# GuidoManni/BodySLAM

Measured on AMD Instinct MI355X. Metric: frames/sec depth+pose+back-proj, 640x480 seq, higher is better.
Workload: dtype f16

## Files before the change

bodyslam_amd/_lib.py:

```python
from __future__ import annotations

import ctypes as C
import os
from typing import Optional

import torch

_HERE = os.path.dirname(os.path.abspath(__file__))
LIB_PATH = os.environ.get("BODYSLAM_HIP_LIB") or os.path.join(_HERE, "libbodyslam_hip.so")

F32, F16, BF16 = 0, 1, 2
F64 = 3
ACT_NONE, ACT_RELU, ACT_GELU, ACT_SOFTPLUS, ACT_SOFTPLUS_FAST = 0, 1, 2, 3, 4
OUT_PLAIN, OUT_SHUFFLE, OUT_QKV = 0, 1, 2

_TORCH2BS = {torch.float32: F32, torch.float16: F16, torch.bfloat16: BF16}
BS2TORCH = {F32: torch.float32, F16: torch.float16, BF16: torch.bfloat16}


class BodySlamHipError(RuntimeError):
    pass


class GemmDesc(C.Structure):
    _fields_ = [
        ("A", C.c_void_p), ("W", C.c_void_p), ("dtype", C.c_int32),
        ("M", C.c_int32), ("N", C.c_int32), ("K", C.c_int32), ("lda", C.c_int32), ("conv", C.c_int32),
        ("Hin", C.c_int32), ("Win", C.c_int32), ("Cin", C.c_int32), ("Hout", C.c_int32), ("Wout", C.c_int32),
        ("KH", C.c_int32), ("KW", C.c_int32), ("stride", C.c_int32), ("pad_h", C.c_int32), ("pad_w", C.c_int32),
        ("relu_a", C.c_int32),
        ("bias", C.c_void_p), ("bias_group_rows", C.c_int32), ("act", C.c_int32),
        ("scale", C.c_void_p), ("res", C.c_void_p), ("res_dtype", C.c_int32), ("ldr", C.c_int32), ("res2", C.c_void_p),
        ("out", C.c_void_p), ("out2", C.c_void_p), ("out3", C.c_void_p),
        ("out_dtype", C.c_int32), ("ldo", C.c_int32), ("out_mode", C.c_int32),
        ("out_group_rows", C.c_int32), ("out_group_stride", C.c_int32), ("out_row_offset", C.c_int32),
        ("shuffle_s", C.c_int32), ("shuffle_cout", C.c_int32),
        ("qkv_hidden", C.c_int32), ("qkv_tokens", C.c_int32), ("qkv_sp", C.c_int32), ("q_scale", C.c_float),
        ("tile", C.c_int32), ("seg1", C.c_int32), ("out_split_off", C.c_int32), ("res_split_off", C.c_int32),
        ("f8_seg", C.c_int32), ("f8_scales", C.c_uint32), ("out_f8", C.c_int32), ("res_f8", C.c_int32),
        ("qkv_cls_last", C.c_int32), ("qkv_cls_rows", C.c_int32), ("qkv_patch_row0", C.c_int32), ("f8_wonly_from", C.c_int32), ("out_lo8_rows", C.c_int32),
        ("f8_skip_from", C.c_int32), ("bias2_row0", C.c_int32), ("bias2_group_rows", C.c_int32), ("out_planes_rows", C.c_int32),
        ("bias2", C.c_void_p),
        ("qkv_lo_off", C.c_int32), ("out2_relu", C.c_int32),
    ]


_lib: Optional[C.CDLL] = None

_SIGS = {
    "bs_init": [C.c_int],
    "bs_version": [],
    "bs_gemm": [C.POINTER(GemmDesc), C.c_void_p],
    "bs_gemm_tile": [C.POINTER(GemmDesc)],
    "bs_attention": [C.c_void_p] * 5 + [C.c_int32] * 5 + [C.c_void_p],
    "bs_attention_table": [C.c_void_p] * 5 + [C.c_int32] * 7 + [C.c_void_p],
    "bs_attention_table_corr": [C.c_void_p] * 8 + [C.c_int32] * 7 + [C.c_void_p],
    "bs_layernorm": [C.c_void_p] * 5 + [C.c_int32, C.c_int32, C.c_float, C.c_int32, C.c_void_p],
    "bs_cast": [C.c_void_p, C.c_void_p, C.c_int64, C.c_int32, C.c_void_p],
    "bs_copy_f32": [C.c_void_p, C.c_void_p, C.c_int64, C.c_void_p],
    "bs_cast_split": [C.c_void_p, C.c_void_p, C.c_int64, C.c_int32, C.c_int32, C.c_void_p],
    "bs_relu_split": [C.c_void_p, C.c_void_p, C.c_int64, C.c_int32, C.c_int32, C.c_void_p],
    "bs_preprocess_patches": [C.c_void_p, C.c_void_p] + [C.c_int32] * 7 + [C.c_void_p],
    "bs_preprocess_image": [C.c_void_p, C.c_void_p] + [C.c_int32] * 6 + [C.c_void_p],
    "bs_fill_rows": [C.c_void_p, C.c_void_p, C.c_int32, C.c_int32, C.c_int32, C.c_void_p],
    "bs_resize_bilinear_nhwc": [C.c_void_p, C.c_void_p] + [C.c_int32] * 8 + [C.c_void_p],
    "bs_upconv_tapsum": [C.c_void_p] * 3 + [C.c_int32] * 9 + [C.c_void_p],
    "bs_upconv_fused": [C.c_void_p] * 4 + [C.c_int32] * 15 + [C.c_void_p],
    "bs_resize_bias_relu_nhwc": [C.c_void_p] * 3 + [C.c_int32] * 8 + [C.c_void_p],
    "bs_col_mean": [C.c_void_p, C.c_int64] + [C.c_int32] * 5 + [C.c_void_p, C.c_void_p, C.c_int64, C.c_int32, C.c_void_p],
    "bs_rank1_bias": [C.c_void_p] * 3 + [C.c_int32] * 3 + [C.c_void_p],
    "bs_depth_u16_to_m": [C.c_void_p, C.c_int64, C.c_double, C.c_double, C.c_void_p, C.c_void_p],
    "bs_engine_load": [C.c_char_p, C.c_void_p],
    "bs_engine_destroy": [C.c_void_p],
    "bs_engine_io": [C.c_void_p, C.c_char_p, C.c_void_p, C.c_void_p],
    "bs_engine_device_bytes": [C.c_void_p],
    "bs_engine_run": [C.c_void_p, C.c_void_p],
    "bs_engine_upload": [C.c_void_p, C.c_char_p, C.c_void_p, C.c_int64],
    "bs_engine_download": [C.c_void_p, C.c_char_p, C.c_void_p, C.c_int64],
    "bs_zoedepth_forward": [C.c_void_p, C.c_void_p, C.c_int32, C.c_int32, C.c_int32, C.c_void_p, C.c_void_p, C.c_void_p],
    "bs_cyclepose_forward": [C.c_void_p, C.c_void_p, C.c_int32, C.c_int32, C.c_int32, C.c_void_p, C.c_int32, C.c_void_p, C.c_void_p],
    "bs_tsdf_frames_upload": [C.c_void_p, C.c_void_p, C.c_void_p, C.c_void_p, C.c_void_p, C.c_int32, C.c_void_p, C.c_void_p],
    "bs_tsdf_touch_batch": [C.c_void_p, C.c_int32, C.c_int32, C.c_int32, C.c_int32, C.c_double, C.c_double, C.c_void_p, C.c_void_p, C.c_int32, C.c_void_p,
                            C.c_void_p],
    "bs_tsdf_integrate_batch": [C.c_void_p, C.c_int32, C.c_int32, C.c_int32, C.c_void_p, C.c_void_p, C.c_void_p, C.c_int32, C.c_void_p, C.c_int32, C.c_void_p,
                                C.c_void_p, C.c_void_p, C.c_void_p, C.c_int32, C.c_int32, C.c_double, C.c_double, C.c_void_p],
    "bs_tsdf_update_batch": [C.c_void_p, C.c_int32, C.c_int32, C.c_int32, C.c_void_p, C.c_void_p, C.c_void_p, C.c_int32, C.c_void_p, C.c_int32, C.c_void_p,
                             C.c_void_p, C.c_void_p, C.c_void_p, C.c_int32, C.c_int32, C.c_double, C.c_double, C.c_uint64, C.c_void_p],
    "bs_odo_prepare": [C.c_void_p, C.c_void_p, C.c_int32, C.c_int32, C.c_int32, C.c_double, C.c_void_p, C.c_void_p, C.c_void_p],
    "bs_odo_pyrdown": [C.c_void_p, C.c_int32, C.c_int32, C.c_int32, C.c_void_p, C.c_int32, C.c_double, C.c_void_p],
    "bs_odo_sobel": [C.c_void_p, C.c_int32, C.c_int32, C.c_int32, C.c_void_p, C.c_void_p, C.c_void_p],
    "bs_odo_accumulate": [C.c_void_p] * 8 + [C.c_int32, C.c_int32, C.c_void_p, C.c_void_p, C.c_double, C.c_double, C.c_double, C.c_void_p, C.c_void_p,
                                              C.c_int32, C.c_void_p],
    "bs_odo_step": [C.c_void_p] * 8 + [C.c_int32, C.c_int32, C.c_int32, C.c_void_p, C.c_void_p, C.c_int32, C.c_double, C.c_double, C.c_double, C.c_void_p,
                                        C.c_void_p, C.c_int32, C.c_void_p],
    "bs_odo_p2p_prepare": [C.c_void_p, C.c_int32, C.c_int32, C.c_int32, C.c_double, C.c_void_p, C.c_void_p],
    "bs_odo_p2p_target": [C.c_void_p, C.c_int32, C.c_int32, C.c_int32, C.c_void_p, C.c_void_p, C.c_void_p],
    "bs_odo_p2p_accumulate": [C.c_void_p, C.c_void_p, C.c_int32, C.c_int32, C.c_void_p, C.c_void_p, C.c_double, C.c_double, C.c_void_p, C.c_void_p,
                              C.c_void_p],
    "bs_odo_p2p_step": [C.c_void_p, C.c_void_p, C.c_int32, C.c_int32, C.c_int32, C.c_void_p, C.c_void_p, C.c_int32, C.c_double, C.c_double, C.c_void_p,
                        C.c_void_p, C.c_void_p],
    "bs_tsdf_touch": [C.c_void_p, C.c_int32, C.c_int32, C.c_int32, C.c_void_p, C.c_void_p, C.c_double, C.c_double, C.c_void_p, C.c_void_p, C.c_void_p,
                      C.c_int32, C.c_int32, C.c_void_p, C.c_int32, C.c_void_p, C.c_void_p, C.c_void_p],
    "bs_tsdf_integrate": [C.c_void_p, C.c_void_p, C.c_int32, C.c_int32, C.c_void_p, C.c_void_p, C.c_void_p, C.c_void_p, C.c_int32, C.c_void_p, C.c_int32,
                          C.c_int32, C.c_double, C.c_double, C.c_void_p, C.c_void_p],
    "bs_tsdf_extract": [C.c_void_p, C.c_int32, C.c_void_p, C.c_void_p, C.c_int32, C.c_void_p, C.c_int32, C.c_int32, C.c_double, C.c_void_p, C.c_void_p,
                        C.c_void_p, C.c_void_p, C.c_void_p, C.c_void_p],
    "bs_tsdf_mesh": [C.c_void_p, C.c_int32, C.c_void_p, C.c_void_p, C.c_int32, C.c_void_p, C.c_int32, C.c_int32, C.c_double, C.c_void_p, C.c_int32] + [C.c_void_p] * 7,
    "bs_tsdf_raycast": [C.c_void_p, C.c_void_p, C.c_int32, C.c_int32, C.c_int32, C.c_double, C.c_double, C.c_void_p, C.c_void_p, C.c_int32, C.c_void_p,
                        C.c_int32, C.c_int32, C.c_double, C.c_double, C.c_void_p, C.c_void_p, C.c_void_p, C.c_void_p, C.c_void_p],
    "bs_attractor_step": [C.c_void_p] * 4 + [C.c_int32] * 8 + [C.c_void_p],
    "bs_add_resized": [C.c_void_p] * 3 + [C.c_int32] * 7 + [C.c_void_p],
    "bs_mlp2": [C.c_void_p, C.c_int32] + [C.c_void_p] * 5 + [C.c_int32] * 6 + [C.c_void_p],
    "bs_mlp2_add": [C.c_void_p] * 7 + [C.c_int32] * 10 + [C.c_void_p],
    "bs_projector_level": [C.c_void_p] * 10 + [C.c_int32] * 9 + [C.c_void_p],
    "bs_logbinom_depth": [C.c_void_p] * 8 + [C.c_int32] * 5 + [C.c_float, C.c_float, C.c_int32, C.c_void_p],
    "bs_logbinom_depth_ex": [C.c_void_p] * 7 + [C.c_int32] + [C.c_void_p] * 2 + [C.c_int32] * 5 + [C.c_float, C.c_float, C.c_int32, C.c_void_p],
    "bs_small_attention": [C.c_void_p, C.c_void_p, C.c_int32, C.c_int32, C.c_int32, C.c_int32, C.c_void_p],
    "bs_route_argmax": [C.c_void_p, C.c_int32, C.c_void_p, C.c_int32, C.c_void_p],
    "bs_postprocess_depth": [C.c_void_p] * 3 + [C.c_int32] * 6 + [C.c_void_p],
    "bs_cyclepose_im2col": [C.c_void_p] * 3 + [C.c_int32] * 4 + [C.c_void_p],
    "bs_cyclepose_im2col_window": [C.c_void_p] * 3 + [C.c_int32] * 8 + [C.c_void_p],
    "bs_instnorm_relu_nhwc": [C.c_void_p] * 4 + [C.c_int32] * 3 + [C.c_float, C.c_int32, C.c_void_p],
    "bs_avgpool_nhwc": [C.c_void_p, C.c_void_p, C.c_int32, C.c_int32, C.c_int32, C.c_void_p],
    "bs_cyclepose_head": [C.c_void_p] * 12 + [C.c_int32] * 3 + [C.c_void_p],
    "bs_backproject": [C.c_void_p, C.c_int32, C.c_int32, C.c_int32, C.c_void_p, C.c_double, C.c_double] + [C.c_void_p] * 6,
    "bs_pose_chain": [C.c_void_p, C.c_int32, C.c_void_p, C.c_void_p, C.c_void_p],
# ... 18 lines not shown
    "bs_loop_register": [C.c_void_p, C.c_int32, C.c_void_p, C.c_int32, C.c_void_p, C.c_void_p, C.c_int32, C.c_double, C.c_int32, C.c_int32,
                         C.c_int32, C.c_uint64, C.c_void_p, C.c_void_p, C.c_void_p],
    "bs_pg_linearise": [C.c_void_p, C.c_int32] + [C.c_void_p] * 5 + [C.c_int32, C.c_double, C.c_int32] + [C.c_void_p] * 8,
    "bs_pg_assemble": [C.c_void_p, C.c_void_p, C.c_int32, C.c_int32, C.c_void_p, C.c_void_p, C.c_int32, C.c_int32] + [C.c_void_p] * 5,
    "bs_pg_solve": [C.c_void_p] * 4 + [C.c_int32, C.c_int32, C.c_double, C.c_void_p, C.c_int32, C.c_void_p, C.c_int32, C.c_void_p, C.c_void_p, C.c_int32,
                                       C.c_void_p, C.c_int32, C.c_int32] + [C.c_void_p] * 7,
    "bs_pg_update": [C.c_void_p, C.c_void_p, C.c_int32] + [C.c_void_p] * 4,
    "bs_pc_bounds": [C.c_void_p, C.c_int64, C.c_void_p, C.c_void_p],
    "bs_pc_grid_count": [C.c_void_p, C.c_int64, C.c_void_p, C.c_void_p, C.c_float, C.c_void_p, C.c_void_p, C.c_void_p],
    "bs_pc_grid_scatter": [C.c_void_p, C.c_int64, C.c_void_p, C.c_void_p, C.c_float, C.c_void_p, C.c_void_p, C.c_int64, C.c_void_p, C.c_void_p],
    "bs_pc_query_grid": [C.c_void_p, C.c_void_p, C.c_int64, C.c_void_p, C.c_void_p, C.c_float, C.c_void_p, C.c_void_p, C.c_int64, C.c_float, C.c_int32,
                         C.c_void_p, C.c_void_p, C.c_void_p, C.c_void_p, C.c_void_p],
    "bs_pc_query_brute": [C.c_void_p, C.c_int64, C.c_void_p, C.c_void_p, C.c_int64, C.c_float, C.c_void_p, C.c_void_p, C.c_void_p, C.c_void_p],
    "bs_pc_transform": [C.c_void_p, C.c_int32, C.c_int64, C.c_void_p, C.c_void_p, C.c_void_p],
    "bs_pc_stats": [C.c_void_p, C.c_int64, C.c_void_p, C.c_int32, C.c_void_p, C.c_int64, C.c_void_p, C.c_void_p],
    "bs_icp_step": [C.c_void_p, C.c_void_p, C.c_int64, C.c_void_p, C.c_void_p, C.c_float, C.c_void_p, C.c_void_p, C.c_void_p, C.c_int64, C.c_void_p,
                    C.c_int32, C.c_int64, C.c_float, C.c_int32, C.c_int32, C.c_void_p, C.c_void_p, C.c_void_p],
    "bs_icp_finish": [C.c_void_p, C.c_int64, C.c_void_p, C.c_void_p, C.c_int32, C.c_int32, C.c_int32, C.c_double, C.c_double, C.c_void_p, C.c_void_p],
}
EXPORTS = sorted(list(_SIGS) + ["bs_last_error"])


def load_library() -> C.CDLL:
    global _lib
    if _lib is not None:
        return _lib
    if not os.path.exists(LIB_PATH):
        raise BodySlamHipError(
            f"{LIB_PATH} is missing: build it with `python -c 'import __graft_entry__ as g; g.build()'` "
            f"(or `make -C bodyslam_amd/csrc`).  There is no CPU fallback.")
    lib = C.CDLL(LIB_PATH)
    for name, args in _SIGS.items():
        fn = getattr(lib, name)
        fn.argtypes = args
        fn.restype = C.c_int
    lib.bs_last_error.restype = C.c_char_p
    lib.bs_last_error.argtypes = []
    lib.bs_engine_device_bytes.restype = C.c_int64
    lib.bs_depth_metrics_workspace.restype = C.c_int64
    _lib = lib
    return lib


_inited_device: Optional[int] = None


def init(device: int = 0) -> None:
    global _inited_device
    lib = load_library()
    if _inited_device == device:
        return
    if not torch.cuda.is_available():
        raise BodySlamHipError("bodyslam_amd needs an MI355X (gfx950) GPU: torch.cuda.is_available() is False "
                               "and there is no CPU fallback")
    check(lib.bs_init(device), "bs_init")
    _inited_device = device


def check(status: int, what: str) -> None:
    if status != 0:
        msg = load_library().bs_last_error().decode(errors="replace")
        raise BodySlamHipError(f"{what} failed with status {status}: {msg}")


def stream_ptr() -> int:
    return torch.cuda.current_stream().cuda_stream


def dt(t: torch.Tensor) -> int:
    return _TORCH2BS[t.dtype]


def p(t: Optional[torch.Tensor]) -> Optional[int]:
    return None if t is None else t.data_ptr()


def make_gemm_desc(A: torch.Tensor, W: torch.Tensor, out: torch.Tensor, *, M: int, N: int, K: int, lda: int,
                   conv=None, relu_a: bool = False, bias: Optional[torch.Tensor] = None, bias_group_rows: int = 0,
                   act: int = ACT_NONE, scale: Optional[torch.Tensor] = None, res: Optional[torch.Tensor] = None,
                   res2: Optional[torch.Tensor] = None, ldr: int = 0, ldo: Optional[int] = None, out_group=None,
                   shuffle=None, qkv=None, a_offset: int = 0, tile: int = 0, seg1: int = 0, out_split_off: int = 0,
                   res_split_off: int = 0, f8_seg: int = 0, f8_scales=(127, 127, 127, 127), out_f8=None, res_f8: bool = False,
                   f8_wonly_from: int = 0, out_lo8_rows: int = 0, f8_skip_from: int = 0, bias2=None, out_planes_rows: int = 0,
                   out_relu: Optional[torch.Tensor] = None) -> GemmDesc:
    d = GemmDesc()
    d.A = A.data_ptr() + a_offset * A.element_size()
    d.W = W.data_ptr()
    assert A.dtype == W.dtype and A.dtype in (torch.float16, torch.bfloat16), (A.dtype, W.dtype)
    d.dtype = dt(A)
    d.M, d.N, d.K, d.lda = M, N, K, lda
    if conv is not None:
        d.conv = 1
        (d.Hin, d.Win, d.Cin, d.Hout, d.Wout, d.KH, d.KW, d.stride, d.pad_h, d.pad_w) = conv
    d.relu_a = int(relu_a)
    if bias is not None:
        assert bias.dtype == torch.float32
        d.bias = bias.data_ptr()
    d.bias_group_rows = bias_group_rows
    d.act = act
    if scale is not None:
        assert scale.dtype == torch.float32
        d.scale = scale.data_ptr()
    if res is not None:
        d.res = res.data_ptr()
        d.res_dtype = dt(res)
        d.ldr = ldr if ldr else N
    if res2 is not None:
        assert res is not None and res2.dtype == A.dtype
        d.res2 = res2.data_ptr()
    d.out = out.data_ptr()
    d.out_dtype = dt(out)
    d.ldo = N if ldo is None else ldo
    if out_group is not None:
        d.out_group_rows, d.out_group_stride, d.out_row_offset = out_group
    if shuffle is not None:
        d.out_mode = OUT_SHUFFLE
        d.shuffle_s, d.shuffle_cout, d.Hout, d.Wout = shuffle
    if qkv is not None:
        d.out_mode = OUT_QKV
        hidden, tokens, sp, q_scale, out_k, out_vt = qkv[:6]
        d.qkv_cls_last = int(bool(qkv[6])) if len(qkv) > 6 else 0
        d.qkv_cls_rows = int(qkv[7]) if len(qkv) > 7 else 0
        d.qkv_patch_row0 = int(qkv[8]) if len(qkv) > 8 else d.qkv_cls_rows
        d.qkv_lo_off = int(qkv[9]) if len(qkv) > 9 else 0
        d.qkv_hidden, d.qkv_tokens, d.qkv_sp, d.q_scale = hidden, tokens, sp, q_scale
        d.out2 = out_k.data_ptr()
        d.out3 = out_vt.data_ptr()
    d.tile = tile
    d.seg1, d.out_split_off, d.res_split_off = seg1, out_split_off, res_split_off
    d.f8_seg = f8_seg
    d.f8_scales = f8_scales[0] | (f8_scales[1] << 8) | (f8_scales[2] << 16) | (f8_scales[3] << 24)
    d.out_f8 = 0 if out_f8 is None else ((out_f8[0] & 0xff) | ((out_f8[1] & 0xff) << 8))
    d.res_f8 = int(res_f8)
    d.f8_wonly_from = f8_wonly_from
    d.out_lo8_rows = out_lo8_rows
    d.f8_skip_from = f8_skip_from
    d.out_planes_rows = out_planes_rows
    if bias2 is not None:
        b2, row0, grows = bias2
        assert b2.dtype == torch.float32 and b2.shape[-1] == N
        d.bias2, d.bias2_row0, d.bias2_group_rows = b2.data_ptr(), row0, grows
    if out_relu is not None:
        assert qkv is None and out_f8 is not None and out_relu.dtype == out.dtype and out_relu.numel() == out.numel()
        d.out2 = out_relu.data_ptr()
        d.out2_relu = 1
    return d


def gemm(A: torch.Tensor, W: torch.Tensor, out: torch.Tensor, **kw) -> None:
    d = make_gemm_desc(A, W, out, **kw)
    check(load_library().bs_gemm(C.byref(d), stream_ptr()), "bs_gemm")


def _gemm_bytes(d) -> float:
    rows_in = float(d.M if not d.conv else d.M / max(d.stride * d.stride, 1))
    rows_f8 = 0.0 if d.f8_skip_from < 0 else (rows_in if (d.conv or not d.f8_skip_from) else float(min(d.f8_skip_from, d.M)))
    taps = d.KH * d.KW if d.conv else 1
    a = rows_in * (d.Cin if d.conv else d.K) * 2 + rows_f8 * d.f8_seg
    w = float(d.N) * (d.K * 2 + taps * d.f8_seg)
    if d.out_dtype == F32:
        per_row = [4.0, 4.0, 4.0]
    elif d.out_f8:
        per_row = [4.0, 3.0, 2.0]
    else:
        per_row = [2.0 * (2 if d.out_split_off else 1)] * 3
    full = float(d.M)
    r_planes = float(min(d.out_planes_rows, d.M)) if d.out_planes_rows else full
    r_lo = float(min(d.out_lo8_rows, d.M)) if d.out_lo8_rows else r_planes
    r_lo = min(r_lo, r_planes)
    out = d.N * (r_lo * per_row[0] + (r_planes - r_lo) * per_row[1] + (full - r_planes) * per_row[2])
    res = float(d.M) * d.N * (4 if (d.res and d.res_dtype == F32) else 0)
    return a + w + out + res


class Plan:

    def __init__(self, device=None):
        self.device = None if device is None else torch.device(device)
        self.calls = []
        self.names = []
        self.keep = []
        self.keep_descs = []
        self.marks = {}
        self.gemm_info = {}
        self.stack_info = {}
        self.events = None
        self._graph = None

    def gemm(self, name, A, W, out, **kw):
        passes = kw.pop("precision_passes", 1)
        d = make_gemm_desc(A, W, out, **kw)
        kw["precision_passes"] = passes
        self.keep.append((d, A, W, out, kw))
        self.keep_descs.append(d)
        self.calls.append((load_library().bs_gemm, (C.byref(d),)))
        self.names.append(name)
        self.gemm_info[len(self.calls) - 1] = dict(
            name=name, tile=load_library().bs_gemm_tile(C.byref(d)), conv=bool(d.conv),
            flops=2.0 * d.N * (d.M * d.K + (0 if d.f8_skip_from < 0 else (min(d.f8_skip_from, d.M) if d.f8_skip_from else d.M)) * (d.KH * d.KW if d.conv else 1) * d.f8_seg
                               / (4 if d.f8_wonly_from else 2)),
            alg_flops=2.0 * d.M * d.N * (d.K / kw.get("precision_passes", 1)),
            bytes=_gemm_bytes(d))

    def add(self, name, fn_name, *args):
        cargs = []
        for a in args:
            if isinstance(a, torch.Tensor):
                self.keep.append(a)
                cargs.append(a.data_ptr())
            else:
                cargs.append(a)
        self.calls.append((getattr(load_library(), fn_name), tuple(cargs)))
        self.names.append(name)

    def tag_stack(self, alg_flops: float, flops: float):
        self.stack_info[len(self.calls) - 1] = dict(name=self.names[-1], alg_flops=float(alg_flops), flops=float(flops))

    def mark(self, name, tensor, meta=None):
        self.marks.setdefault(len(self.calls), []).append((name, tensor, meta))

    def run_timed(self, events: list):
        stream = torch.cuda.current_stream(self.device)
        st = stream.cuda_stream
        for i, (fn, args) in enumerate(self.calls):
            if i in self.gemm_info or i in self.stack_info:
                e0, e1 = torch.cuda.Event(enable_timing=True), torch.cuda.Event(enable_timing=True)
                e0.record(stream)
                rc = fn(*args, st)
                e1.record(stream)
                events.append((i, e0, e1))
            else:
                rc = fn(*args, st)
            if rc:
                check(rc, self.names[i])

    def capture(self):
        if self._graph is not None:
            return
        self.run()
        torch.cuda.synchronize(self.device)
        g = torch.cuda.CUDAGraph()
        cap = torch.cuda.Stream(device=self.device)
        cap.wait_stream(torch.cuda.current_stream(self.device))
        with torch.cuda.stream(cap):
            with torch.cuda.graph(g, stream=cap, capture_error_mode="thread_local"):
                self.run()
        torch.cuda.current_stream(self.device).wait_stream(cap)
        self._graph = g

    def run(self, taps: Optional[dict] = None):
        if taps is None and self.events is not None:
            return self.run_timed(self.events)
        if taps is None and self._graph is not None and not torch.cuda.is_current_stream_capturing():
            self._graph.replay()
            return
        st = torch.cuda.current_stream(self.device).cuda_stream
        if taps is None:
            for i, (fn, args) in enumerate(self.calls):
                rc = fn(*args, st)
                if rc:
                    check(rc, self.names[i])
            return
        means = taps.get("__site_means__")
        for i in range(len(self.calls) + 1):
            for (name, t, meta) in self.marks.get(i, []):
                if meta and meta[0] == "chanmean":
                    if means is not None:
                        _, off, M, lda, K = meta
                        means[name] = t.view(-1)[off: off + M * lda].view(M, lda)[:, :K].float().mean(0)
                    continue
                if means is None:
                    taps[name] = (t.clone(), meta)
            if i < len(self.calls):
                fn, args = self.calls[i]
                check(fn(*args, st), self.names[i])


_F8_ON_DEVICE = {}


def _f8_pack_device(device):
    if device is None or os.environ.get("BS_PACK_ON_HOST") == "1":
        return torch.device("cpu")
    device = torch.device(device)
    if device.type != "cuda":
        return torch.device("cpu")
    ok = _F8_ON_DEVICE.get(device.index)
    if ok is None:
        g = torch.Generator().manual_seed(7)
        t = torch.cat([torch.randn(4096, generator=g) * 100.0, torch.randn(4096, generator=g) * 1e-2, torch.linspace(-460.0, 460.0, 4097),
                       torch.arange(0, 4096, dtype=torch.float32) * 2.0 ** -11, torch.tensor([0.0, -0.0, 448.0, -448.0, 2.0 ** -9, 2.0 ** -10, 3 * 2.0 ** -11])])
        t = t.clamp(-448.0, 448.0)
        try:
            ok = bool(torch.equal(t.to(torch.float8_e4m3fn).view(torch.uint8), t.to(device).to(torch.float8_e4m3fn).view(torch.uint8).cpu()))
        except Exception:
            ok = False
        _F8_ON_DEVICE[device.index] = ok
    return device if ok else torch.device("cpu")


def f8_weight(w: torch.Tensor, dtype, planes: str = "both", device=None) -> tuple:
    import math
    w = w.detach().to(_f8_pack_device(device)).float()
    hi = w.to(dtype)
    lo = w - hi.float()

    def plane(t):
        mx = float(t.abs().max())
        e = 0 if mx == 0.0 else min(int(math.floor(math.log2(448.0 / mx))), 100)
        return (t * (2.0 ** e)).clamp(-448.0, 448.0).to(torch.float8_e4m3fn).view(torch.uint8), e

    hi8, e_hi = plane(hi.float())
    lo8, e_lo = plane(lo)
    hi16 = hi.contiguous().view(torch.uint8).view(w.shape[0], -1)
    if planes == "lo":
        row = torch.cat([hi16, lo8], 1).contiguous()
    elif planes == "hi_only":
        row = torch.cat([hi16, torch.zeros_like(lo8), hi8], 1).contiguous()
    else:
        row = torch.cat([hi16, lo8, hi8], 1).contiguous()
    return row.view(dtype), (127 - e_lo, 127 - e_hi)


def f8_conv_weight(w_ohwi: torch.Tensor, dtype, device=None) -> tuple:
    import math
    w = w_ohwi.detach().to(_f8_pack_device(device)).float()
    O, kh, kw, I = w.shape
    assert I % 128 == 0, I
    hi = w.to(dtype)
    lo = w - hi.float()

    def plane(t):
        mx = float(t.abs().max())
        e = 0 if mx == 0.0 else min(int(math.floor(math.log2(448.0 / mx))), 100)
        q = (t * (2.0 ** e)).clamp(-448.0, 448.0).to(torch.float8_e4m3fn).view(torch.uint8)
        return q.reshape(O, kh, kw, I // 128, 128).permute(0, 3, 1, 2, 4).reshape(O, -1), e

    hi8, e_hi = plane(hi.float())
    lo8, e_lo = plane(lo)
    hi16 = conv_weight(hi).view(torch.uint8).view(O, -1)
    row = torch.cat([hi16, lo8, hi8], 1).contiguous()
    return row.view(dtype), (127 - e_lo, 127 - e_hi)


F8_ACT_HI_EXP, F8_ACT_LO_EXP = 0, 11


def conv_weight(w_ohwi: torch.Tensor) -> torch.Tensor:
    O, kh, kw, I = w_ohwi.shape
    assert I % 64 == 0, I
    return w_ohwi.reshape(O, kh, kw, I // 64, 64).permute(0, 3, 1, 2, 4).reshape(O, -1).contiguous()


def conv_geom(Hin, Win, Cin, KH, KW, stride, pad):
    Hout = (Hin + 2 * pad - KH) // stride + 1
# ... 386 lines not shown
```

bodyslam_amd/csrc/common.h:

```cpp
#pragma once
#include <hip/hip_runtime.h>
#include <stdint.h>
#include <stdio.h>
#include <stdlib.h>

#include <atomic>

#include "../../include/bodyslam_hip.h"

namespace bs {

typedef _Float16 f16;
typedef __bf16 bf16;
typedef _Float16 f16x4 __attribute__((ext_vector_type(4)));
typedef _Float16 f16x8 __attribute__((ext_vector_type(8)));
typedef __bf16 bf16x4 __attribute__((ext_vector_type(4)));
typedef __bf16 bf16x8 __attribute__((ext_vector_type(8)));
typedef float f32x4 __attribute__((ext_vector_type(4)));
typedef float f32x16 __attribute__((ext_vector_type(16)));
typedef unsigned int u32x4 __attribute__((ext_vector_type(4)));
typedef unsigned int u32x2 __attribute__((ext_vector_type(2)));

void set_error(const char* fmt, ...);
const void* zero_page();
// ... 70 lines not shown
    float p = 2.5060822736122645e-05f;
    p = fmaf(p, t, -0.0006993855931796134f);
    p = fmaf(p, t, 0.00785447470843792f);
    p = fmaf(p, t, -0.053071241825819016f);
    p = fmaf(p, t, -0.4590134918689728f);
    p = fmaf(p, t, -1.1511290073394775f);
    p = fmaf(p, t, -0.9999995231628418f);
    const float e = __builtin_amdgcn_exp2f(p);
    return x * (x < 0.0f ? e : 1.0f - e);
}
typedef float f32x2_ __attribute__((ext_vector_type(2)));
__device__ __forceinline__ f32x2_ gelu_erf2(f32x2_ x) {
    const f32x2_ t = __builtin_elementwise_min(__builtin_elementwise_abs(x), f32x2_{6.0f, 6.0f});
    f32x2_ p = f32x2_{2.5060822736122645e-05f, 2.5060822736122645e-05f};
    p = __builtin_elementwise_fma(p, t, f32x2_{-0.0006993855931796134f, -0.0006993855931796134f});
    p = __builtin_elementwise_fma(p, t, f32x2_{0.00785447470843792f, 0.00785447470843792f});
    p = __builtin_elementwise_fma(p, t, f32x2_{-0.053071241825819016f, -0.053071241825819016f});
    p = __builtin_elementwise_fma(p, t, f32x2_{-0.4590134918689728f, -0.4590134918689728f});
    p = __builtin_elementwise_fma(p, t, f32x2_{-1.1511290073394775f, -1.1511290073394775f});
    p = __builtin_elementwise_fma(p, t, f32x2_{-0.9999995231628418f, -0.9999995231628418f});
    const f32x2_ e = {__builtin_amdgcn_exp2f(p[0]), __builtin_amdgcn_exp2f(p[1])};
    const f32x2_ om = f32x2_{1.0f, 1.0f} - e;
    const f32x2_ s = {x[0] < 0.0f ? e[0] : om[0], x[1] < 0.0f ? e[1] : om[1]};
    return x * s;
}
__device__ __forceinline__ f32x2_ bilerp2(f32x2_ p00, f32x2_ p01, f32x2_ p10, f32x2_ p11, f32x2_ hx, f32x2_ lx, f32x2_ hy, f32x2_ ly) {
    const f32x2_ top = __builtin_elementwise_fma(lx, p01, hx * p00), bot = __builtin_elementwise_fma(lx, p11, hx * p10);
    return __builtin_elementwise_fma(ly, bot, hy * top);
}
__device__ __forceinline__ float erf_as(float x) {
    const float ax = fabsf(x);
    const float t = __frcp_rn(1.0f + 0.3275911f * ax);
    const float poly = ((((1.061405429f * t - 1.453152027f) * t + 1.421413741f) * t - 0.284496736f) * t + 0.254829592f) * t;
    const float r = 1.0f - poly * __expf(-ax * ax);
    return copysignf(r, x);
}
__device__ __forceinline__ float gelu_erf_as(float x) { return 0.5f * x * (1.0f + erf_as(x * 0.70710678118654752440f)); }
__device__ __forceinline__ f32x2_ gelu_erf_as2(f32x2_ x) {
    const f32x2_ ax = __builtin_elementwise_abs(x) * f32x2_{0.70710678118654752440f, 0.70710678118654752440f};
    const f32x2_ den = __builtin_elementwise_fma(f32x2_{0.3275911f, 0.3275911f}, ax, f32x2_{1.0f, 1.0f});
    const f32x2_ t = {__builtin_amdgcn_rcpf(den[0]), __builtin_amdgcn_rcpf(den[1])};
    f32x2_ q = __builtin_elementwise_fma(f32x2_{1.061405429f, 1.061405429f}, t, f32x2_{-1.453152027f, -1.453152027f});
    q = __builtin_elementwise_fma(q, t, f32x2_{1.421413741f, 1.421413741f});
    q = __builtin_elementwise_fma(q, t, f32x2_{-0.284496736f, -0.284496736f});
    q = __builtin_elementwise_fma(q, t, f32x2_{0.254829592f, 0.254829592f});
    q = q * t;
    const f32x2_ arg = (ax * ax) * f32x2_{-1.4426950408889634f, -1.4426950408889634f};
    const f32x2_ ex = {__builtin_amdgcn_exp2f(arg[0]), __builtin_amdgcn_exp2f(arg[1])};
    const f32x2_ r = __builtin_elementwise_fma(-q, ex, f32x2_{1.0f, 1.0f});
    const f32x2_ erf = {copysignf(r[0], x[0]), copysignf(r[1], x[1])};
    return (x * f32x2_{0.5f, 0.5f}) * (erf + f32x2_{1.0f, 1.0f});
}
__device__ __forceinline__ float softplus20(float x) { return x > 20.0f ? x : log1pf(expf(x)); }
__device__ __forceinline__ float softplus_fast(float x) {
    const float e = __builtin_amdgcn_exp2f(x * 1.4426950408889634f);
    const float series = e * fmaf(e, fmaf(e, fmaf(e, -0.25f, 0.3333333432674408f), -0.5f), 1.0f);
    const float lg = __builtin_amdgcn_logf(1.0f + e) * 0.6931471805599453f;
    const float y = e < 0.015625f ? series : lg;
    return x > 20.0f ? x : y;
}

__device__ __forceinline__ float apply_act(float y, int act) {
    if (act == BS_ACT_RELU) return fmaxf(y, 0.0f);
    if (act == BS_ACT_GELU) return gelu_erf(y);
    if (act == BS_ACT_SOFTPLUS) return softplus20(y);
    if (act == BS_ACT_SOFTPLUS_FAST) return softplus_fast(y);
    return y;
}

__device__ __forceinline__ int f8_pack4(float a, float b, float c, float d) {
    auto cl = [](float v) { return __builtin_amdgcn_fmed3f(v, -448.0f, 448.0f); };
    int r = 0;
    r = __builtin_amdgcn_cvt_pk_fp8_f32(cl(a), cl(b), r, false);
    r = __builtin_amdgcn_cvt_pk_fp8_f32(cl(c), cl(d), r, true);
    return r;
}
__device__ __forceinline__ void f8_unpack4(int packed, float (&o)[4]) {
    typedef float f32x2 __attribute__((ext_vector_type(2)));
    const f32x2 a = __builtin_amdgcn_cvt_pk_f32_fp8(packed, false), b = __builtin_amdgcn_cvt_pk_f32_fp8(packed, true);
    o[0] = a[0]; o[1] = a[1]; o[2] = b[0]; o[3] = b[1];
}
constexpr int F8_ACT_HI_EXP = BS_F8_ACT_HI_EXP, F8_ACT_LO_EXP = BS_F8_ACT_LO_EXP;

__device__ __forceinline__ void glds16(const void* gptr, void* lds_wave_base) {
    __builtin_amdgcn_global_load_lds((const __attribute__((address_space(1))) void*)gptr,
                                     (__attribute__((address_space(3))) void*)lds_wave_base, 16, 0, 0);
}

static inline int cdiv(int a, int b) { return (a + b - 1) / b; }
static inline int64_t cdiv64(int64_t a, int64_t b) { return (a + b - 1) / b; }

}
```

bodyslam_amd/csrc/elementwise.hip:

```cpp
#include "common.h"

namespace bs {

template <typename T>
__global__ __launch_bounds__(256) void layernorm_kernel(const float* x, const float* gamma, const float* beta, T* out16, float* out32,
                                                         int rows, int cols, float eps, int split, int plane_rows) {
    const int row = blockIdx.x * 4 + (threadIdx.x >> 6), lane = threadIdx.x & 63;
    if (row >= rows) return;
    const float* xr = x + (int64_t)row * cols;
    constexpr int VPT = 4;
    f32x4 v[VPT];
    const int nvec = cols >> 2;
    const bool cached = nvec <= 64 * VPT;
    float s = 0.f;
    if (cached) {
#pragma unroll
        for (int i = 0; i < VPT; ++i) {
            const int vi = lane + i * 64;
            v[i] = vi < nvec ? *reinterpret_cast<const f32x4*>(xr + vi * 4) : f32x4{0, 0, 0, 0};
            s += v[i][0] + v[i][1] + v[i][2] + v[i][3];
        }
    } else {
        for (int vi = lane; vi < nvec; vi += 64) {
            const f32x4 t = *reinterpret_cast<const f32x4*>(xr + vi * 4);
// ... 144 lines not shown
    const int b = blockIdx.x;
    for (int i = threadIdx.x; i < cols; i += blockDim.x) x[(int64_t)b * rows_per_image * cols + i] = v[i];
}

struct PreGeom {
    int H, W, ph, pw, nh, nw;
    float sy, sx;
};

__device__ __forceinline__ float pre_sample(const uint8_t* frame, const PreGeom& g, int c, int y, int x) {
    const float fy = g.sy * (float)y, fx = g.sx * (float)x;
    const int Hp = g.H + 2 * g.ph, Wp = g.W + 2 * g.pw;
    int y0 = (int)fy, x0 = (int)fx;
    y0 = y0 > Hp - 1 ? Hp - 1 : y0;
    x0 = x0 > Wp - 1 ? Wp - 1 : x0;
    const int y1 = y0 + (y0 < Hp - 1 ? 1 : 0), x1 = x0 + (x0 < Wp - 1 ? 1 : 0);
    const float ly = fy - (float)y0, lx = fx - (float)x0;
    const float hy = 1.0f - ly, hx = 1.0f - lx;
    auto refl = [](int i, int pad, int n) {
        int s = i - pad;
        s = s < 0 ? -s : s;
        return s >= n ? 2 * (n - 1) - s : s;
    };
    const int sy0 = refl(y0, g.ph, g.H), sy1 = refl(y1, g.ph, g.H);
    const int sx0 = refl(x0, g.pw, g.W), sx1 = refl(x1, g.pw, g.W);
    const float k = 1.0f / 255.0f;
    const float p00 = (float)frame[((int64_t)sy0 * g.W + sx0) * 3 + c] * k;
    const float p01 = (float)frame[((int64_t)sy0 * g.W + sx1) * 3 + c] * k;
    const float p10 = (float)frame[((int64_t)sy1 * g.W + sx0) * 3 + c] * k;
    const float p11 = (float)frame[((int64_t)sy1 * g.W + sx1) * 3 + c] * k;
    const float v = hy * (hx * p00 + lx * p01) + ly * (hx * p10 + lx * p11);
    return (v - 0.5f) / 0.5f;
}

template <typename T>
__global__ __launch_bounds__(256) void pre_patches_kernel(const uint8_t* frames, T* out, int B, int nimg, PreGeom g, int split) {
    const int hp = g.nh / 16, wp = g.nw / 16;
    const int64_t total = (int64_t)nimg * hp * wp * 768;
    const int64_t gid = (int64_t)blockIdx.x * blockDim.x + threadIdx.x;
    if (gid >= total) return;
    const int k = (int)(gid % 768);
    const int64_t r = gid / 768;
    const int px = (int)(r % wp), py = (int)((r / wp) % hp), img = (int)(r / ((int64_t)wp * hp));
    const int c = k >> 8, ky = (k >> 4) & 15, kx = k & 15;
    const int y = py * 16 + ky;
    int x = px * 16 + kx;
    const int b = img >= B ? img - B : img;
    if (img >= B) x = g.nw - 1 - x;
    const float v = pre_sample(frames + (int64_t)b * g.H * g.W * 3, g, c, y, x);
    const T hi = T16<T>::from_f32(v);
    if (split == 2) {
        out[r * 1536 + k] = hi;
        char* planes = reinterpret_cast<char*>(out + r * 1536 + 768);
        planes[k] = (char)(f8_pack4(v * __builtin_ldexpf(1.0f, F8_ACT_HI_EXP), 0.f, 0.f, 0.f) & 0xff);
        planes[768 + k] = (char)(f8_pack4((v - T16<T>::to_f32(hi)) * __builtin_ldexpf(1.0f, F8_ACT_LO_EXP), 0.f, 0.f, 0.f) & 0xff);
    } else if (split) {
        out[r * 1536 + k] = hi;
        out[r * 1536 + 768 + k] = T16<T>::from_f32(v - T16<T>::to_f32(hi));
    } else {
        out[gid] = hi;
    }
}

__global__ __launch_bounds__(256) void pre_image_kernel(const uint8_t* frames, float* out, int B, int nimg, PreGeom g) {
    const int64_t total = (int64_t)nimg * 3 * g.nh * g.nw;
    const int64_t gid = (int64_t)blockIdx.x * blockDim.x + threadIdx.x;
    if (gid >= total) return;
    int x = (int)(gid % g.nw);
    const int y = (int)((gid / g.nw) % g.nh), c = (int)((gid / ((int64_t)g.nw * g.nh)) % 3), img = (int)(gid / ((int64_t)3 * g.nw * g.nh));
    const int b = img >= B ? img - B : img;
    if (img >= B) x = g.nw - 1 - x;
    out[gid] = pre_sample(frames + (int64_t)b * g.H * g.W * 3, g, c, y, x);
}

template <typename T, bool LO = true, bool HI8 = true>
__global__ __launch_bounds__(256) void resize_nhwc_f8_kernel(const T* x, T* out, int B, int Hin, int Win, int C, int Hout, int Wout, float sy,
                                                              float sx, int align) {
    const int c16n = C >> 4;
    const unsigned idx = blockIdx.x * blockDim.x + threadIdx.x;
    if (idx >= (unsigned)Wout * c16n) return;
    const int c16 = idx % c16n, ox = idx / c16n;
    const int b = blockIdx.y / Hout, oy = blockIdx.y - b * Hout;
    const int64_t pix = ((int64_t)b * Hout + oy) * Wout + ox;
    float fy, fx;
    if (align) {
        fy = sy * (float)oy;
        fx = sx * (float)ox;
    } else {
        fy = fmaxf(__fmaf_rn(sy, (float)oy + 0.5f, -0.5f), 0.0f);
        fx = fmaxf(__fmaf_rn(sx, (float)ox + 0.5f, -0.5f), 0.0f);
    }
    int y0 = (int)fy, x0 = (int)fx;
    y0 = y0 > Hin - 1 ? Hin - 1 : y0;
    x0 = x0 > Win - 1 ? Win - 1 : x0;
    const int y1 = y0 + (y0 < Hin - 1 ? 1 : 0), x1 = x0 + (x0 < Win - 1 ? 1 : 0);
    const float ly = fy - (float)y0, lx = fx - (float)x0, hy = 1.0f - ly, hx = 1.0f - lx;
    typedef typename T16<T>::v8 v8;
    typedef int i32x4 __attribute__((ext_vector_type(4)));
    const T* xb = x + (int64_t)b * Hin * Win * C * 2;
    const float sc = __builtin_ldexpf(1.0f, -F8_ACT_LO_EXP);
    float q00[16], q01[16], q10[16], q11[16];
    auto ld = [&](int yy, int xx, float (&q)[16]) {
        const T* pp = xb + ((int64_t)yy * Win + xx) * C * 2;
        const v8 h0 = *reinterpret_cast<const v8*>(pp + c16 * 16), h1 = *reinterpret_cast<const v8*>(pp + c16 * 16 + 8);
        const i32x4 l = *reinterpret_cast<const i32x4*>(reinterpret_cast<const char*>(pp + C + (C >> 1)) + c16 * 16);
#pragma unroll
        for (int e = 0; e < 8; ++e) {
            q[e] = (float)h0[e];
            q[8 + e] = (float)h1[e];
        }
#pragma unroll
        for (int g = 0; g < 4; ++g) {
            float lo[4];
            f8_unpack4(l[g], lo);
#pragma unroll
            for (int e = 0; e < 4; ++e) q[4 * g + e] = fmaf(lo[e], sc, q[4 * g + e]);
        }
    };
    ld(y0, x0, q00);
    ld(y0, x1, q01);
    ld(y1, x0, q10);
    ld(y1, x1, q11);
    v8 o0, o1;
    float vv[16], rl[16];
    const f32x2_ hx2 = {hx, hx}, lx2 = {lx, lx}, hy2 = {hy, hy}, ly2 = {ly, ly};
#pragma unroll
    for (int e = 0; e < 16; e += 2) {
        const f32x2_ v2 = bilerp2(f32x2_{q00[e], q00[e + 1]}, f32x2_{q01[e], q01[e + 1]}, f32x2_{q10[e], q10[e + 1]}, f32x2_{q11[e], q11[e + 1]}, hx2, lx2, hy2, ly2);
#pragma unroll
        for (int u = 0; u < 2; ++u) {
            const float v = v2[u];
            vv[e + u] = v;
            const T h = T16<T>::from_f32(v);
            if (e + u < 8) o0[e + u] = h; else o1[e + u - 8] = h;
            if (LO) rl[e + u] = v - (float)h;
        }
    }
    T* op = out + pix * C * 2;
    *reinterpret_cast<v8*>(op + c16 * 16) = o0;
    *reinterpret_cast<v8*>(op + c16 * 16 + 8) = o1;
    if (!HI8) return;
    const float sh = __builtin_ldexpf(1.0f, F8_ACT_HI_EXP), sl = __builtin_ldexpf(1.0f, F8_ACT_LO_EXP);
    char* planes = reinterpret_cast<char*>(op + C);
    i32x4 ph, pl;
#pragma unroll
    for (int g = 0; g < 4; ++g) {
        ph[g] = f8_pack4(vv[4 * g] * sh, vv[4 * g + 1] * sh, vv[4 * g + 2] * sh, vv[4 * g + 3] * sh);
        if (LO) pl[g] = f8_pack4(rl[4 * g] * sl, rl[4 * g + 1] * sl, rl[4 * g + 2] * sl, rl[4 * g + 3] * sl);
    }
    *reinterpret_cast<i32x4*>(planes + c16 * 16) = ph;
    if (LO) *reinterpret_cast<i32x4*>(planes + C + c16 * 16) = pl;
}

template <typename T, int SPLIT>
__global__ __launch_bounds__(256) void upconv_tapsum_kernel(const float* y, const float* bias, T* out, int B, int Hin, int Win, int Co, int Hout,
                                                             int Wout, float sy, float sx, int align, int relu) {
    const int groups = Co >> 2;
    const int per = 256 / groups, TW = per >= 8 ? 8 : per, TH = per / TW;
    const int g = threadIdx.x % groups, px = threadIdx.x / groups;
    const int ox = blockIdx.x * TW + px % TW;
    const int nty = (Hout + TH - 1) / TH;
    const int b = blockIdx.y / nty, oy = (blockIdx.y - b * nty) * TH + px / TW;
    if (px >= per || ox >= Wout || oy >= Hout) return;
    const int ld = 9 * Co;
    const float* yb = y + (int64_t)b * Hin * Win * ld + 4 * g;
    typedef float f32x4_ __attribute__((ext_vector_type(4)));
    f32x4_ acc = *reinterpret_cast<const f32x4_*>(bias + 4 * g);
#pragma unroll
    for (int ky = 0; ky < 3; ++ky) {
        const int r = oy + ky - 1;
        if (r < 0 || r >= Hout) continue;
        const float fy = align ? sy * (float)r : fmaxf(__fmaf_rn(sy, (float)r + 0.5f, -0.5f), 0.0f);
        int y0 = (int)fy;
        y0 = y0 > Hin - 1 ? Hin - 1 : y0;
        const int y1 = y0 + (y0 < Hin - 1 ? 1 : 0);
        const float ly = fy - (float)y0, hy = 1.0f - ly;
#pragma unroll
        for (int kx = 0; kx < 3; ++kx) {
            const int c = ox + kx - 1;
            if (c < 0 || c >= Wout) continue;
            const float fx = align ? sx * (float)c : fmaxf(__fmaf_rn(sx, (float)c + 0.5f, -0.5f), 0.0f);
            int x0 = (int)fx;
            x0 = x0 > Win - 1 ? Win - 1 : x0;
            const int x1 = x0 + (x0 < Win - 1 ? 1 : 0);
            const float lx = fx - (float)x0, hx = 1.0f - lx;
            const float* yt = yb + (ky * 3 + kx) * Co;
            const f32x4_ q00 = *reinterpret_cast<const f32x4_*>(yt + ((int64_t)y0 * Win + x0) * ld);
            const f32x4_ q01 = *reinterpret_cast<const f32x4_*>(yt + ((int64_t)y0 * Win + x1) * ld);
            const f32x4_ q10 = *reinterpret_cast<const f32x4_*>(yt + ((int64_t)y1 * Win + x0) * ld);
            const f32x4_ q11 = *reinterpret_cast<const f32x4_*>(yt + ((int64_t)y1 * Win + x1) * ld);
            typedef float f32x2 __attribute__((ext_vector_type(2)));
            const f32x2 hx2 = {hx, hx}, lx2 = {lx, lx}, hy2 = {hy, hy}, ly2 = {ly, ly};
#pragma unroll
            for (int e = 0; e < 4; e += 2) {
                const f32x2 top = __builtin_elementwise_fma(lx2, f32x2{q01[e], q01[e + 1]}, hx2 * f32x2{q00[e], q00[e + 1]});
                const f32x2 bot = __builtin_elementwise_fma(lx2, f32x2{q11[e], q11[e + 1]}, hx2 * f32x2{q10[e], q10[e + 1]});
                const f32x2 v = __builtin_elementwise_fma(ly2, bot, hy2 * top);
                acc[e] += v[0];
                acc[e + 1] += v[1];
            }
        }
    }
    if (relu) {
#pragma unroll
        for (int e = 0; e < 4; ++e) acc[e] = fmaxf(acc[e], 0.0f);
    }
    const int64_t pix = ((int64_t)b * Hout + oy) * Wout + ox;
    typedef T t4 __attribute__((ext_vector_type(4)));
    t4 hi;
    float rl[4];
#pragma unroll
    for (int e = 0; e < 4; ++e) {
        hi[e] = T16<T>::from_f32(acc[e]);
        rl[e] = acc[e] - T16<T>::to_f32(hi[e]);
    }
    if (SPLIT == 0) {
        *reinterpret_cast<t4*>(out + pix * Co + 4 * g) = hi;
    } else if (SPLIT == 1) {
        t4 lo;
#pragma unroll
        for (int e = 0; e < 4; ++e) lo[e] = T16<T>::from_f32(rl[e]);
        *reinterpret_cast<t4*>(out + pix * 2 * Co + 4 * g) = hi;
        *reinterpret_cast<t4*>(out + pix * 2 * Co + Co + 4 * g) = lo;
    } else {
        T* op = out + pix * 2 * Co;
        *reinterpret_cast<t4*>(op + 4 * g) = hi;
        const float sh = __builtin_ldexpf(1.0f, F8_ACT_HI_EXP), sl = __builtin_ldexpf(1.0f, F8_ACT_LO_EXP);
        char* planes = reinterpret_cast<char*>(op + Co);
        *reinterpret_cast<int*>(planes + 4 * g) = f8_pack4(acc[0] * sh, acc[1] * sh, acc[2] * sh, acc[3] * sh);
        *reinterpret_cast<int*>(planes + Co + 4 * g) = f8_pack4(rl[0] * sl, rl[1] * sl, rl[2] * sl, rl[3] * sl);
    }
}
// ... 51 lines not shown
            const float l = f - (float)i0, h = 1.0f - l;
            e = i32x4_{(i0 - w0) * unit, (i1 - w0) * unit, __float_as_int(h), __float_as_int(l)};
        }
        tabs[tid] = e;
    }
    asm volatile("s_waitcnt vmcnt(0)" ::: "memory");
    __syncthreads();
    const int g = tid & 7;
    const f32x4_ bias4 = *reinterpret_cast<const f32x4_*>(bias + 4 * g);
    const char* yg = smem + TS_TAB + 16 * g;
    for (int it = 0; it < TS_TW * TS_TH / 64; ++it) {
        const int px = it * 64 + (tid >> 3);
        const int lx_ = px % TS_TW, ly_ = px / TS_TW;
        const int ox = tx0 + lx_, oy = ty0 + ly_;
        if (ox >= Wout || oy >= Hout) continue;
        f32x2 a01 = {bias4[0], bias4[1]}, a23 = {bias4[2], bias4[3]};
#pragma unroll
        for (int ky = 0; ky < 3; ++ky) {
            const i32x4_ ry = tabs[ly_ + ky];
            const float hy = __int_as_float(ry[2]), wy = __int_as_float(ry[3]);
#pragma unroll
            for (int kx = 0; kx < 3; ++kx) {
                const i32x4_ cx = tabs[TS_TH + 2 + lx_ + kx];
                const float hx = __int_as_float(cx[2]), wx = __int_as_float(cx[3]);
                const char* yt = yg + (ky * 3 + kx) * Co * 4;
                const f32x4_ q00 = *reinterpret_cast<const f32x4_*>(yt + ry[0] + cx[0]);
                const f32x4_ q01 = *reinterpret_cast<const f32x4_*>(yt + ry[0] + cx[1]);
                const f32x4_ q10 = *reinterpret_cast<const f32x4_*>(yt + ry[1] + cx[0]);
                const f32x4_ q11 = *reinterpret_cast<const f32x4_*>(yt + ry[1] + cx[1]);
                const float w00 = hy * hx, w01 = hy * wx, w10 = wy * hx, w11 = wy * wx;
                const f32x2 v00 = {w00, w00}, v01 = {w01, w01}, v10 = {w10, w10}, v11 = {w11, w11};
                a01 = __builtin_elementwise_fma(v00, f32x2{q00[0], q00[1]}, a01);
                a23 = __builtin_elementwise_fma(v00, f32x2{q00[2], q00[3]}, a23);
                a01 = __builtin_elementwise_fma(v01, f32x2{q01[0], q01[1]}, a01);
                a23 = __builtin_elementwise_fma(v01, f32x2{q01[2], q01[3]}, a23);
                a01 = __builtin_elementwise_fma(v10, f32x2{q10[0], q10[1]}, a01);
                a23 = __builtin_elementwise_fma(v10, f32x2{q10[2], q10[3]}, a23);
                a01 = __builtin_elementwise_fma(v11, f32x2{q11[0], q11[1]}, a01);
                a23 = __builtin_elementwise_fma(v11, f32x2{q11[2], q11[3]}, a23);
            }
        }
        f32x4_ acc = {a01[0], a01[1], a23[0], a23[1]};
        if (relu) {
#pragma unroll
            for (int e = 0; e < 4; ++e) acc[e] = fmaxf(acc[e], 0.0f);
        }
        const int64_t pix = ((int64_t)b * Hout + oy) * Wout + ox;
        typedef T t4 __attribute__((ext_vector_type(4)));
        t4 hi;
        float rl[4];
#pragma unroll
        for (int e = 0; e < 4; ++e) {
            hi[e] = T16<T>::from_f32(acc[e]);
            rl[e] = acc[e] - T16<T>::to_f32(hi[e]);
        }
        if (SPLIT == 0) {
            *reinterpret_cast<t4*>(out + pix * Co + 4 * g) = hi;
        } else if (SPLIT == 1) {
            t4 lo;
#pragma unroll
            for (int e = 0; e < 4; ++e) lo[e] = T16<T>::from_f32(rl[e]);
            *reinterpret_cast<t4*>(out + pix * 2 * Co + 4 * g) = hi;
            *reinterpret_cast<t4*>(out + pix * 2 * Co + Co + 4 * g) = lo;
        } else {
            T* op = out + pix * 2 * Co;
            *reinterpret_cast<t4*>(op + 4 * g) = hi;
            const float sh = __builtin_ldexpf(1.0f, F8_ACT_HI_EXP), sl = __builtin_ldexpf(1.0f, F8_ACT_LO_EXP);
            char* planes = reinterpret_cast<char*>(op + Co);
            *reinterpret_cast<int*>(planes + 4 * g) = f8_pack4(acc[0] * sh, acc[1] * sh, acc[2] * sh, acc[3] * sh);
            *reinterpret_cast<int*>(planes + Co + 4 * g) = f8_pack4(rl[0] * sl, rl[1] * sl, rl[2] * sl, rl[3] * sl);
        }
    }
}

template <typename T, bool ADD, int SPLIT, bool BIAS_RELU = false>
__global__ __launch_bounds__(256) void resize_nhwc_kernel(const T* x, const T* addend, T* out, int B, int Hin, int Win, int C, int Hout,
                                                           int Wout, float sy, float sx, int align, const float* bias = nullptr) {
    const int c8n = C >> 3;
    const unsigned idx = blockIdx.x * blockDim.x + threadIdx.x;
    if (idx >= (unsigned)Wout * c8n) return;
    const int c8 = idx % c8n, ox = idx / c8n;
    const int b = blockIdx.y / Hout, oy = blockIdx.y - b * Hout;
    const int64_t pix = ((int64_t)b * Hout + oy) * Wout + ox;
    float fy, fx;
    if (align) {
        fy = sy * (float)oy;
        fx = sx * (float)ox;
    } else {
        fy = fmaxf(__fmaf_rn(sy, (float)oy + 0.5f, -0.5f), 0.0f);
        fx = fmaxf(__fmaf_rn(sx, (float)ox + 0.5f, -0.5f), 0.0f);
    }
    int y0 = (int)fy, x0 = (int)fx;
    y0 = y0 > Hin - 1 ? Hin - 1 : y0;
    x0 = x0 > Win - 1 ? Win - 1 : x0;
    const int y1 = y0 + (y0 < Hin - 1 ? 1 : 0), x1 = x0 + (x0 < Win - 1 ? 1 : 0);
    const float ly = fy - (float)y0, lx = fx - (float)x0, hy = 1.0f - ly, hx = 1.0f - lx;
    typedef typename T16<T>::v8 v8;
    constexpr int PS = SPLIT ? 2 : 1;
    const T* xb = x + (int64_t)b * Hin * Win * C * PS + c8 * 8;
    float q00[8], q01[8], q10[8], q11[8], av[8];
    auto ld = [&](const T* ptr, float (&dst)[8]) {
        const v8 h = *reinterpret_cast<const v8*>(ptr);
#pragma unroll
        for (int e = 0; e < 8; ++e) dst[e] = (float)h[e];
        if (SPLIT == 1) {
            const v8 l = *reinterpret_cast<const v8*>(ptr + C);
#pragma unroll
            for (int e = 0; e < 8; ++e) dst[e] += (float)l[e];
        } else if (SPLIT == 2) {
            const char* lo8 = reinterpret_cast<const char*>(ptr - c8 * 8 + C + (C >> 1)) + c8 * 8;
            const int p0 = *reinterpret_cast<const int*>(lo8), p1 = *reinterpret_cast<const int*>(lo8 + 4);
            float l0[4], l1[4];
            f8_unpack4(p0, l0);
            f8_unpack4(p1, l1);
            const float sc = __builtin_ldexpf(1.0f, -F8_ACT_LO_EXP);
#pragma unroll
            for (int e = 0; e < 4; ++e) {
                dst[e] = fmaf(l0[e], sc, dst[e]);
                dst[4 + e] = fmaf(l1[e], sc, dst[4 + e]);
            }
        }
    };
    ld(xb + ((int64_t)y0 * Win + x0) * C * PS, q00);
    ld(xb + ((int64_t)y0 * Win + x1) * C * PS, q01);
    ld(xb + ((int64_t)y1 * Win + x0) * C * PS, q10);
    ld(xb + ((int64_t)y1 * Win + x1) * C * PS, q11);
    if (ADD) ld(addend + pix * C * PS + c8 * 8, av);
    v8 o, ol;
    float vv[8];
    const f32x2_ hx2 = {hx, hx}, lx2 = {lx, lx}, hy2 = {hy, hy}, ly2 = {ly, ly};
#pragma unroll
    for (int e = 0; e < 8; e += 2) {
        f32x2_ v = bilerp2(f32x2_{q00[e], q00[e + 1]}, f32x2_{q01[e], q01[e + 1]}, f32x2_{q10[e], q10[e + 1]}, f32x2_{q11[e], q11[e + 1]}, hx2, lx2, hy2, ly2);
        if (ADD) v += f32x2_{av[e], av[e + 1]};
        if (BIAS_RELU) {
            v += *reinterpret_cast<const f32x2_*>(bias + c8 * 8 + e);
            v = f32x2_{fmaxf(v[0], 0.0f), fmaxf(v[1], 0.0f)};
        }
#pragma unroll
        for (int u = 0; u < 2; ++u) {
            vv[e + u] = v[u];
            o[e + u] = T16<T>::from_f32(v[u]);
            if (SPLIT == 1) ol[e + u] = T16<T>::from_f32(v[u] - (float)o[e + u]);
        }
    }
    *reinterpret_cast<v8*>(out + pix * C * PS + c8 * 8) = o;
    if (SPLIT == 1) *reinterpret_cast<v8*>(out + pix * C * PS + C + c8 * 8) = ol;
    if (SPLIT == 2) {
        const float sh = __builtin_ldexpf(1.0f, F8_ACT_HI_EXP), sl = __builtin_ldexpf(1.0f, F8_ACT_LO_EXP);
        char* planes = reinterpret_cast<char*>(out + pix * C * 2 + C);
        typedef int i32x2 __attribute__((ext_vector_type(2)));
        *reinterpret_cast<i32x2*>(planes + c8 * 8) = i32x2{f8_pack4(vv[0] * sh, vv[1] * sh, vv[2] * sh, vv[3] * sh),
                                                           f8_pack4(vv[4] * sh, vv[5] * sh, vv[6] * sh, vv[7] * sh)};
        *reinterpret_cast<i32x2*>(planes + C + c8 * 8) =
            i32x2{f8_pack4((vv[0] - (float)o[0]) * sl, (vv[1] - (float)o[1]) * sl, (vv[2] - (float)o[2]) * sl, (vv[3] - (float)o[3]) * sl),
                  f8_pack4((vv[4] - (float)o[4]) * sl, (vv[5] - (float)o[5]) * sl, (vv[6] - (float)o[6]) * sl, (vv[7] - (float)o[7]) * sl)};
    }
}

__device__ __forceinline__ void cubic_coeffs(float t, float (&c)[4]) {
    const float A = -0.75f;
    auto c1 = [&](float x) { return ((A + 2.0f) * x - (A + 3.0f)) * x * x + 1.0f; };
    auto c2 = [&](float x) { return ((A * x - 5.0f * A) * x + 8.0f * A) * x - 4.0f * A; };
    c[0] = c2(t + 1.0f);
    c[1] = c1(t);
    c[2] = c1(1.0f - t);
    c[3] = c2(2.0f - t);
}

__global__ __launch_bounds__(256) void postprocess_kernel(const float* dnet, float* depth_m, uint16_t* depth_u16, int B, int H, int W,
                                                           int nh, int nw, int ph, int pw, float sy, float sx, int flip) {
    const int64_t total = (int64_t)B * H * W;
    const int64_t gid = (int64_t)blockIdx.x * blockDim.x + threadIdx.x;
    if (gid >= total) return;
    const int x = (int)(gid % W), y = (int)((gid / W) % H), b = (int)(gid / ((int64_t)W * H));
    const int yp = y + ph, xp = x + pw;
    const float fy = __fmaf_rn(sy, (float)yp + 0.5f, -0.5f), fx = __fmaf_rn(sx, (float)xp + 0.5f, -0.5f);
    const float fly = floorf(fy), flx = floorf(fx);
    const int iy = (int)fly, ix = (int)flx;
    float cy[4], cx[4];
    cubic_coeffs(fy - fly, cy);
    cubic_coeffs(fx - flx, cx);
    const float* d0 = dnet + (int64_t)b * nh * nw;
    const float* d1 = dnet + (int64_t)(B + b) * nh * nw;
    float acc = 0.f;
#pragma unroll
    for (int i = 0; i < 4; ++i) {
        int yy = iy - 1 + i;
        yy = yy < 0 ? 0 : (yy > nh - 1 ? nh - 1 : yy);
        float row = 0.f;
#pragma unroll
        for (int j = 0; j < 4; ++j) {
            int xx = ix - 1 + j;
            xx = xx < 0 ? 0 : (xx > nw - 1 ? nw - 1 : xx);
            float v = d0[(int64_t)yy * nw + xx];
            if (flip) v = (v + d1[(int64_t)yy * nw + (nw - 1 - xx)]) / 2.0f;
            row += v * cx[j];
        }
        acc += row * cy[i];
    }
    depth_m[gid] = acc;
    if (depth_u16) {
        float s = acc * 256.0f;
        s = s < 0.f ? 0.f : (s > 65535.f ? 65535.f : s);
        depth_u16[gid] = (uint16_t)s;
    }
}

static PreGeom make_geom(int H, int W, int nh, int nw) {
    PreGeom g;
    g.H = H; g.W = W; g.nh = nh; g.nw = nw;
    g.ph = (int)(sqrt((double)H / 2.0) * 3.0);
    g.pw = (int)(sqrt((double)W / 2.0) * 3.0);
    g.sy = nh > 1 ? (float)(H + 2 * g.ph - 1) / (float)(nh - 1) : 0.f;
    g.sx = nw > 1 ? (float)(W + 2 * g.pw - 1) / (float)(nw - 1) : 0.f;
    return g;
}

}

using namespace bs;
#define BS_ENTRY(name) \
    if (!initialized()) { set_error(name ": call bs_init first"); return BS_ERR_NOT_INIT; }

extern "C" int bs_layernorm(const float* x, const float* gamma, const float* beta, void* out16, float* out32, int32_t rows,
                            int32_t cols, float eps, int32_t dtype, void* stream) {
    BS_ENTRY("bs_layernorm");
    BS_REQUIRE(x && gamma && beta && (out16 || out32) && rows >= 0 && cols > 0 && cols % 4 == 0, "bs_layernorm: bad argument");
    const int split = (dtype & 32) ? 2 : ((dtype & 16) ? 1 : 0);
    const int plane_rows = dtype >> 8;
    dtype &= 15;
    BS_REQUIRE(!out16 || dtype == BS_F16 || dtype == BS_BF16, "bs_layernorm: dtype");
    if (rows == 0) return BS_OK;
    hipStream_t st = reinterpret_cast<hipStream_t>(stream);
    dim3 grid(cdiv(rows, 4));
    if (dtype == BS_BF16)
        hipLaunchKernelGGL(layernorm_kernel<bf16>, grid, dim3(256), 0, st, x, gamma, beta, (bf16*)out16, out32, rows, cols, eps, split, plane_rows);
    else
        hipLaunchKernelGGL(layernorm_kernel<f16>, grid, dim3(256), 0, st, x, gamma, beta, (f16*)out16, out32, rows, cols, eps, split, plane_rows);
    BS_CHECK_LAUNCH();
    return BS_OK;
}

extern "C" int bs_cast(const float* x, void* out, int64_t n, int32_t out_dtype, void* stream) {
    BS_ENTRY("bs_cast");
    BS_REQUIRE(x && out && n >= 0 && n % 4 == 0, "bs_cast: n must be a multiple of 4");
    BS_REQUIRE(out_dtype == BS_F16 || out_dtype == BS_BF16, "bs_cast: dtype");
    if (n == 0) return BS_OK;
    hipStream_t st = reinterpret_cast<hipStream_t>(stream);
    const int64_t n4 = n / 4;
    const unsigned blocks = (unsigned)(cdiv64(n4, 256) < 8192 ? cdiv64(n4, 256) : 8192);
    if (out_dtype == BS_F16)
        hipLaunchKernelGGL(cast_kernel<f16>, dim3(blocks), dim3(256), 0, st, x, (f16*)out, n4);
    else
        hipLaunchKernelGGL(cast_kernel<bf16>, dim3(blocks), dim3(256), 0, st, x, (bf16*)out, n4);
    BS_CHECK_LAUNCH();
    return BS_OK;
}

extern "C" int bs_fill_rows(float* x, const float* v, int32_t B, int32_t rows_per_image, int32_t cols, void* stream) {
    BS_ENTRY("bs_fill_rows");
    BS_REQUIRE(x && v && B >= 0 && rows_per_image > 0 && cols > 0, "bs_fill_rows: bad argument");
    if (B == 0) return BS_OK;
    hipLaunchKernelGGL(fill_rows_kernel, dim3(B), dim3(256), 0, reinterpret_cast<hipStream_t>(stream), x, v, rows_per_image, cols);
    BS_CHECK_LAUNCH();
    return BS_OK;
}

extern "C" int bs_preprocess_patches(const uint8_t* frames, void* out, int32_t B, int32_t H, int32_t W, int32_t nh, int32_t nw,
                                     int32_t flip, int32_t out_dtype, void* stream) {
    BS_ENTRY("bs_preprocess_patches");
    BS_REQUIRE(frames && out && B >= 0 && H > 1 && W > 1 && nh % 16 == 0 && nw % 16 == 0 && nh > 0 && nw > 0,
               "bs_preprocess_patches: bad geometry");
    const int split = (out_dtype & 32) ? 2 : ((out_dtype & 16) ? 1 : 0);
    out_dtype &= 15;
    BS_REQUIRE(out_dtype == BS_F16 || out_dtype == BS_BF16, "bs_preprocess_patches: dtype");
    if (B == 0) return BS_OK;
    const PreGeom g = make_geom(H, W, nh, nw);
    BS_REQUIRE(g.ph < H && g.pw < W, "bs_preprocess_patches: reflect pad exceeds the frame");
    const int nimg = flip ? 2 * B : B;
    const int64_t total = (int64_t)nimg * (nh / 16) * (nw / 16) * 768;
    hipStream_t st = reinterpret_cast<hipStream_t>(stream);
    if (out_dtype == BS_F16)
        hipLaunchKernelGGL(pre_patches_kernel<f16>, dim3((unsigned)cdiv64(total, 256)), dim3(256), 0, st, frames, (f16*)out, B, nimg, g, split);
    else
        hipLaunchKernelGGL(pre_patches_kernel<bf16>, dim3((unsigned)cdiv64(total, 256)), dim3(256), 0, st, frames, (bf16*)out, B, nimg, g, split);
    BS_CHECK_LAUNCH();
    return BS_OK;
}

extern "C" int bs_preprocess_image(const uint8_t* frames, float* out, int32_t B, int32_t H, int32_t W, int32_t nh, int32_t nw,
                                   int32_t flip, void* stream) {
    BS_ENTRY("bs_preprocess_image");
    BS_REQUIRE(frames && out && B >= 0 && H > 1 && W > 1 && nh > 0 && nw > 0, "bs_preprocess_image: bad geometry");
    if (B == 0) return BS_OK;
    const PreGeom g = make_geom(H, W, nh, nw);
    BS_REQUIRE(g.ph < H && g.pw < W, "bs_preprocess_image: reflect pad exceeds the frame");
    const int nimg = flip ? 2 * B : B;
    const int64_t total = (int64_t)nimg * 3 * nh * nw;
    hipLaunchKernelGGL(pre_image_kernel, dim3((unsigned)cdiv64(total, 256)), dim3(256), 0, reinterpret_cast<hipStream_t>(stream), frames,
                       out, B, nimg, g);
    BS_CHECK_LAUNCH();
    return BS_OK;
}

template <typename T>
static int launch_resize(const void* x, const void* addend, void* out, int B, int Hin, int Win, int C, int Hout, int Wout, int align,
                         hipStream_t st, int split = 0) {
    float sy, sx;
    if (align) {
        sy = Hout > 1 ? (float)(Hin - 1) / (float)(Hout - 1) : 0.f;
        sx = Wout > 1 ? (float)(Win - 1) / (float)(Wout - 1) : 0.f;
    } else {
        sy = (float)Hin / (float)Hout;
        sx = (float)Win / (float)Wout;
    }
    const dim3 blocks(cdiv(Wout * (C / 8), 256), B * Hout);
    if (split >= 2 && split <= 4) {
        const dim3 blocks16(cdiv(Wout * (C / 16), 256), B * Hout);
        if (split == 4)
            hipLaunchKernelGGL((resize_nhwc_f8_kernel<T, false, false>), blocks16, dim3(256), 0, st, (const T*)x, (T*)out, B, Hin, Win, C, Hout, Wout, sy, sx, align);
        else if (split == 3)
            hipLaunchKernelGGL((resize_nhwc_f8_kernel<T, false>), blocks16, dim3(256), 0, st, (const T*)x, (T*)out, B, Hin, Win, C, Hout, Wout, sy, sx, align);
        else
            hipLaunchKernelGGL((resize_nhwc_f8_kernel<T, true>), blocks16, dim3(256), 0, st, (const T*)x, (T*)out, B, Hin, Win, C, Hout, Wout, sy, sx, align);
        BS_CHECK_LAUNCH();
        return BS_OK;
    }
    if (split) {
        if (addend)
            hipLaunchKernelGGL((resize_nhwc_kernel<T, true, 1>), blocks, dim3(256), 0, st, (const T*)x, (const T*)addend, (T*)out, B, Hin, Win,
                               C, Hout, Wout, sy, sx, align);
        else
            hipLaunchKernelGGL((resize_nhwc_kernel<T, false, 1>), blocks, dim3(256), 0, st, (const T*)x, (const T*)nullptr, (T*)out, B, Hin,
                               Win, C, Hout, Wout, sy, sx, align);
        BS_CHECK_LAUNCH();
        return BS_OK;
    }
    if (addend)
        hipLaunchKernelGGL((resize_nhwc_kernel<T, true, 0>), blocks, dim3(256), 0, st, (const T*)x, (const T*)addend, (T*)out, B, Hin,
                           Win, C, Hout, Wout, sy, sx, align);
    else
        hipLaunchKernelGGL((resize_nhwc_kernel<T, false, 0>), blocks, dim3(256), 0, st, (const T*)x, (const T*)nullptr, (T*)out, B,
                           Hin, Win, C, Hout, Wout, sy, sx, align);
    BS_CHECK_LAUNCH();
    return BS_OK;
}

template <typename T>
__global__ __launch_bounds__(256) void col_mean_kernel(const T* A, int64_t lda, int row0, int rows_per_group, int row_step, int K,
                                                        bf16* out, float* zero_out, int64_t zero_n) {
    for (int64_t i = ((int64_t)blockIdx.y * gridDim.x + blockIdx.x) * 256 + threadIdx.x; i < zero_n; i += (int64_t)gridDim.x * gridDim.y * 256)
        zero_out[i] = 0.0f;
    typedef typename T16<T>::v8 v8;
    __shared__ float red[8][32][8];
    const int tx = threadIdx.x & 31, ty = threadIdx.x >> 5;
    const int g = blockIdx.y, c0 = (blockIdx.x * 32 + tx) * 8;
    const T* base = A + ((int64_t)row0 + (int64_t)g * rows_per_group) * lda;
    float acc[8] = {0.f, 0.f, 0.f, 0.f, 0.f, 0.f, 0.f, 0.f};
    if (c0 < K) {
        for (int j = ty * row_step; j < rows_per_group; j += 8 * row_step) {
            const v8 v = *reinterpret_cast<const v8*>(base + (int64_t)j * lda + c0);
#pragma unroll
            for (int e = 0; e < 8; ++e) acc[e] += T16<T>::to_f32(v[e]);
        }
    }
#pragma unroll
    for (int e = 0; e < 8; ++e) red[ty][tx][e] = acc[e];
    __syncthreads();
    if (ty == 0 && c0 < K) {
        const int count = (rows_per_group + row_step - 1) / row_step;
        const float inv = 1.0f / (float)count;
#pragma unroll
        for (int e = 0; e < 8; ++e) {
            float s_ = 0.f;
#pragma unroll
            for (int r = 0; r < 8; ++r) s_ += red[r][tx][e];
            out[(int64_t)g * K + c0 + e] = T16<bf16>::from_f32(s_ * inv);
        }
    }
}

extern "C" int bs_col_mean(const void* A, int64_t lda, int32_t row0, int32_t rows_per_group, int32_t groups, int32_t row_step, int32_t K,
                           void* out_bf16, float* zero_out, int64_t zero_n, int32_t dtype, void* stream) {
    BS_ENTRY("bs_col_mean");
    BS_REQUIRE(A && out_bf16, "bs_col_mean: null operand");
    BS_REQUIRE(row0 >= 0 && rows_per_group > 0 && groups > 0 && row_step > 0 && K > 0 && K % 8 == 0 && lda >= K && lda % 8 == 0,
               "bs_col_mean: bad geometry (K and lda must be multiples of 8)");
    BS_REQUIRE(dtype == BS_F16 || dtype == BS_BF16, "bs_col_mean: dtype must be f16 or bf16");
    hipStream_t st = reinterpret_cast<hipStream_t>(stream);
    const dim3 grid(cdiv(K, 256), groups);
    if (dtype == BS_F16)
        hipLaunchKernelGGL((col_mean_kernel<f16>), grid, dim3(256), 0, st, (const f16*)A, lda, row0, rows_per_group, row_step, K,
                           (bf16*)out_bf16, zero_out, zero_out ? zero_n : 0);
    else
        hipLaunchKernelGGL((col_mean_kernel<bf16>), grid, dim3(256), 0, st, (const bf16*)A, lda, row0, rows_per_group, row_step, K,
                           (bf16*)out_bf16, zero_out, zero_out ? zero_n : 0);
    BS_CHECK_LAUNCH();
    return BS_OK;
// ... 243 lines not shown
```

bodyslam_amd/csrc/engine.hip:

```cpp
#include <stdio.h>
#include <string.h>

#include <exception>
#include <map>
#include <string>
#include <tuple>
#include <type_traits>
#include <utility>
#include <memory>
#include <vector>

#include "common.h"

namespace {

constexpr char kMagic[8] = {'B', 'S', 'E', 'N', 'G', '0', '2', '\0'};
enum { KIND_WORKSPACE = 0, KIND_ZERO = 1, KIND_DATA = 2 };
enum { ARG_I64 = 0, ARG_F64 = 1, ARG_PTR = 2, ARG_NULL = 3, ARG_DESC = 4 };
enum { OP_CALL = 0, OP_SIGNAL = 1, OP_WAIT = 2 };

struct Arg {
    int64_t i = 0;
    double d = 0.0;
    void* p = nullptr;
};

template <typename T>
T arg_as(const Arg& a) {
    if constexpr (std::is_pointer<T>::value) return reinterpret_cast<T>(a.p);
    else if constexpr (std::is_floating_point<T>::value) return static_cast<T>(a.d);
    else return static_cast<T>(a.i);
}
template <typename... Args, size_t... I>
int call_unpacked(int (*fn)(Args...), const Arg* args, void* st, std::index_sequence<I...>) {
    using Tup = std::tuple<Args...>;
    return fn(arg_as<std::tuple_element_t<I, Tup>>(args[I])..., st);
}
struct Entry {
    int nargs;
    int (*thunk)(const void* fn, const Arg* args, void* st);
    const void* fn;
};
template <typename... Args>
Entry make_entry(int (*fn)(Args...)) {
    static_assert(sizeof...(Args) >= 1, "an entry point takes the stream last");
    Entry e;
    e.nargs = (int)sizeof...(Args) - 1;
    e.fn = reinterpret_cast<const void*>(fn);
    e.thunk = [](const void* f, const Arg* args, void* st) {
        return call_unpacked<Args...>(reinterpret_cast<int (*)(Args...)>(const_cast<void*>(f)), args, st, std::make_index_sequence<sizeof...(Args) - 1>{});
    };
    return e;
}
#define BS_ENGINE_ENTRY(name) {#name, make_entry(name)}
const std::map<std::string, Entry>& entries() {
    static const std::map<std::string, Entry> m = {
        BS_ENGINE_ENTRY(bs_gemm),           BS_ENGINE_ENTRY(bs_attention),          BS_ENGINE_ENTRY(bs_attention_table),
        BS_ENGINE_ENTRY(bs_attention_table_corr),
        BS_ENGINE_ENTRY(bs_layernorm),      BS_ENGINE_ENTRY(bs_cast),               BS_ENGINE_ENTRY(bs_copy_f32),
        BS_ENGINE_ENTRY(bs_cast_split),     BS_ENGINE_ENTRY(bs_relu_split),         BS_ENGINE_ENTRY(bs_preprocess_patches),
        BS_ENGINE_ENTRY(bs_fill_rows),      BS_ENGINE_ENTRY(bs_upconv_tapsum),      BS_ENGINE_ENTRY(bs_small_attention),
        BS_ENGINE_ENTRY(bs_route_argmax),   BS_ENGINE_ENTRY(bs_resize_bilinear_nhwc), BS_ENGINE_ENTRY(bs_rank1_bias),
        BS_ENGINE_ENTRY(bs_postprocess_depth), BS_ENGINE_ENTRY(bs_logbinom_depth_ex), BS_ENGINE_ENTRY(bs_col_mean),
        BS_ENGINE_ENTRY(bs_attractor_step), BS_ENGINE_ENTRY(bs_add_resized),        BS_ENGINE_ENTRY(bs_instnorm_relu_nhwc),
        BS_ENGINE_ENTRY(bs_cyclepose_im2col), BS_ENGINE_ENTRY(bs_cyclepose_im2col_window), BS_ENGINE_ENTRY(bs_cyclepose_head),
        BS_ENGINE_ENTRY(bs_avgpool_nhwc),   BS_ENGINE_ENTRY(bs_mlp2),            BS_ENGINE_ENTRY(bs_mlp2_add),
        BS_ENGINE_ENTRY(bs_upconv_fused),   BS_ENGINE_ENTRY(bs_resize_bias_relu_nhwc), BS_ENGINE_ENTRY(bs_projector_level),
    };
    return m;
}

struct Op {
    int kind = OP_CALL, lane = 0;
    const Entry* entry = nullptr;
    std::vector<Arg> args;
    std::vector<char> desc;
    std::string name;
};
struct Io {
    void* ptr;
    int64_t nbytes;
};

}

struct bs_engine {
    int device = 0;
    std::vector<void*> bufs;
    std::vector<Op> ops;
    std::map<std::string, Io> io;
    hipStream_t side = nullptr;
    std::map<int, hipEvent_t> events;
    int64_t device_bytes = 0;
};

namespace {

struct Reader {
    FILE* f;
// ... 296 lines not shown
```

bodyslam_amd/csrc/igemm.hip:

```cpp
#include <stdlib.h>

#include <map>
#include <mutex>
#include <utility>

#include "igemm_kernel.h"

namespace bs {

#define BS_DECL_TILE(t, cm)                                                  \
    int igemm_launch_tile##t##_f16_cm##cm(const IgemmParams&, bool, hipStream_t); \
    int igemm_launch_tile##t##_bf16_cm##cm(const IgemmParams&, bool, hipStream_t);
BS_DECL_TILE(1, 0) BS_DECL_TILE(1, 1)
BS_DECL_TILE(2, 0) BS_DECL_TILE(2, 1)
BS_DECL_TILE(3, 0) BS_DECL_TILE(3, 1)
BS_DECL_TILE(9, 0) BS_DECL_TILE(9, 1)
BS_DECL_TILE(10, 0) BS_DECL_TILE(11, 0)
BS_DECL_TILE(9s8, 0) BS_DECL_TILE(9s8, 1)
#undef BS_DECL_TILE

static int auto_tile(int M, int N, int K, int tile, bool conv) {
    if (tile != 0) return tile;
    if (N <= 32) return 3;
    if (N <= 64) return 2;
// ... 50 lines not shown
    int dev = 0;
    BS_CHECK_HIP(hipGetDevice(&dev));
    std::lock_guard<std::mutex> lock(mu);
    auto it = lanes.find({dev, caller});
    if (it == lanes.end()) {
        TailLane l{};
        BS_CHECK_HIP(hipStreamCreateWithFlags(&l.side, hipStreamNonBlocking));
        BS_CHECK_HIP(hipEventCreateWithFlags(&l.fork, hipEventDisableTiming));
        BS_CHECK_HIP(hipEventCreateWithFlags(&l.join, hipEventDisableTiming));
        it = lanes.emplace(std::make_pair(dev, caller), l).first;
    }
    side = it->second.side; ev_fork = it->second.fork; ev_join = it->second.join;
    return BS_OK;
}

static int dispatch(IgemmParams& p, int dtype, bool conv, int tile, hipStream_t st) {
    tile = auto_tile(p.M, p.N, p.K, tile, conv);
    if ((p.f8_seg > 0 || p.out_f8 || p.res_f8) && (tile == 10 || tile == 11)) tile = 9;
    int BM, BN;
    tile_dims(tile, BM, BN);
    const int rem = p.M % BM, full = p.M / BM, ntn = cdiv(p.N, BN), cus = cu_count();
    static const bool no_split = diag_env("BS_NO_TAIL_SPLIT") != nullptr;
    if (!no_split && !(p.ablate & 8) && !conv && BM == 256 && p.K >= 2048 && full > 0 && rem > 0 && rem <= 128 && p.N % 128 == 0 &&
        cdiv(full * ntn, cus) < cdiv((full + 1) * ntn, cus)) {
        IgemmParams main = p;
        main.M = full * BM;
        main.m_begin = 0;
        p.m_begin = full * BM;
        static const bool side_ok = diag_env("BS_NO_TAIL_STREAM") == nullptr;
        hipStream_t side = nullptr;
        hipEvent_t ev_fork = nullptr, ev_join = nullptr;
        if (side_ok) {
            const int rc = tail_lane(st, side, ev_fork, ev_join);
            if (rc != BS_OK) return rc;
        }
        if (!side_ok) {
            const int rc = launch_tile(main, dtype, conv, tile, st);
            if (rc != BS_OK) return rc;
            return launch_tile(p, dtype, conv, 1, st);
        }
        BS_CHECK_HIP(hipEventRecord(ev_fork, st));
        BS_CHECK_HIP(hipStreamWaitEvent(side, ev_fork, 0));
        int rc = launch_tile(main, dtype, conv, tile, st);
        if (rc != BS_OK) return rc;
        rc = launch_tile(p, dtype, conv, 1, side);
        if (rc != BS_OK) return rc;
        BS_CHECK_HIP(hipEventRecord(ev_join, side));
        BS_CHECK_HIP(hipStreamWaitEvent(st, ev_join, 0));
        return BS_OK;
    }
    p.m_begin = 0;
    return launch_tile(p, dtype, conv, tile, st);
}

}

extern "C" int bs_gemm_tile(const bs_gemm_desc* d) {
    if (!d) return BS_ERR_INVALID;
    const int tile = bs::auto_tile(d->M, d->N, d->K + d->f8_seg / 2, d->tile % 100, d->conv != 0);
    return ((d->f8_seg > 0 || d->out_f8 || d->res_f8) && (tile == 10 || tile == 11)) ? 9 : tile;
}

extern "C" int bs_gemm(const bs_gemm_desc* d, void* stream) {
    using namespace bs;
    if (!initialized()) { set_error("bs_gemm: call bs_init first"); return BS_ERR_NOT_INIT; }
    BS_REQUIRE(d && d->A && d->W && d->out, "bs_gemm: null operand");
    BS_REQUIRE(d->dtype == BS_F16 || d->dtype == BS_BF16, "bs_gemm: dtype must be f16 or bf16");
    BS_REQUIRE(d->M > 0 && d->N > 0 && d->K > 0, "bs_gemm: empty problem M=%d N=%d K=%d", d->M, d->N, d->K);
    BS_REQUIRE(d->N % 4 == 0, "bs_gemm: N=%d must be a multiple of 4", d->N);
    BS_REQUIRE(d->K % 64 == 0, "bs_gemm: K=%d must be a multiple of 64", d->K);
    BS_REQUIRE(d->lda % 8 == 0, "bs_gemm: lda=%d must be a multiple of 8 (16-byte rows)", d->lda);
    BS_REQUIRE(d->out_dtype == BS_F32 || d->out_dtype == d->dtype, "bs_gemm: out_dtype must be f32 or the operand dtype");
    BS_REQUIRE(!d->res || d->res_dtype == BS_F32 || d->res_dtype == d->dtype, "bs_gemm: res_dtype must be f32 or the operand dtype");
    IgemmParams p{};
    p.A = d->A; p.W = d->W; p.zero = zero_page();
    p.a_bytes = d->conv ? (long long)(d->M / (d->Hout > 0 && d->Wout > 0 ? d->Hout * d->Wout : 1)) * d->Hin * d->Win * d->lda * 2
                        : ((long long)(d->M - 1) * d->lda + (d->K + d->f8_seg / 2 - d->seg1)) * 2;
    BS_REQUIRE((long long)d->N * (d->K + d->f8_seg / 2) * 2 < 0x7FFFFFF0ll, "bs_gemm: weight matrix too large for one descriptor");
    p.M = d->M; p.N = d->N; p.K = d->K + d->f8_seg / 2; p.lda = d->lda;
    p.f8_seg = d->f8_seg;
    p.f8_sa0 = d->f8_scales & 0xff; p.f8_sb0 = (d->f8_scales >> 8) & 0xff; p.f8_sa1 = (d->f8_scales >> 16) & 0xff; p.f8_sb1 = d->f8_scales >> 24;
    p.out_f8 = d->out_f8;
    p.res_f8 = d->res_f8;
    BS_REQUIRE(!d->res_f8 || (d->res && d->res_dtype == d->dtype && d->res_split_off == 0 && d->ldr >= 2 * d->N && d->N % 8 == 0), "bs_gemm: res_f8 needs a 16-bit residual in (hi16 | hi8 | lo8) rows, ldr >= 2N");
    BS_REQUIRE(d->f8_seg >= 0 && d->f8_seg % 256 == 0, "bs_gemm: f8_seg=%d must be a multiple of 256 (two halves of whole 128-byte stages)", d->f8_seg);
    BS_REQUIRE(d->f8_seg == 0 || (d->seg1 == 0 && !d->relu_a), "bs_gemm: the FP8 segment excludes seg1 and relu_a");
    p.f8_stages = d->f8_seg / 128;
    BS_REQUIRE(d->out_f8 == 0 || (d->out_dtype == d->dtype && d->ldo % 8 == 0 &&
                                  ((d->out_mode == BS_OUT_PLAIN && d->out_split_off == d->N && d->N % 8 == 0) ||
                                   (d->out_mode == BS_OUT_SHUFFLE && d->out_split_off == d->shuffle_cout && d->shuffle_cout % 8 == 0))),
               "bs_gemm: out_f8 needs a plain / shuffle 16-bit output with out_split_off = channels, channels %% 8 == 0");
    p.Hin = d->Hin; p.Win = d->Win; p.Cin = d->Cin; p.Hout = d->Hout; p.Wout = d->Wout;
    p.KH = d->KH; p.KW = d->KW; p.stride = d->stride; p.pad_h = d->pad_h; p.pad_w = d->pad_w;
    if (d->conv) {
        BS_REQUIRE(d->Cin > 0 && d->Cin % 64 == 0, "bs_gemm: conv Cin=%d must be a multiple of 64", d->Cin);
        BS_REQUIRE(d->K == d->KH * d->KW * (d->Cin + d->seg1), "bs_gemm: conv K=%d != KH*KW*(Cin+seg1)", d->K);
        BS_REQUIRE(d->Hout > 0 && d->Wout > 0 && d->M % (d->Hout * d->Wout) == 0, "bs_gemm: conv M=%d not a multiple of Hout*Wout", d->M);
        BS_REQUIRE(d->stride > 0 && d->lda >= d->Cin, "bs_gemm: bad conv stride/lda");
        BS_REQUIRE(d->KH > 0 && d->KW > 0 && d->KH * d->KW <= 32, "bs_gemm: conv window %dx%d: at most 32 taps", d->KH, d->KW);
        BS_REQUIRE((long long)d->Hin * d->Win * d->lda * 2 * 4 < 0x7FFFFFF0ll, "bs_gemm: image too large for the 2 GiB tile window");
        p.tiles_per_tap = d->Cin / 64;
        if (d->f8_seg > 0) {
            BS_REQUIRE(d->f8_seg == 2 * d->Cin && d->Cin % 128 == 0 && d->lda >= 2 * d->Cin, "bs_gemm: conv FP8 segment needs f8_seg = 2*Cin, Cin %% 128 == 0, lda >= 2*Cin");
            p.Cin = 2 * d->Cin;
            p.K = d->KH * d->KW * p.Cin;
            p.f8_stages = d->KH * d->KW * (d->f8_seg / 128);
            BS_REQUIRE((long long)d->N * p.K * 2 < 0x7FFFFFF0ll, "bs_gemm: weight matrix too large for one descriptor");
        }
    }
    p.relu_a = d->relu_a;
    p.cin1 = d->seg1;
    p.split_off = d->out_split_off;
    p.res_split_off = d->res_split_off;
    BS_REQUIRE(d->seg1 >= 0 && d->seg1 % 64 == 0, "bs_gemm: seg1=%d must be a multiple of 64", d->seg1);
    BS_REQUIRE(d->conv || d->seg1 < d->K, "bs_gemm: seg1 must be smaller than K");
    BS_REQUIRE(d->out_split_off == 0 || (d->out_mode != BS_OUT_QKV && d->out_dtype == d->dtype), "bs_gemm: split output needs a plain / shuffle 16-bit output");
    BS_REQUIRE(d->res_split_off == 0 || (d->res && d->res_dtype == d->dtype), "bs_gemm: split residual must be 16-bit");
    p.ablate = d->tile >= 100 ? d->tile / 100 : 0;

    BS_REQUIRE(!d->relu_a || d->conv, "bs_gemm: relu_a is only built for conv mode");
    BS_REQUIRE(d->act >= BS_ACT_NONE && d->act <= BS_ACT_SOFTPLUS_FAST, "bs_gemm: unknown activation %d", d->act);
    p.bias = d->bias; p.bias_group_rows = d->bias_group_rows; p.act = d->act; p.scale = d->scale;
    p.res = d->res; p.res2 = d->res2; p.res_dtype = d->res_dtype; p.ldr = d->ldr;
    BS_REQUIRE(!d->res2 || d->res, "bs_gemm: res2 needs res (they share ldr)");
    p.out = d->out; p.out2 = d->out2; p.out3 = d->out3; p.out_dtype = d->out_dtype; p.ldo = d->ldo; p.out_mode = d->out_mode;
    p.out_group_rows = d->out_group_rows; p.out_group_stride = d->out_group_stride; p.out_row_offset = d->out_row_offset;
    p.shuffle_s = d->shuffle_s; p.shuffle_cout = d->shuffle_cout;
    p.qkv_hidden = d->qkv_hidden; p.qkv_tokens = d->qkv_tokens; p.qkv_sp = d->qkv_sp; p.q_scale = d->q_scale;
    p.qkv_cls_last = d->qkv_cls_last;
    p.qkv_cls_rows = d->qkv_cls_rows;
    p.qkv_patch_row0 = d->qkv_patch_row0;
    p.qkv_lo_off = d->qkv_lo_off;
    p.out2_relu = d->out2_relu;
    BS_REQUIRE(!d->out2_relu || (d->out2 && d->out_mode == BS_OUT_PLAIN && d->out_f8 && !d->scale && !d->out_group_rows && !d->bias_group_rows &&
                                 !d->bias2 && (d->act == BS_ACT_NONE || d->act == BS_ACT_RELU) && d->out_split_off == d->N && d->N % 256 == 0 &&
                                 d->ldo % 8 == 0 && d->out_dtype == d->dtype && (!d->res || d->res_f8)),
               "bs_gemm: out2_relu needs the plain (hi16 | hi8 | lo8) output form (out_f8, N %% 256 == 0, no scale / row groups / bias2)");
    BS_REQUIRE(d->qkv_lo_off == 0 || (d->out_mode == BS_OUT_QKV && d->qkv_lo_off > 0 && d->qkv_lo_off % 8 == 0),
               "bs_gemm: qkv_lo_off needs BS_OUT_QKV and a multiple of 8 elements");
    p.f8_wonly_from = d->f8_wonly_from;
    p.out_lo8_rows = d->out_lo8_rows;
    p.f8_skip_from = d->f8_skip_from;
    p.out_planes_rows = d->out_planes_rows;
    BS_REQUIRE(d->out_planes_rows == 0 || (d->out_f8 && d->out_planes_rows > 0 && d->out_planes_rows % 256 == 0),
               "bs_gemm: out_planes_rows needs out_f8 and a multiple of 256 rows");
    p.bias2 = d->bias2;
    p.bias2_row0 = d->bias2_row0;
    p.bias2_group_rows = d->bias2_group_rows;
    BS_REQUIRE(d->f8_skip_from == 0 || (d->f8_seg > 0 && (d->f8_skip_from == -1 || (d->f8_skip_from > 0 && d->f8_skip_from % 256 == 0 && !d->conv))),
               "bs_gemm: f8_skip_from needs the FP8 correction segment and is -1 (every tile) or, for a plain GEMM, a multiple of 256 rows");
    BS_REQUIRE(!d->bias2 || (d->bias2_group_rows > 0 && d->bias2_row0 >= 0 && d->bias_group_rows == 0 && !d->conv && d->out_mode != BS_OUT_SHUFFLE &&
                             d->N % 4 == 0),
               "bs_gemm: bias2 needs bias2_group_rows > 0, a plain GEMM (PLAIN or QKV output) and no bias_group_rows");
    BS_REQUIRE(d->out_lo8_rows == 0 || (d->out_f8 && d->out_lo8_rows % 256 == 0), "bs_gemm: out_lo8_rows needs out_f8 and a multiple of 256 rows");
    BS_REQUIRE(d->f8_wonly_from == 0 || d->f8_seg > 0, "bs_gemm: f8_wonly_from needs the FP8 correction segment");
    BS_REQUIRE(d->qkv_cls_rows == 0 || (d->out_mode == BS_OUT_QKV && d->qkv_cls_last && d->qkv_tokens > 1 && d->qkv_patch_row0 >= d->qkv_cls_rows &&
                                        d->M == d->qkv_patch_row0 + d->qkv_cls_rows * (d->qkv_tokens - 1)),
               "bs_gemm: qkv_cls_rows needs BS_OUT_QKV, qkv_cls_last and M = qkv_patch_row0 + qkv_cls_rows * (tokens - 1)");
    if (d->out_mode == BS_OUT_SHUFFLE) {
        BS_REQUIRE(!d->conv && d->shuffle_s > 0 && d->shuffle_cout % 4 == 0 && d->N == d->shuffle_s * d->shuffle_s * d->shuffle_cout,
                   "bs_gemm: bad shuffle geometry");
        BS_REQUIRE(d->Hout > 0 && d->Wout > 0 && d->M % (d->Hout * d->Wout) == 0, "bs_gemm: shuffle needs the input grid in Hout/Wout");
    } else if (d->out_mode == BS_OUT_QKV) {
        BS_REQUIRE(d->out2 && d->out3 && d->qkv_hidden % 64 == 0 && d->N == 3 * d->qkv_hidden && d->qkv_tokens > 0 &&
                       (d->qkv_cls_rows > 0 || d->M % d->qkv_tokens == 0) && d->qkv_sp >= d->qkv_tokens && d->out_dtype == d->dtype,
                   "bs_gemm: bad qkv geometry");
    } else {
        BS_REQUIRE(d->out_mode == BS_OUT_PLAIN && d->ldo >= d->N, "bs_gemm: bad out_mode/ldo");
        BS_REQUIRE(d->ldo % 4 == 0, "bs_gemm: ldo must be a multiple of 4");
    }
    hipStream_t st = reinterpret_cast<hipStream_t>(stream);
    const int tile = d->tile % 100;
    return dispatch(p, d->dtype, d->conv != 0, tile, st);
}
```

bodyslam_amd/csrc/igemm_kernel.h:

```cpp
#pragma once
#include <type_traits>

#include "common.h"

namespace bs {

struct IgemmParams {
    const void* A;
    const void* W;
    const void* zero;
    long long a_bytes;
    int M, N, K, lda;
    int Hin, Win, Cin, Hout, Wout, KH, KW, stride, pad_h, pad_w;
    int tiles_per_tap;
    int cin1;
    int split_off;
    int res_split_off;
    int relu_a;
    const float* bias;
    int bias_group_rows;
    int act;
    const float* scale;
    const void* res;
    const void* res2;
    int res_dtype, ldr;
    void* out;
    void* out2;
    void* out3;
    int out_dtype, ldo, out_mode;
    int out_group_rows, out_group_stride, out_row_offset;
    int shuffle_s, shuffle_cout;
    int qkv_hidden, qkv_tokens, qkv_sp;
    int qkv_cls_last;
    int qkv_cls_rows;
    int qkv_patch_row0;
    int qkv_lo_off;
    int f8_wonly_from;
    float q_scale;
    int ntm, ntn;
    int m_begin;
    int f8_seg;
    int f8_sa0, f8_sb0, f8_sa1, f8_sb1;
    int f8_stages;
    int res_f8;
    int out_f8;
    int out2_relu;
    int out_lo8_rows;
    int f8_skip_from;
    int out_planes_rows;
    const float* bias2;
    int bias2_row0, bias2_group_rows;
    int strip;
    int ablate;
};

template <typename T>
__device__ __forceinline__ typename T16<T>::v8 relu8(typename T16<T>::v8 x) {
    typedef short s16x8 __attribute__((ext_vector_type(8)));
    s16x8 b = __builtin_bit_cast(s16x8, x);
    s16x8 neg = b >> 15;
    b = b & ~neg;
    return __builtin_bit_cast(typename T16<T>::v8, b);
}

template <typename T>
__device__ __forceinline__ void store4(void* base, int64_t off, int out_dtype, const float (&y)[4], int split_off = 0) {
    if (split_off > 0) {
        typename T16<T>::v4 h, l;
#pragma unroll
        for (int e = 0; e < 4; ++e) {
            h[e] = T16<T>::from_f32(y[e]);
            l[e] = T16<T>::from_f32(y[e] - T16<T>::to_f32(h[e]));
        }
        *reinterpret_cast<typename T16<T>::v4*>(reinterpret_cast<T*>(base) + off) = h;
        *reinterpret_cast<typename T16<T>::v4*>(reinterpret_cast<T*>(base) + off + split_off) = l;
        return;
    }
    if (out_dtype == BS_F32) {
        f32x4 v = {y[0], y[1], y[2], y[3]};
        *reinterpret_cast<f32x4*>(reinterpret_cast<float*>(base) + off) = v;
    } else {
        typename T16<T>::v4 v;
        v[0] = T16<T>::from_f32(y[0]);
        v[1] = T16<T>::from_f32(y[1]);
        v[2] = T16<T>::from_f32(y[2]);
        v[3] = T16<T>::from_f32(y[3]);
        *reinterpret_cast<typename T16<T>::v4*>(reinterpret_cast<T*>(base) + off) = v;
    }
}

template <typename T>
__device__ __forceinline__ void store8(void* base, int64_t off, int out_dtype, const float (&y)[8], int split_off = 0) {
    typedef typename T16<T>::v8 v8;
    if (split_off > 0) {
        v8 h, l;
#pragma unroll
        for (int e = 0; e < 8; ++e) {
            h[e] = T16<T>::from_f32(y[e]);
            l[e] = T16<T>::from_f32(y[e] - T16<T>::to_f32(h[e]));
        }
        *reinterpret_cast<v8*>(reinterpret_cast<T*>(base) + off) = h;
        *reinterpret_cast<v8*>(reinterpret_cast<T*>(base) + off + split_off) = l;
        return;
    }
    if (out_dtype == BS_F32) {
        *reinterpret_cast<f32x4*>(reinterpret_cast<float*>(base) + off) = f32x4{y[0], y[1], y[2], y[3]};
        *reinterpret_cast<f32x4*>(reinterpret_cast<float*>(base) + off + 4) = f32x4{y[4], y[5], y[6], y[7]};
    } else {
        v8 v;
#pragma unroll
        for (int e = 0; e < 8; ++e) v[e] = T16<T>::from_f32(y[e]);
        *reinterpret_cast<v8*>(reinterpret_cast<T*>(base) + off) = v;
    }
}

template <typename T>
__device__ __forceinline__ void store8_f8(void* base, int64_t row_off, int n, int plane_off, const float (&y)[8], int ea, int el, bool lo = true,
                                          bool hi8 = true) {
    typedef typename T16<T>::v8 v8;
    typedef int i32x2 __attribute__((ext_vector_type(2)));
    v8 h;
    f32x2_ yh[4];
    const float sa = __builtin_ldexpf(1.0f, ea), sl = __builtin_ldexpf(1.0f, el);
    const f32x2_ sa2 = {sa, sa}, sl2 = {sl, sl};
#pragma unroll
    for (int e = 0; e < 8; e += 2) {
        h[e] = T16<T>::from_f32(y[e]);
        h[e + 1] = T16<T>::from_f32(y[e + 1]);
        const f32x2_ v = f32x2_{y[e], y[e + 1]} * sa2;
        yh[e >> 1] = f32x2_{__builtin_amdgcn_fmed3f(v[0], -448.0f, 448.0f), __builtin_amdgcn_fmed3f(v[1], -448.0f, 448.0f)};
    }
    T* rowp = reinterpret_cast<T*>(base) + row_off;
    *reinterpret_cast<v8*>(rowp + n) = h;
    if (!hi8) return;
    int ph0 = 0, ph1 = 0;
    ph0 = __builtin_amdgcn_cvt_pk_fp8_f32(yh[0][0], yh[0][1], ph0, false);
    ph0 = __builtin_amdgcn_cvt_pk_fp8_f32(yh[1][0], yh[1][1], ph0, true);
    ph1 = __builtin_amdgcn_cvt_pk_fp8_f32(yh[2][0], yh[2][1], ph1, false);
    ph1 = __builtin_amdgcn_cvt_pk_fp8_f32(yh[3][0], yh[3][1], ph1, true);
    char* bytes = reinterpret_cast<char*>(rowp + plane_off);
    *reinterpret_cast<i32x2*>(bytes + n) = i32x2{ph0, ph1};
    if (lo) {
        f32x2_ yl[4];
#pragma unroll
        for (int e = 0; e < 8; e += 2) {
            const f32x2_ r = (f32x2_{y[e], y[e + 1]} + f32x2_{-T16<T>::to_f32(h[e]), -T16<T>::to_f32(h[e + 1])}) * sl2;
            yl[e >> 1] = f32x2_{__builtin_amdgcn_fmed3f(r[0], -448.0f, 448.0f), __builtin_amdgcn_fmed3f(r[1], -448.0f, 448.0f)};
        }
        int pl0 = 0, pl1 = 0;
        pl0 = __builtin_amdgcn_cvt_pk_fp8_f32(yl[0][0], yl[0][1], pl0, false);
        pl0 = __builtin_amdgcn_cvt_pk_fp8_f32(yl[1][0], yl[1][1], pl0, true);
        pl1 = __builtin_amdgcn_cvt_pk_fp8_f32(yl[2][0], yl[2][1], pl1, false);
        pl1 = __builtin_amdgcn_cvt_pk_fp8_f32(yl[3][0], yl[3][1], pl1, true);
        *reinterpret_cast<i32x2*>(bytes + plane_off + n) = i32x2{pl0, pl1};
    }
}

template <typename T>
__device__ __forceinline__ void add_lo8(float* y, const void* base, int64_t row_off, int C, int n) {
    const char* lp = reinterpret_cast<const char*>(reinterpret_cast<const T*>(base) + row_off + C + (C >> 1)) + n;
    const int packed = *reinterpret_cast<const int*>(lp);
    typedef float f32x2 __attribute__((ext_vector_type(2)));
    const f32x2 a = __builtin_amdgcn_cvt_pk_f32_fp8(packed, false), b = __builtin_amdgcn_cvt_pk_f32_fp8(packed, true);
    const float sc = __builtin_ldexpf(1.0f, -BS_F8_ACT_LO_EXP);
    y[0] += a[0] * sc; y[1] += a[1] * sc; y[2] += b[0] * sc; y[3] += b[1] * sc;
}

constexpr int NW_CHECK(int a, int b) { return a * b; }

template <int N>
__device__ __forceinline__ void wait_vmcnt() {
    asm volatile("s_waitcnt vmcnt(%0)" ::"n"(N) : "memory");
}

template <typename T, int BM, int BN, int WM, int WN, int BK, int STAGES, int MODE, bool PP = false, int CM = 0, int SCHED = 0>
__global__ __launch_bounds__(WM* WN * 64, 2) void igemm_kernel(const IgemmParams p) {
#if defined(__HIP_DEVICE_COMPILE__)
    constexpr bool CONV = MODE != 0;
    constexpr bool RELU_A = MODE == 2;
    constexpr bool F8 = CM != 0;
    constexpr int NT = WM * WN * 64;
    constexpr int ROWB = BK * 2;
    constexpr int LPR = ROWB / 16;
    constexpr int RPR = NT / LPR;
    constexpr int RPW = 64 / LPR;
    constexpr int RA = BM / RPR, RB = BN / RPR;
    static_assert(BK == 64 || BK == 32, "BK");
    static_assert(BM % RPR == 0 && BN % RPR == 0, "tile rows must be a multiple of the DMA round");
    constexpr int GL = RA + RB;
    static_assert(GL * (STAGES - 1) <= 63, "vmcnt range");
    constexpr int TM = BM / WM, TN = BN / WN;
    constexpr int FM = TM / 16, FN = TN / 16;
    static_assert(TM % 16 == 0 && TN % 16 == 0, "wave tile must be a multiple of 16");
    constexpr int A_BYTES = BM * ROWB, B_BYTES = BN * ROWB, STAGE = A_BYTES + B_BYTES;
    constexpr int LDS_BYTES = STAGES * STAGE;
    constexpr unsigned OOB = 0x80000000u;
    typedef typename T16<T>::v8 v8;

    extern __shared__ __attribute__((aligned(16))) char smem[];

    const int nwg = gridDim.x, bid = blockIdx.x;
    const int xq = nwg >> 3, xr = nwg & 7, xcd = bid & 7, loc = bid >> 3;
    const int wg = (xcd < xr ? xcd * (xq + 1) : xr * (xq + 1) + (xcd - xr) * xq) + loc;
    int tm, tn;
    if (p.strip > 0) {
        const int per = p.ntm * p.strip, s = wg / per, r = wg - s * per;
        const int wl = p.ntn - s * p.strip < p.strip ? p.ntn - s * p.strip : p.strip;
        tm = r / wl;
        tn = s * p.strip + (r - tm * wl);
    } else {
        tm = wg / p.ntn;
        tn = wg - tm * p.ntn;
    }

    const int tid = threadIdx.x, lane = tid & 63;
    const int wave = __builtin_amdgcn_readfirstlane(tid >> 6);
    const int wm = wave / WN, wn = wave - wm * WN;
    const int srow = tid / LPR;
    const int sswz = (BK == 64) ? (srow & 7) : ((0 - (srow >> 2)) & 3);
    const int cs16 = ((tid & (LPR - 1)) ^ sswz) * 16;

    const int m0 = p.m_begin + tm * BM;
    long long a_base_el;
    int img0 = 0;
    if (CONV) {
        img0 = m0 / (p.Hout * p.Wout);
        a_base_el = (long long)img0 * p.Hin * p.Win * p.lda;
    } else {
        a_base_el = (long long)m0 * p.lda;
    }
    long long a_left = p.a_bytes - a_base_el * 2;
    a_left = a_left > 0x7FFFFFF0ll ? 0x7FFFFFF0ll : a_left;
    const __amdgpu_buffer_rsrc_t a_rsrc = __builtin_amdgcn_make_buffer_rsrc(
        const_cast<T*>(reinterpret_cast<const T*>(p.A)) + a_base_el, 0, (int)a_left, 0x00020000);
    const int w_pitch = p.K * 2;
    const __amdgpu_buffer_rsrc_t w_rsrc = __builtin_amdgcn_make_buffer_rsrc(
        const_cast<void*>(p.W), 0, (int)((long long)p.N * w_pitch), 0x00020000);

    unsigned a_off[RA];
    unsigned a_mask[RA];
#pragma unroll
    for (int j = 0; j < RA; ++j) {
        int m = m0 + j * RPR + srow;
        m = m < p.M ? m : p.M - 1;
        if (CONV) {
            const int hw = p.Hout * p.Wout;
            const int b = m / hw, rem = m - b * hw;
            const int oy = rem / p.Wout, ox = rem - oy * p.Wout;
            const int iy0 = oy * p.stride - p.pad_h, ix0 = ox * p.stride - p.pad_w;
            a_off[j] = (unsigned)((((b - img0) * p.Hin + iy0) * p.Win + ix0) * p.lda * 2 + cs16);
// ... 332 lines not shown
        const int grp = wm;
        v8 af[FM], bf[FN];
        auto load_frags = [&](int buf) {
            const char* sa = smem + buf * STAGE;
            const char* sb = sa + A_BYTES;
#pragma unroll
            for (int i = 0; i < FM; ++i) {
                af[i] = *reinterpret_cast<const v8*>(sa + a_base + i * 16 * ROWB + koff0);
                if (RELU_A) af[i] = relu8<T>(af[i]);
            }
#pragma unroll
            for (int j = 0; j < FN; ++j) bf[j] = *reinterpret_cast<const v8*>(sb + b_base + j * 16 * ROWB + koff0);
        };
        auto compute = [&]() {
            __builtin_amdgcn_s_setprio(1);
#pragma unroll
            for (int i = 0; i < FM; ++i)
#pragma unroll
                for (int j = 0; j < FN; ++j) acc[i][j] = T16<T>::mfma16(bf[j], af[i], acc[i][j]);
            __builtin_amdgcn_s_setprio(0);
        };
        auto wait_tiles = [&](int younger) {
            if (younger >= 2) wait_vmcnt<2 * GL>();
            else if (younger == 1) wait_vmcnt<GL>();
            else wait_vmcnt<0>();
        };
        auto phase_barrier = [&]() {
            __builtin_amdgcn_sched_barrier(0);
            __builtin_amdgcn_s_barrier();
            __builtin_amdgcn_sched_barrier(0);
        };
#pragma unroll
        for (int s = 0; s < 3; ++s)
            if (s < nt) stage(s);
        wait_tiles((nt - 1 < 2 ? nt - 1 : 2));
        phase_barrier();
        int issued = nt - 1 < 2 ? nt - 1 : 2;
        if (grp == 1) {
            phase_barrier();
            if (3 < nt) { stage(3); issued = 3; }
        }
        __builtin_amdgcn_s_waitcnt(0xc07f);
        load_frags(0);
        int buf = 0;
        const int last = nt - 1;
        for (int t = 0; t < nt; ++t) {
            const int nbuf = buf == 3 ? 0 : buf + 1;
            if (grp == 1 && t + 1 < nt) wait_tiles(issued - (t + 1));
            phase_barrier();
            compute();
            if (grp == 0 && t + 1 < nt) wait_tiles(issued - (t + 1));
            phase_barrier();
            if (t + 1 < nt) {
                if (issued < last) { ++issued; stage(issued & 3); }
                load_frags(nbuf);
            }
            buf = nbuf;
        }
        if (grp == 0) phase_barrier();
    }

#define BS_FRESH_LANE                                                                                                       \
    int lane;                                                                                                               \
    asm volatile("v_mbcnt_lo_u32_b32 %0, -1, 0\n\tv_mbcnt_hi_u32_b32 %0, -1, %0" : "=v"(lane));                             \
    const int frow = lane & 15, fq = lane >> 4;                                                                             \
    (void)frow; (void)fq;
    {
    const int n_wave = tn * BN + wn * TN;
    const bool v_tile = (p.out_mode == BS_OUT_QKV) && (tn * BN >= 2 * p.qkv_hidden);
    if (p.ablate & 4) {
        if (acc[0][0][0] == 12345.678f) reinterpret_cast<float*>(p.out)[0] = 1.f;
        return;
    }
    int g2 = -1;
    bool b2_rows = false;
    if (p.bias2) {
        const int lo = m0 - p.bias2_row0, hi = (m0 + BM < p.M ? m0 + BM : p.M) - 1 - p.bias2_row0;
        if (hi >= 0) {
            if (lo >= 0 && lo / p.bias2_group_rows == hi / p.bias2_group_rows) g2 = lo / p.bias2_group_rows;
            else b2_rows = true;
        }
    }
    if (!v_tile) {
        auto epi = [&](auto act_tag) {
            constexpr int ACT = decltype(act_tag)::value;
            BS_FRESH_LANE
            f32x4 bj[FN], sj[FN];
            int n0j[FN];
            int64_t coff[FN];
            int which[FN];
#pragma unroll
            for (int j = 0; j < FN; ++j) {
                const int n0 = n_wave + (j >> 1) * 32 + fq * 8 + (j & 1) * 4;
                n0j[j] = n0;
                const bool ok = n0 < p.N;
                bj[j] = (p.bias && !p.bias_group_rows && ok) ? *reinterpret_cast<const f32x4*>(p.bias + n0) : f32x4{0.f, 0.f, 0.f, 0.f};
                if (g2 >= 0 && ok) bj[j] += *reinterpret_cast<const f32x4*>(p.bias2 + (int64_t)g2 * p.N + n0);
                sj[j] = (p.scale && ok) ? *reinterpret_cast<const f32x4*>(p.scale + n0) : f32x4{1.f, 1.f, 1.f, 1.f};
                which[j] = 0;
                if (p.out_mode == BS_OUT_PLAIN) {
                    coff[j] = n0;
                } else if (p.out_mode == BS_OUT_SHUFFLE) {
                    const int s = p.shuffle_s;
                    const int tap = n0 / p.shuffle_cout, co = n0 - tap * p.shuffle_cout;
                    const int ky = tap / s, kx = tap - ky * s;
                    coff[j] = ((int64_t)ky * (p.Wout * s) + kx) * p.ldo + co;
                } else {
                    const int w_ = n0 / p.qkv_hidden, rem = n0 - w_ * p.qkv_hidden;
                    which[j] = w_;
                    coff[j] = (int64_t)(rem >> 6) * p.qkv_sp * 64 + (rem & 63);
                    if (w_ == 0) {
#pragma unroll
                        for (int e = 0; e < 4; ++e) { sj[j][e] *= p.q_scale; bj[j][e] *= 1.0f; }
                    }
                }
            }
            const bool wide_ok = (p.out_mode == BS_OUT_QKV) || (p.ldo % 8 == 0 && p.split_off % 8 == 0);
#pragma unroll
            for (int i = 0; i < FM; ++i) {
                const int m = m0 + wm * TM + i * 16 + frow;
                if (m >= p.M) continue;
                int64_t orow = m;
                int64_t roff;
                const float* brow = nullptr;
                if (p.bias && p.bias_group_rows) brow = p.bias + (int64_t)(m / p.bias_group_rows) * p.N;
                const float* brow2 = (b2_rows && m >= p.bias2_row0) ? p.bias2 + (int64_t)((m - p.bias2_row0) / p.bias2_group_rows) * p.N : nullptr;
                if (p.out_mode == BS_OUT_PLAIN) {
                    if (p.out_group_rows) {
                        const int g = m / p.out_group_rows;
                        orow = (int64_t)g * p.out_group_stride + (m - g * p.out_group_rows) + p.out_row_offset;
                    }
                    roff = orow * p.ldo;
                } else if (p.out_mode == BS_OUT_SHUFFLE) {
                    const int hw = p.Hout * p.Wout;
                    const int ob = m / hw, rem = m - ob * hw;
                    const int oy = rem / p.Wout, ox = rem - oy * p.Wout;
                    const int s = p.shuffle_s;
                    roff = (((int64_t)(ob * p.Hout + oy) * s) * (p.Wout * s) + ox * s) * p.ldo;
                } else {
                    int ob, otok;
                    if (p.qkv_cls_rows > 0) {
                        if (m >= p.qkv_cls_rows && m < p.qkv_patch_row0) continue;
                        const int mp = m - p.qkv_patch_row0;
                        ob = mp < 0 ? m : mp / (p.qkv_tokens - 1);
                        otok = mp < 0 ? p.qkv_tokens - 1 : mp - ob * (p.qkv_tokens - 1);
                    } else {
                        ob = m / p.qkv_tokens;
                        otok = m - ob * p.qkv_tokens;
                        if (p.qkv_cls_last) otok = otok == 0 ? p.qkv_tokens - 1 : otok - 1;
                    }
                    roff = ((int64_t)ob * (p.qkv_hidden >> 6) * p.qkv_sp + otok) * 64;
                }
                float yall[FN / 2][8];
#pragma unroll
                for (int jp = 0; jp < FN / 2; ++jp) {
                    float (&y8)[8] = yall[jp];
#pragma unroll
                    for (int h = 0; h < 2; ++h) {
                        const int j = jp * 2 + h;
                        float* y = y8 + h * 4;
                        if (n0j[j] >= p.N) continue;
                        f32x4 bsum = brow ? *reinterpret_cast<const f32x4*>(brow + n0j[j]) : bj[j];
                        if (brow2) bsum += *reinterpret_cast<const f32x4*>(brow2 + n0j[j]);
#pragma unroll
                        for (int e = 0; e < 4; ++e) y[e] = acc[i][j][e] + bsum[e];
                        const bool res32 = p.res && p.res_dtype == BS_F32;
                        if (ACT == BS_ACT_GELU) {
                            const f32x2_ g0 = gelu_erf2(f32x2_{y[0], y[1]}), g1 = gelu_erf2(f32x2_{y[2], y[3]});
                            y[0] = g0[0]; y[1] = g0[1]; y[2] = g1[0]; y[3] = g1[1];
                        }
#pragma unroll
                        for (int e = 0; e < 4; ++e) {
                            if (ACT == BS_ACT_RELU) y[e] = fmaxf(y[e], 0.0f);
                            else if (ACT == BS_ACT_SOFTPLUS) y[e] = softplus20(y[e]);
                            else if (ACT == BS_ACT_SOFTPLUS_FAST) y[e] = softplus_fast(y[e]);
                            if (!res32) y[e] *= sj[j][e];
                        }
                        if (p.res) {
                            const int64_t ro = orow * p.ldr + n0j[j];
                            if (p.res_dtype == BS_F32) {
                                const f32x4 rr = *reinterpret_cast<const f32x4*>(reinterpret_cast<const float*>(p.res) + ro);
#pragma unroll
                                for (int e = 0; e < 4; ++e) y[e] = __builtin_fmaf(y[e], sj[j][e], rr[e]);
                            } else {
                                const typename T16<T>::v4 rr = *reinterpret_cast<const typename T16<T>::v4*>(reinterpret_cast<const T*>(p.res) + ro);
#pragma unroll
                                for (int e = 0; e < 4; ++e) y[e] += T16<T>::to_f32(rr[e]);
                                if (p.res_split_off > 0) {
                                    const typename T16<T>::v4 rl = *reinterpret_cast<const typename T16<T>::v4*>(reinterpret_cast<const T*>(p.res) + ro + p.res_split_off);
#pragma unroll
                                    for (int e = 0; e < 4; ++e) y[e] += T16<T>::to_f32(rl[e]);
                                } else if (F8 && p.res_f8) {
                                    add_lo8<T>(y, p.res, orow * p.ldr, p.N, n0j[j]);
                                }
                            }
                            if (p.res2) {
                                const typename T16<T>::v4 rr = *reinterpret_cast<const typename T16<T>::v4*>(reinterpret_cast<const T*>(p.res2) + ro);
#pragma unroll
                                for (int e = 0; e < 4; ++e) y[e] += T16<T>::to_f32(rr[e]);
                                if (p.res_split_off > 0) {
                                    const typename T16<T>::v4 rl = *reinterpret_cast<const typename T16<T>::v4*>(reinterpret_cast<const T*>(p.res2) + ro + p.res_split_off);
#pragma unroll
                                    for (int e = 0; e < 4; ++e) y[e] += T16<T>::to_f32(rl[e]);
                                } else if (F8 && p.res_f8) {
                                    add_lo8<T>(y, p.res2, orow * p.ldr, p.N, n0j[j]);
                                }
                            }
                        }
                    }
                }
#pragma unroll
                for (int jp = 0; jp < FN / 2; ++jp) {
                    float (&y8)[8] = yall[jp];
                    const int j0 = jp * 2, j1 = j0 + 1;
                    if (n0j[j0] >= p.N) continue;
                    void* dst = (p.out_mode == BS_OUT_QKV && which[j0] == 1) ? p.out2 : p.out;
                    const int so = p.out_mode != BS_OUT_QKV ? p.split_off : p.qkv_lo_off;
                    if (F8 && p.out_f8) {
                        const int nloc = p.out_mode == BS_OUT_SHUFFLE ? n0j[j0] % p.shuffle_cout : n0j[j0];
                        store8_f8<T>(dst, roff + coff[j0] - nloc, nloc, so, y8, p.out_f8 & 0xff, (p.out_f8 >> 8) & 0xff);
                    } else if (wide_ok && n0j[j1] < p.N && coff[j1] == coff[j0] + 4 && which[j1] == which[j0]) {
                        store8<T>(dst, roff + coff[j0], p.out_dtype, y8, so);
                    } else {
                        const float(&ya)[4] = *reinterpret_cast<const float(*)[4]>(y8);
                        store4<T>(dst, roff + coff[j0], p.out_dtype, ya, so);
                        if (n0j[j1] < p.N) {
                            const float(&yb)[4] = *reinterpret_cast<const float(*)[4]>(y8 + 4);
                            void* dst1 = (p.out_mode == BS_OUT_QKV && which[j1] == 1) ? p.out2 : p.out;
                            store4<T>(dst1, roff + coff[j1], p.out_dtype, yb, so);
                        }
                    }
                }
            }
        };
        const bool plain_full = p.out_mode == BS_OUT_PLAIN && !p.out_group_rows && p.bias && !p.bias_group_rows && p.N % BN == 0 &&
                                p.ldo % 8 == 0 && !b2_rows && !(p.ablate & 16);
        if (plain_full && p.act == BS_ACT_NONE && p.res && p.res_dtype == BS_F32 && !p.res2 && p.out_dtype == BS_F32 && p.split_off == 0 &&
            !(F8 && p.out_f8) && p.scale && p.ldr % 4 == 0) {
            BS_FRESH_LANE
            constexpr int NP = FM * (FN / 2), DEPTH = 8;
            const float* resp = reinterpret_cast<const float*>(p.res);
            float* outp = reinterpret_cast<float*>(p.out);
            f32x4 bj[FN], sj[FN];
#pragma unroll
            for (int j = 0; j < FN; ++j) {
                const int n0 = n_wave + (j >> 1) * 32 + fq * 8 + (j & 1) * 4;
                bj[j] = *reinterpret_cast<const f32x4*>(p.bias + n0);
                if (g2 >= 0) bj[j] += *reinterpret_cast<const f32x4*>(p.bias2 + (int64_t)g2 * p.N + n0);
                sj[j] = *reinterpret_cast<const f32x4*>(p.scale + n0);
            }
            const int mrow = m0 + wm * TM + frow;
            f32x4 rq[DEPTH][2];
            auto issue = [&](int it, int slot) {
                const int i = it / (FN / 2), jp = it - i * (FN / 2);
                int m = mrow + i * 16;
                m = m < p.M ? m : p.M - 1;
                const float* rp = resp + (int64_t)m * p.ldr + n_wave + jp * 32 + fq * 8;
                rq[slot][0] = *reinterpret_cast<const f32x4*>(rp);
                rq[slot][1] = *reinterpret_cast<const f32x4*>(rp + 4);
            };
#pragma unroll
            for (int it = 0; it < DEPTH; ++it) issue(it, it);
#pragma unroll
            for (int it = 0; it < NP; ++it) {
                const int i = it / (FN / 2), jp = it - i * (FN / 2);
                const int m = mrow + i * 16;
                f32x4 y0, y1;
#pragma unroll
                for (int e = 0; e < 4; ++e) {
                    y0[e] = __builtin_fmaf(acc[i][2 * jp][e] + bj[2 * jp][e], sj[2 * jp][e], rq[it % DEPTH][0][e]);
                    y1[e] = __builtin_fmaf(acc[i][2 * jp + 1][e] + bj[2 * jp + 1][e], sj[2 * jp + 1][e], rq[it % DEPTH][1][e]);
                }
                if (it + DEPTH < NP) issue(it + DEPTH, it % DEPTH);
                if (m < p.M) {
                    float* op = outp + (int64_t)m * p.ldo + n_wave + jp * 32 + fq * 8;
                    *reinterpret_cast<f32x4*>(op) = y0;
                    *reinterpret_cast<f32x4*>(op + 4) = y1;
                }
            }
            return;
        }
        if constexpr (F8) {
            if (p.out_mode == BS_OUT_PLAIN && !p.out_group_rows && !p.bias_group_rows && p.N % BN == 0 && p.ldo % 8 == 0 && !b2_rows &&
                !(p.ablate & (16 | 2048)) && p.out_f8 && !p.scale && (p.act == BS_ACT_NONE || p.act == BS_ACT_RELU) && p.split_off == p.N &&
                p.N % 8 == 0 && p.out_dtype != BS_F32 &&
                (!p.res || (p.res_f8 && p.res_dtype != BS_F32 && p.res_split_off == 0 && p.ldr % 8 == 0)) && (!p.res2 || p.res)) {
                BS_FRESH_LANE
                typedef typename T16<T>::v8 v8;
                typedef int i32x2 __attribute__((ext_vector_type(2)));
                typedef float f32x2 __attribute__((ext_vector_type(2)));
                constexpr int NP = FM * (FN / 2), RDEPTH = 4;
                f32x4 bj[FN];
#pragma unroll
                for (int j = 0; j < FN; ++j) {
                    const int n0 = n_wave + (j >> 1) * 32 + fq * 8 + (j & 1) * 4;
                    bj[j] = p.bias ? *reinterpret_cast<const f32x4*>(p.bias + n0) : f32x4{0.f, 0.f, 0.f, 0.f};
                    if (g2 >= 0) bj[j] += *reinterpret_cast<const f32x4*>(p.bias2 + (int64_t)g2 * p.N + n0);
                }
                const bool relu = p.act == BS_ACT_RELU;
                const int mrow = m0 + wm * TM + frow;
                const int ea = p.out_f8 & 0xff, el = (p.out_f8 >> 8) & 0xff;
                const bool lo_plane = !(p.out_lo8_rows > 0 && m0 >= p.out_lo8_rows);
                const bool hi_plane = !(p.out_planes_rows > 0 && m0 >= p.out_planes_rows);
                const float lsc = __builtin_ldexpf(1.0f, -BS_F8_ACT_LO_EXP);
                auto body = [&](auto nres_tag) {
                    constexpr int NRES = decltype(nres_tag)::value;
                    v8 rh[NRES ? RDEPTH : 1][NRES ? NRES : 1];
                    i32x2 rl[NRES ? RDEPTH : 1][NRES ? NRES : 1];
                    auto issue = [&](int it, int slot) {
                        const int i = it / (FN / 2), jp = it - i * (FN / 2);
                        int m = mrow + i * 16;
                        m = m < p.M ? m : p.M - 1;
                        const int n = n_wave + jp * 32 + fq * 8;
#pragma unroll
                        for (int q = 0; q < NRES; ++q) {
                            const T* rp = reinterpret_cast<const T*>(q ? p.res2 : p.res) + (int64_t)m * p.ldr;
                            rh[slot][q] = *reinterpret_cast<const v8*>(rp + n);
                            rl[slot][q] = *reinterpret_cast<const i32x2*>(reinterpret_cast<const char*>(rp + p.N + (p.N >> 1)) + n);
                        }
                    };
                    if constexpr (NRES > 0) {
#pragma unroll
                        for (int it = 0; it < RDEPTH; ++it) issue(it, it);
                    }
#pragma unroll
                    for (int it = 0; it < NP; ++it) {
                        const int i = it / (FN / 2), jp = it - i * (FN / 2);
                        const int m = mrow + i * 16;
                        float y8[8];
#pragma unroll
                        for (int h = 0; h < 2; ++h)
#pragma unroll
                            for (int e = 0; e < 4; ++e) {
                                float y = acc[i][2 * jp + h][e] + bj[2 * jp + h][e];
                                if (relu) y = fmaxf(y, 0.0f);
                                y8[4 * h + e] = y;
                            }
                        if constexpr (NRES > 0) {
#pragma unroll
                            for (int q = 0; q < NRES; ++q) {
                                const v8 hv = rh[it % RDEPTH][q];
                                const i32x2 lv = rl[it % RDEPTH][q];
#pragma unroll
                                for (int h = 0; h < 2; ++h) {
#pragma unroll
                                    for (int e = 0; e < 4; ++e) y8[4 * h + e] += T16<T>::to_f32(hv[4 * h + e]);
                                    const f32x2 a = __builtin_amdgcn_cvt_pk_f32_fp8(lv[h], false), b = __builtin_amdgcn_cvt_pk_f32_fp8(lv[h], true);
                                    y8[4 * h] += a[0] * lsc; y8[4 * h + 1] += a[1] * lsc; y8[4 * h + 2] += b[0] * lsc; y8[4 * h + 3] += b[1] * lsc;
                                }
                            }
                            if (it + RDEPTH < NP) issue(it + RDEPTH, it % RDEPTH);
                        }
                        if (m < p.M) store8_f8<T>(p.out, (int64_t)m * p.ldo, n_wave + jp * 32 + fq * 8, p.split_off, y8, ea, el, lo_plane && hi_plane, hi_plane);
                        if (p.out2_relu) {
#pragma unroll
                            for (int e = 0; e < 8; ++e) y8[e] = fmaxf(y8[e], 0.0f);
                            if (m < p.M) store8_f8<T>(p.out2, (int64_t)m * p.ldo, n_wave + jp * 32 + fq * 8, p.split_off, y8, ea, el);
                        }
                    }
                };
                if (p.res2) body(std::integral_constant<int, 2>{});
                else if (p.res) body(std::integral_constant<int, 1>{});
                else body(std::integral_constant<int, 0>{});
                return;
            }
            if (plain_full && p.act == BS_ACT_GELU && !p.res && p.out_f8 && !p.scale && p.split_off == p.N && p.N % 8 == 0) {
                BS_FRESH_LANE
                const bool lo = !(p.out_lo8_rows > 0 && m0 >= p.out_lo8_rows);
                const bool planes = !(p.out_planes_rows > 0 && m0 >= p.out_planes_rows);
                f32x4 bj[FN];
#pragma unroll
                for (int j = 0; j < FN; ++j) {
                    const int n0 = n_wave + (j >> 1) * 32 + fq * 8 + (j & 1) * 4;
                    bj[j] = *reinterpret_cast<const f32x4*>(p.bias + n0);
                    if (g2 >= 0) bj[j] += *reinterpret_cast<const f32x4*>(p.bias2 + (int64_t)g2 * p.N + n0);
                }
                if constexpr (TM == 128 && TN == 64 && LDS_BYTES >= WM * WN * 16384) {
                    if (!planes && m0 + BM <= p.M && !(p.ablate & 1024)) {
                        typedef unsigned u32x4_ __attribute__((ext_vector_type(4)));
                        __syncthreads();
                        char* sw = smem + wave * 16384;
                        const int s7 = frow & 7;
                        const int wb0 = frow * 128 + ((fq ^ s7) << 4), wb1 = frow * 128 + (((4 + fq) ^ s7) << 4);
                        const int rr = lane >> 3, pc = lane & 7;
                        const int rb = rr * 128 + ((pc ^ rr) << 4);
                        T* op = reinterpret_cast<T*>(p.out) + (int64_t)(m0 + wm * TM + rr) * p.ldo + n_wave + pc * 8;
                        const int64_t step = (int64_t)8 * p.ldo;
#pragma unroll
                        for (int ip = 0; ip < FM; ip += 2) {
                            char* sr = sw + ((ip >> 1) & 1) * 4096;
#pragma unroll
                            for (int ii = 0; ii < 2; ++ii) {
                                const int i = ip + ii;
#pragma unroll
                                for (int jp = 0; jp < FN / 2; ++jp) {
                                    typename T16<T>::v8 h8v;
#pragma unroll
                                    for (int h = 0; h < 2; ++h) {
                                        const f32x4 v = acc[i][2 * jp + h] + bj[2 * jp + h];
                                        const f32x2_ g0 = gelu_erf2(f32x2_{v[0], v[1]}), g1 = gelu_erf2(f32x2_{v[2], v[3]});
                                        h8v[4 * h] = T16<T>::from_f32(g0[0]); h8v[4 * h + 1] = T16<T>::from_f32(g0[1]);
                                        h8v[4 * h + 2] = T16<T>::from_f32(g1[0]); h8v[4 * h + 3] = T16<T>::from_f32(g1[1]);
                                    }
                                    *reinterpret_cast<typename T16<T>::v8*>(sr + (jp ? wb1 : wb0) + ii * 2048) = h8v;
                                }
                            }
                            __builtin_amdgcn_fence(__ATOMIC_RELEASE, "wavefront");
                            __builtin_amdgcn_wave_barrier();
#pragma unroll
                            for (int it = 0; it < 4; ++it) {
                                *reinterpret_cast<u32x4_*>(op) = *reinterpret_cast<const u32x4_*>(sr + rb + it * 1024);
                                op += step;
                            }
                        }
                        return;
                    }
                }
#pragma unroll
                for (int i = 0; i < FM; ++i) {
                    const int m = m0 + wm * TM + i * 16 + frow;
                    if (m >= p.M) continue;
#pragma unroll
                    for (int jp = 0; jp < FN / 2; ++jp) {
                        float y8[8];
#pragma unroll
                        for (int h = 0; h < 2; ++h) {
                            const f32x4 v = acc[i][2 * jp + h] + bj[2 * jp + h];
                            const f32x2_ g0 = gelu_erf2(f32x2_{v[0], v[1]}), g1 = gelu_erf2(f32x2_{v[2], v[3]});
                            y8[4 * h] = g0[0]; y8[4 * h + 1] = g0[1]; y8[4 * h + 2] = g1[0]; y8[4 * h + 3] = g1[1];
                        }
                        if (planes) {
                            store8_f8<T>(p.out, (int64_t)m * p.ldo, n_wave + jp * 32 + fq * 8, p.split_off, y8, p.out_f8 & 0xff, (p.out_f8 >> 8) & 0xff, lo);
                        } else {
                            typename T16<T>::v8 h;
#pragma unroll
                            for (int e = 0; e < 8; ++e) h[e] = T16<T>::from_f32(y8[e]);
                            *reinterpret_cast<typename T16<T>::v8*>(reinterpret_cast<T*>(p.out) + (int64_t)m * p.ldo + n_wave + jp * 32 + fq * 8) = h;
                        }
                    }
                }
                return;
            }
        }
        if (F8 && p.out_mode == BS_OUT_QKV && p.qkv_hidden % BN == 0 && p.act == BS_ACT_NONE && !p.res && p.bias && !p.bias_group_rows && !b2_rows &&
            p.out_dtype != BS_F32 && !(p.ablate & 16)) {
            BS_FRESH_LANE
// ... 302 lines not shown
```

bodyslam_amd/engine_export.py:

```python
from __future__ import annotations

import bisect
import ctypes as C
import struct
from typing import Dict, Iterable, List, Tuple

import torch

from . import _lib as L

MAGIC = b"BSENG02\0"
KIND_WORKSPACE, KIND_ZERO, KIND_DATA = 0, 1, 2
ARG_I64, ARG_F64, ARG_PTR, ARG_NULL, ARG_DESC = 0, 1, 2, 3, 4
OP_CALL = 0


def _tensors(obj, out: list):
    if isinstance(obj, torch.Tensor):
        if obj.is_cuda:
            out.append(obj)
    elif isinstance(obj, (tuple, list)):
        for o in obj:
            _tensors(o, out)
    elif isinstance(obj, dict):
        for o in obj.values():
            _tensors(o, out)


class _Buffers:

    def __init__(self, tensors: Iterable[torch.Tensor], workspace_ptrs: set):
        seen: Dict[int, torch.Tensor] = {}
        for t in tensors:
            st = t.untyped_storage()
            if st.data_ptr() not in seen:
                seen[st.data_ptr()] = t
        self.base = sorted(seen)
        self.size = [seen[b].untyped_storage().nbytes() for b in self.base]
        self.rep = [seen[b] for b in self.base]
        self.workspace = [b in workspace_ptrs for b in self.base]

    def locate(self, ptr: int, what: str) -> Tuple[int, int]:
        i = bisect.bisect_right(self.base, ptr) - 1
        if i < 0 or ptr >= self.base[i] + max(self.size[i], 1):
            raise ValueError(f"engine export: {what} points at device memory the plan does not keep alive ({ptr:#x})")
        return i, ptr - self.base[i]

    def bytes_of(self, i: int) -> torch.Tensor:
        st = self.rep[i].untyped_storage()
        return torch.empty(0, dtype=torch.uint8, device=self.rep[i].device).set_(st, 0, (st.nbytes(),)).cpu()


def _pack_name(s: str, n: int) -> bytes:
    b = s.encode()
    assert len(b) < n, s
    return b + b"\0" * (n - len(b))


def export_plan(plan: L.Plan, path: str, io: Dict[str, torch.Tensor], workspace: Iterable[torch.Tensor] = ()) -> dict:
    ts: List[torch.Tensor] = []
    _tensors(plan.keep, ts)
    _tensors(list(io.values()), ts)
    ws = list(workspace)
    _tensors(ws, ts)
    bufs = _Buffers(ts, {t.untyped_storage().data_ptr() for t in ws})
    io_ptrs = {t.untyped_storage().data_ptr() for t in io.values()}
    desc_of = {}
    gi = 0
    for i, (fn, args) in enumerate(plan.calls):
        if fn.__name__ == "bs_gemm":
            desc_of[i] = plan.keep_descs[gi]
            gi += 1
    ptr_fields = [(name, getattr(L.GemmDesc, name).offset) for name, ty in L.GemmDesc._fields_ if ty is C.c_void_p]

    calls = bytearray()
    n_ops = 0
    for i, (fn, args) in enumerate(plan.calls):
        name = fn.__name__
        sig = L._SIGS[name][:-1]
        assert len(sig) == len(args), (name, len(sig), len(args))
        calls += struct.pack("<II", OP_CALL, 0) + _pack_name(name, 48) + struct.pack("<I", len(args))
        for j, (ty, a) in enumerate(zip(sig, args)):
            if name == "bs_gemm":
                d = desc_of[i]
                raw = bytes(C.string_at(C.addressof(d), C.sizeof(d)))
                rel = []
                for fname, off in ptr_fields:
                    v = getattr(d, fname)
                    if v:
                        b, o = bufs.locate(int(v), f"{plan.names[i]}: bs_gemm_desc.{fname}")
                        rel.append((off, b, o))
                calls += struct.pack("<II", ARG_DESC, len(raw)) + raw + struct.pack("<I", len(rel))
                for off, b, o in rel:
                    calls += struct.pack("<IIq", off, b, o)
# ... 84 lines not shown
```

bodyslam_amd/zoedepth.py:

```python
from __future__ import annotations

import math
import os
import warnings
import dataclasses
from dataclasses import dataclass
from typing import Dict, Optional, Sequence, Tuple

import numpy as np
import torch
import torch.nn.functional as F

from . import _lib as L
from .calibration import DEFAULT_POLICY, NECK_RELHEAD_WONLY, CalibrationPolicy, Scope, choose, finish_report, saving_gflop, worst

LOG2E = 1.4426950408889634


@dataclass
class ZoeConfig:
    hidden: int = 1024
    layers: int = 24
    heads: int = 16
    intermediate: int = 4096
    taps: Tuple[int, ...] = (6, 12, 18, 24)
    image_size: int = 384
    patch: int = 16
    ln_eps: float = 1e-12
    neck_hidden: Tuple[int, ...] = (256, 512, 1024, 1024)
    fusion: int = 256
    rel_features: int = 32
    bottleneck: int = 256
    bin_dim: int = 128
    n_attractors: int = 16
    n_bins: int = 64
    min_temp: float = 0.0212
    max_temp: float = 50.0
    pt_layers: int = 4
    pt_hidden: int = 128
    pt_inter: int = 1024
    pt_heads: int = 4
    head_names: Tuple[str, ...] = ("nyu", "kitti")
    add_projection: bool = True
    level_attractors: Tuple[int, ...] = (16, 8, 4, 1)

    @property
    def single_head(self) -> bool:
        return len(self.head_names) == 1

    @property
    def seed_mlp(self) -> int:
        return 256 if self.single_head else self.bin_dim // 2

    @property
    def proj_mlp(self) -> int:
        return 128 if self.single_head else self.bin_dim // 2

    @property
    def clb_hidden(self) -> int:
        return (self.rel_features + 1 + self.bin_dim) // 2 if self.single_head else (self.rel_features + self.bin_dim) // 4

    def attractors_at(self, level: int) -> int:
        return self.level_attractors[level] if self.single_head else self.n_attractors


BACKBONE_CLASSES = ("qkv", "o", "fc1", "fc2")
ACCURATE_CLASS_MODES = "auto"
AUTO_CANDIDATES = DEFAULT_POLICY.candidates
AUTO_TOL_CLASS_M = DEFAULT_POLICY.tol_class
AUTO_TOL_TOTAL_M = DEFAULT_POLICY.tol_total
AUTO_TOL_ABS_M = DEFAULT_POLICY.tol_abs
TOLERANCE_M = DEFAULT_POLICY.tolerance_m
ACCURATE_ATTN_MODE = "auto"
AUTO_ATTN_RATE_FACTOR = DEFAULT_POLICY.attn_rate_factor
AUTO_NECK_CANDIDATES = DEFAULT_POLICY.neck_candidates
AUTO_TOL_NECK_ABS_M = DEFAULT_POLICY.tol_neck_abs
AUTO_NECK_SITE_MIN_SHARE = DEFAULT_POLICY.neck_site_min_share
AUTO_NECK_SMALL_GROUPS = dict(DEFAULT_POLICY.neck_small_groups)
AUTO_NECK_PLAIN_MIN_SHARE = DEFAULT_POLICY.neck_plain_min_share
AUTO_TOL_NECK_PLAIN_ABS_M = DEFAULT_POLICY.tol_neck_plain_abs
AUTO_NECK_WONLY_INCREMENT_M = DEFAULT_POLICY.neck_wonly_increment
AUTO_NECK_PLAIN_INCREMENT_M = DEFAULT_POLICY.neck_plain_increment
AUTO_TOL_NECK_CAP_M = DEFAULT_POLICY.tol_neck_cap
AUTO_CAL_FRAMES = DEFAULT_POLICY.cal_frames
AUTO_HOLDOUT_FRAMES = DEFAULT_POLICY.holdout_frames
AUTO_TOL_HOLDOUT_M = DEFAULT_POLICY.tol_holdout
AUTO_CAL_SEEDS = DEFAULT_POLICY.cal_seeds
AUTO_HOLDOUT_SEEDS = DEFAULT_POLICY.holdout_seeds
ACCURATE_NECK_MODE = "full"

_CALIBRATION_CACHE: Dict[Tuple, dict] = {}
_ARITHMETIC_SWITCHES = ("BS_UPCONV_FUSED", "BS_NECK_PLAIN", "BS_MLP2", "BS_NECK_BIAS_CORR", "BS_PROJECTOR_LEVEL", "BS_AUTO_WSTAT")

ZOED_NK = ZoeConfig()
ZOED_N = ZoeConfig(head_names=("nyu",))
ZOED_K = ZoeConfig(head_names=("kitti",))


def pad_sizes(h: int, w: int) -> Tuple[int, int]:
    return int(np.sqrt(h / 2) * 3), int(np.sqrt(w / 2) * 3)


def net_size(h: int, w: int, out_hw=(384, 512), multiple: int = 32) -> Tuple[int, int]:
    ph, pw = pad_sizes(h, w)
    hp, wp = h + 2 * ph, w + 2 * pw
    sh, sw = out_hw[0] / hp, out_hw[1] / wp
    if abs(1 - sw) < abs(1 - sh):
        sh = sw
    else:
        sw = sh
    return int(np.round(sh * hp / multiple) * multiple), int(np.round(sw * wp / multiple) * multiple)


def _relative_position_index(wh: int, ww: int) -> torch.Tensor:
    nrd = (2 * wh - 1) * (2 * ww - 1) + 3
    coords = torch.stack(torch.meshgrid(torch.arange(wh), torch.arange(ww), indexing="ij")).flatten(1)
    rel = (coords[:, :, None] - coords[:, None, :]).permute(1, 2, 0).contiguous()
    rel[:, :, 0] += wh - 1
    rel[:, :, 1] += ww - 1
    rel[:, :, 0] *= 2 * ww - 1
    idx = torch.zeros((wh * ww + 1,) * 2, dtype=rel.dtype)
    idx[1:, 1:] = rel.sum(-1)
    idx[0, 0:] = nrd - 3
    idx[0:, 0] = nrd - 2
    idx[0, 0] = nrd - 1
    return idx


class _Measurement:

    def __init__(self, eng: "ZoeDepthEngine", frames_u8: torch.Tensor):
        self.eng, self.frames, self.hold = eng, frames_u8, None
        self.ncal, self.H, self.W = int(frames_u8.shape[0]), int(frames_u8.shape[1]), int(frames_u8.shape[2])
        self.site_flops: Dict[str, float] = {}
        self.ref = self.truth = self.truth_hold = None

    def depth(self, modes, neck, attn, holdout=False, means=None):
        frames = self.hold if holdout else self.frames
        self.eng.set_class_modes(modes, neck, attn)
        plan = _ZoePlan(self.eng, int(frames.shape[0]), self.H, self.W, True)
        plan.frames.copy_(frames)
        plan.run(None if means is None else {"__site_means__": means})
        d = plan.depth_m.clone()
        torch.cuda.synchronize(self.eng.dev)
        self.site_flops.update(plan.site_flops)
        del plan
        return d

    def set_site_bias_corr(self, means):
        e = self.eng
        e.site_bias_corr = {k_[3:]: (e.dw_sum[k_[3:]].double() * m_.double()).sum(1).float().contiguous() for k_, m_ in means.items() if k_[3:] in e.dw_sum}
        e._bias_corr_cache.clear()
        return sorted(e.site_bias_corr)

class ZoeDepthEngine:

    def __init__(self, weights: Dict[str, torch.Tensor], cfg: Optional[ZoeConfig] = None, dtype=torch.float16,
                 device: int = 0, target_hw: Tuple[int, int] = (384, 512), precision: str = "fast",
                 class_modes: Optional[Dict[str, str]] = None, neck_mode: Optional[str] = None, attn_mode: Optional[str] = None):
        L.init(device)
        assert precision in ("fast", "accurate", "reference")
        if precision == "reference":
            class_modes, neck_mode, attn_mode = "pairs", "pairs", "corr"
        self.precision = precision
        self.acc = precision != "fast"
        self._sd = weights if self.acc else None
        self.target_hw = target_hw
        self.cfg = cfg or ZoeConfig()
        assert dtype in (torch.float16, torch.bfloat16)
        self.dtype = dtype
        self.dev = torch.device("cuda", device)
        self.w: Dict[str, torch.Tensor] = {}
        self._bias_cache: Dict[Tuple[int, int], list] = {}
        self._plans: Dict[Tuple, "_ZoePlan"] = {}
        self._raw_tables = []
# ... 724 lines not shown
                P.gemm(f"ro{i}.tok", t16, w[f"ro{i}.w_tok"], r16, M=NB * T0, N=Hd, K=Hd * np3, lda=Hd * m2, conv=(1, S, Hd * m2, 1, T0, 1, 1, 1, 0, -1),
                       seg1=Hd if acc else 0, bias=cb, bias_group_rows=T0, act=L.ACT_GELU, ldo=Hd * m2, out_split_off=Hd if acc else 0,
                       precision_passes=np3)
            pr = e16(NB * T0, ch * m2)
            nplain(f"ra{i}.proj", r16, f"ra{i}.proj.w", pr, NB * T0, ch, Hd, bias=w[f"ra{i}.proj.b"])
            if i == 0 or i == 1:
                s_ = 4 if i == 0 else 2
                up = e16(NB, hp * s_, wp * s_, ch * m2)
                nplain(f"ra{i}.up", pr, f"ra{i}.up.w", up, NB * T0, s_ * s_ * ch, ch, shuffle=(s_, ch, hp, wp), bias=w[f"ra{i}.up.b"])
                free(pr)
                fh, fw, src = hp * s_, wp * s_, up
            elif i == 2:
                fh, fw, src = hp, wp, pr
            else:
                fh, fw = (hp + 2 - 3) // 2 + 1, (wp + 2 - 3) // 2 + 1
                src = e16(NB, fh, fw, ch * m2)
                nconv(f"ra{i}.down", pr, f"ra{i}.down.w", src, hp, wp, ch, ch, stride=2, bias=w[f"ra{i}.down.b"])
                free(pr)
            P.mark(f"reassemble{i}", src, ("nhwc", NB, fh, fw, ch, self.mfmt()))
            f16_ = e16(NB, fh, fw, c.fusion * m2)
            nconv(f"nc{i}", src, f"nc{i}.w", f16_, fh, fw, ch, c.fusion)
            free(src)
            P.mark(f"neckconv{i}", f16_, ("nhwc", NB, fh, fw, c.fusion, self.mfmt()))
            feats.append(f16_)
            fshape.append((fh, fw))
        free(r16, cb)
        return feats, fshape

    def _bins_seed(self, bott, bh_, bw_):
        c, w, P, NB, acc, m2, np3, dev = self.c, self.w, self.plan, self.NB, self.acc, self.m2, self.np3, self.eng.dev
        e16, e32 = self.e16, self.e32
        Mb = NB * bh_ * bw_
        xb = e16(Mb, c.bottleneck * m2)
        self.nplain("mh.conv2", bott, "mh.conv2.w", xb, Mb, c.bottleneck, c.bottleneck, bias=w["mh.conv2.b"], out8=False)
        self.logits = torch.empty(NB, 4, device=dev, dtype=torch.float32)
        self.route = torch.zeros(NB, dtype=torch.int32, device=dev)
        if not c.single_head:
            self._router(xb, bh_, bw_)
        E, nb, SM, PM, KB = c.bin_dim, c.n_bins, c.seed_mlp, c.proj_mlp, c.bottleneck
        sh = e16(Mb, 2 * SM * m2)
        P.gemm("seed.c1", xb, w["seed.c1.w"], sh, M=Mb, N=2 * SM, K=KB * np3, lda=KB * m2, seg1=KB if acc else 0, bias=w["seed.c1.b"], act=L.ACT_RELU,
               ldo=2 * SM * m2, out_split_off=2 * SM if acc else 0, precision_passes=np3)
        bins = e32(NB, bh_, bw_, 2 * nb)
        P.gemm("seed.c2", sh, w["seed.c2.w"], bins, M=Mb, N=2 * nb, K=2 * SM * np3, lda=2 * SM * m2, seg1=2 * SM if acc else 0, bias=w["seed.c2.b"],
               act=L.ACT_SOFTPLUS, precision_passes=np3)
        shp = e16(Mb, PM)
        P.gemm("seedproj.c1", xb, w["seedproj.c1.w"], shp, M=Mb, N=PM, K=KB, lda=KB * m2, bias=w["seedproj.c1.b"], act=L.ACT_RELU)
        emb = e16(Mb, E * m2)
        P.gemm("seedproj.c2", shp, w["seedproj.c2.w"], emb, M=Mb, N=E, K=PM, lda=PM, bias=w["seedproj.c2.b"],
               ldo=E * m2, out_split_off=E if acc else 0)
        return bins, emb

    def _router(self, xb, bh_, bw_):
        c, w, P, NB, e16, e32 = self.c, self.w, self.plan, self.NB, self.e16, self.e32
        D, St, Mb = c.pt_hidden, bh_ * bw_ + 1, NB * bh_ * bw_
        pos = torch.arange(0, St, dtype=torch.float32).unsqueeze(1)
        div = torch.exp(torch.arange(0, D, 2, dtype=torch.float32).unsqueeze(0) * (-torch.log(torch.full((), 10000.0)) / D))
        pe_tab = torch.cat([torch.sin(pos * div), torch.cos(pos * div)], dim=1).to(self.eng.dev)
        pe_src = pe_tab.unsqueeze(0).expand(NB, St, D).contiguous().view(NB * St, D)
        e32b = e32(NB * St, D)
        e16b = e16(NB * St, D)
        P.add("rt.init", "bs_copy_f32", pe_src, e32b, e32b.numel())
        P.gemm("rt.emb", xb, w["rt.emb.w"], e32b, M=Mb, N=D, K=c.bottleneck, lda=c.bottleneck * self.m2, bias=w["rt.emb.b"], res=e32b, ldr=D,
               out_group=(bh_ * bw_, St, 1))
        P.add("rt.cast", "bs_cast", e32b, e16b, e32b.numel(), L.dt(e16b))
        qkv32 = e32(NB * St, 3 * D)
        at16 = e16(NB * St, D)
        tmp32 = e32(NB * St, D)
        h16 = e16(NB * St, c.pt_inter)
        for l in range(c.pt_layers):
            P.gemm(f"rt{l}.qkv", e16b, w[f"rt{l}.qkv.w"], qkv32, M=NB * St, N=3 * D, K=D, lda=D, bias=w[f"rt{l}.qkv.b"])
            P.add(f"rt{l}.attn", "bs_small_attention", qkv32, at16, NB, St, c.pt_heads, L.dt(at16))
            P.gemm(f"rt{l}.o", at16, w[f"rt{l}.o.w"], tmp32, M=NB * St, N=D, K=D, lda=D, bias=w[f"rt{l}.o.b"], res=e32b, ldr=D)
            P.add(f"rt{l}.n1", "bs_layernorm", tmp32, w[f"rt{l}.n1.g"], w[f"rt{l}.n1.b"], e16b, e32b, NB * St, D, 1e-5, L.dt(e16b))
            P.gemm(f"rt{l}.l1", e16b, w[f"rt{l}.l1.w"], h16, M=NB * St, N=c.pt_inter, K=D, lda=D, bias=w[f"rt{l}.l1.b"], act=L.ACT_RELU)
            P.gemm(f"rt{l}.l2", h16, w[f"rt{l}.l2.w"], tmp32, M=NB * St, N=D, K=c.pt_inter, lda=c.pt_inter, bias=w[f"rt{l}.l2.b"], res=e32b, ldr=D)
            P.add(f"rt{l}.n2", "bs_layernorm", tmp32, w[f"rt{l}.n2.g"], w[f"rt{l}.n2.b"], e16b, e32b, NB * St, D, 1e-5, L.dt(e16b))
        c1 = e16(NB, D)
        P.gemm("cl.l1", e16b, w["cl.l1.w"], c1, M=NB, N=D, K=D, lda=St * D, bias=w["cl.l1.b"], act=L.ACT_RELU)
        P.gemm("cl.l2", c1, w["cl.l2.w"], self.logits, M=NB, N=4, K=D, lda=D, bias=w["cl.l2.b"])
        P.add("route", "bs_route_argmax", self.logits, 4, self.route, NB)
        P.mark("logits", self.logits, ("raw",))

    def res_unit(self, name, xin, hh, ww, other=None):
        w, P, NB, Fc, nf8, e16, free, nconv = self.w, self.plan, self.NB, self.c.fusion, self.nf8, self.e16, self.pool.free, self.nconv
        t = e16(NB, hh, ww, Fc * self.m2)
        y = e16(NB, hh, ww, Fc * self.m2)
        if self.acc:
            xr = e16(NB, hh, ww, Fc * self.m2)
            P.add(name + ".relu", "bs_relu_split", xin, xr, NB * hh * ww, Fc, L.dt(xr) | (32 if nf8 else 0) | (64 if self.lo8_rows(name + ".c1.w") else 0) | (128 if self.hi8_rows(name + ".c1.w") else 0))
            nconv(name + ".c1", xr, name + ".c1.w", t, hh, ww, Fc, Fc, bias=w[name + ".c1.b"], act=L.ACT_RELU, out_lo8_rows=self.lo8_rows(name + ".c2.w"),
                  out_planes_rows=self.hi8_rows(name + ".c2.w"))
            free(xr)
        else:
            nconv(name + ".c1", xin, name + ".c1.w", t, hh, ww, Fc, Fc, relu_a=True, bias=w[name + ".c1.b"], act=L.ACT_RELU)
        nconv(name + ".c2", t, name + ".c2.w", y, hh, ww, Fc, Fc, bias=w[name + ".c2.b"], res=xin, res2=other)
        free(t)
        return y

    def _fusion(self, feats, fshape):
        w, P, eng, NB, m2, Fc, PM = self.w, self.plan, self.eng, self.NB, self.m2, self.c.fusion, self.c.proj_mlp
        e16, free, nplain = self.e16, self.pool.free, self.nplain
        rh_in = "rh.projection.w" if eng.add_projection else "rh.conv1.w"
        pj_low, fused_list = [], []
        fused = None
        for li in range(4):
            feat = feats[3 - li]
            fh, fw = fshape[3 - li]
            if fused is None:
                cur = feat
            else:
                cur = self.res_unit(f"fu{li}.r1", feat, fh, fw, other=fused)
                free(feat)
                free(fused)
            cur_in = cur
            cur = self.res_unit(f"fu{li}.r2", cur, fh, fw)
            if fused is not None:
                free(cur_in)
            lowp = e16(NB, fh, fw, Fc * m2)
            nplain(f"fu{li}.proj", cur, f"fu{li}.proj.w", lowp, NB * fh * fw, Fc, Fc, bias=w[f"fu{li}.proj.b"])
            free(cur)
            z = e16(NB * fh * fw, PM * m2)
            nplain(f"pj{li}.c1", lowp, f"pj{li}.c1.w", z, NB * fh * fw, PM, Fc, out8=False)
            pj_low.append((z, fh, fw))
            fused = e16(NB, 2 * fh, 2 * fw, Fc * m2)
            nolo = bool(li == 3 and self.lo8_rows(rh_in))
            nopl = bool(nolo and self.hi8_rows(rh_in))
            P.add(f"fu{li}.up", "bs_resize_bilinear_nhwc", lowp, fused, NB, fh, fw, Fc, 2 * fh, 2 * fw, self.RZ | (8 if nolo else 0) | (16 if nopl else 0), L.dt(fused))
            free(lowp)
            P.mark(f"fused{li}", fused, ("nhwc", NB, 2 * fh, 2 * fw, Fc, 3 if nolo else self.mfmt()))
            fused_list.append((fused, 2 * fh, 2 * fw))
        return fused_list, pj_low

    def _relative_head(self, f3, h3, w3):
        c, w, P, eng, NB, acc, m2, nf8, Fc = self.c, self.w, self.plan, self.eng, self.NB, self.acc, self.m2, self.nf8, self.c.fusion
        e16, free, nconv = self.e16, self.pool.free, self.nconv
        if eng.add_projection:
            rp = e16(NB, h3, w3, Fc * m2)
            nconv("rh.projection", f3, "rh.projection.w", rp, h3, w3, Fc, Fc, bias=w["rh.projection.b"], act=L.ACT_RELU, out_lo8_rows=self.lo8_rows("rh.conv1.w"))
            free(f3)
        else:
            rp = f3
        r1 = e16(NB, h3, w3, (Fc // 2) * m2)
        nconv("rh.conv1", rp, "rh.conv1.w", r1, h3, w3, Fc, Fc // 2, bias=w["rh.conv1.b"], out_lo8_rows=self.lo8_rows("rh.conv2.w"))
        free(rp)
        fused_up = (os.environ.get("BS_UPCONV_FUSED", "1") != "0" and Fc // 2 == 128 and c.rel_features == 32
                    and ((not acc) or (nf8 and "rh.conv2.w" in eng.f8s)))
        if fused_up:
            last = e16(NB, 2 * h3, 2 * w3, c.rel_features * m2)
            if acc:
                umode, usc = (1 if eng.neck_site_wonly("rh.conv2.w") else 2), self.f8_scales("rh.conv2.w")
                self.site_flops["rh.conv2.w"] = 2.0 * NB * h3 * w3 * 9 * c.rel_features * (Fc // 2)
            else:
                umode, usc = 0, (127, 127, 127, 127)
            P.add("rh.conv2", "bs_upconv_fused", r1, w["rh.conv2.w"], w["rh.conv2.b"], last, NB, h3, w3, Fc // 2, c.rel_features, 2 * h3, 2 * w3,
                  self.RZ, 1, umode, *usc, L.dt(last))
            f_low = 2.0 * NB * h3 * w3 * 9 * c.rel_features * (Fc // 2)
            P.tag_stack(4.0 * f_low, f_low * (1.0, 1.5, 2.0)[umode])
            free(r1)
        else:
            y9 = self.e32(NB, h3, w3, 9 * c.rel_features)
            self.nplain("rh.conv2", r1, "rh.conv2.w", y9, NB * h3 * w3, 9 * c.rel_features, Fc // 2, out_pairs=False, tile=2)
            free(r1)
            last = e16(NB, 2 * h3, 2 * w3, c.rel_features * m2)
            P.add("rh.tapsum", "bs_upconv_tapsum", y9, w["rh.conv2.b"], last, NB, h3, w3, c.rel_features, 2 * h3, 2 * w3, self.RZ, 1, L.dt(last))
            free(y9)
        P.mark("rel_features", last, ("nhwc", NB, 2 * h3, 2 * w3, c.rel_features, self.mfmt()))
        return last

    def _projector_level_fits(self, fused_list, pj_low):
        c, w, eng = self.c, self.w, self.eng
        return (os.environ.get("BS_PROJECTOR_LEVEL", "1") != "0" and self.acc and c.proj_mlp == 64 and c.bin_dim == 128
                and 2 * c.clb_hidden <= 80 and (2 * c.clb_hidden) % 16 == 0 and eng.fuse_mlp
                and all(fw_ % 32 == 0 and 2 * zw_ == fw_ and 2 * zh_ == fh_ for (_, fh_, fw_), (_, zh_, zw_) in zip(fused_list, pj_low))
                and all(tuple(w[f"at{i_}.c1.w"].shape) == (256, 128) and 2 * eng.na_eff[i_] <= 32 for i_ in range(4)))

    def _attractor_step(self, i, A, bins_prev, ph_, pw_, fh, fw):
        NB, nb = self.NB, self.c.n_bins
        bins = self.e32(NB, fh, fw, 2 * nb)
        self.plan.add(f"at{i}.step", "bs_attractor_step", A, bins_prev, bins, self.route, NB, ph_, pw_, fh, fw, 2, nb, self.eng.na_eff[i])
        self.pool.free(A, bins_prev)
        self.plan.mark(f"bins{i}", bins, ("nhwc_route", NB, fh, fw, 2 * nb))
        return bins

    def _levels_fused(self, fused_list, pj_low, bins_prev, emb_prev, ph_, pw_):
        c, w, P, eng, NB, m2 = self.c, self.w, self.plan, self.eng, self.NB, self.m2
        e16, e32, free = self.e16, self.e32, self.pool.free
        E, PM, HID = c.bin_dim, c.proj_mlp, c.clb_hidden
        Eh = None
        for i in range(4):
            _, fh, fw = fused_list[i]
            Mi = NB * fh * fw
            z, zh, zw = pj_low[i]
            assert (zh, zw) == (ph_, pw_), "the projector's low-resolution map and the previous level's embedding share a grid"
            last_lv = i == 3
            x16 = e16(Mi, E)
            emb = None if last_lv else e16(Mi, E * m2)
            if last_lv:
                Eh = e32(Mi, 2 * HID)
            P.add(f"pj{i}.level", "bs_projector_level", z, w[f"pj{i}.c1.b"], emb_prev, w[f"pj{i}.c2.w"], w[f"pj{i}.c2.b"],
                  w["clb.e1.w"] if last_lv else None, w["clb.e1.b"] if last_lv else None, x16, emb, Eh, NB, zh, zw, fh, fw, PM, E, 2 * HID,
                  L.dt(x16))
            f_alg = 2.0 * Mi * PM * (E + (2 * HID if last_lv else 0))
            P.tag_stack(f_alg, 3.0 * f_alg)
            free(z, emb_prev)
            na = eng.na_eff[i]
            A = e32(Mi, 2 * na)
# ... 73 lines not shown
```

include/bodyslam_hip.h:

```cpp
#ifndef BODYSLAM_HIP_H
#define BODYSLAM_HIP_H

#include <stdint.h>

#ifdef __cplusplus
extern "C" {
#endif

typedef enum {
    BS_OK = 0,
    BS_ERR_INVALID = -1,
    BS_ERR_HIP = -2,
    BS_ERR_NOT_INIT = -3
} bs_status;

enum { BS_F32 = 0, BS_F16 = 1, BS_BF16 = 2, BS_F64 = 3  };
enum { BS_ACT_NONE = 0, BS_ACT_RELU = 1, BS_ACT_GELU = 2, BS_ACT_SOFTPLUS = 3, BS_ACT_SOFTPLUS_FAST = 4 };
enum { BS_OUT_PLAIN = 0, BS_OUT_SHUFFLE = 1, BS_OUT_QKV = 2 };

int bs_init(int device);
const char* bs_last_error(void);
int bs_version(void);

#define BS_F8_ACT_HI_EXP 0
#define BS_F8_ACT_LO_EXP 11
typedef struct bs_gemm_desc {
    const void* A;
    const void* W;
    int32_t dtype;
    int32_t M, N, K;
    int32_t lda;
    int32_t conv;
    int32_t Hin, Win, Cin, Hout, Wout, KH, KW, stride, pad_h, pad_w;
    int32_t relu_a;
    const float* bias;
    int32_t bias_group_rows;
    int32_t act;
    const float* scale;
    const void* res;
    int32_t res_dtype;
    int32_t ldr;
    const void* res2;
    void* out;
    void* out2;
    void* out3;
    int32_t out_dtype;
    int32_t ldo;
    int32_t out_mode;
    int32_t out_group_rows, out_group_stride, out_row_offset;
    int32_t shuffle_s, shuffle_cout;
    int32_t qkv_hidden, qkv_tokens, qkv_sp;
    float q_scale;
    int32_t tile;
    int32_t seg1;
    int32_t out_split_off;
    int32_t res_split_off;
    int32_t f8_seg;
    uint32_t f8_scales;
    int32_t out_f8;
    int32_t res_f8;
    int32_t qkv_cls_last;
    int32_t qkv_cls_rows;
    int32_t qkv_patch_row0;
    int32_t f8_wonly_from;
    int32_t out_lo8_rows;
    int32_t f8_skip_from;
    int32_t bias2_row0;
    int32_t bias2_group_rows;
    int32_t out_planes_rows;
    const float* bias2;
    int32_t qkv_lo_off;
    int32_t out2_relu;
} bs_gemm_desc;
int bs_gemm(const bs_gemm_desc* d, void* stream);
int bs_gemm_tile(const bs_gemm_desc* d);

int bs_col_mean(const void* A, int64_t lda, int32_t row0, int32_t rows_per_group, int32_t groups, int32_t row_step, int32_t K,
                void* out_bf16, float* zero_out, int64_t zero_n, int32_t dtype, void* stream);
int bs_rank1_bias(const void* abar_bf16, const void* dw_bf16, float* out, int32_t G, int32_t N, int32_t K, void* stream);

int bs_attention(const void* q, const void* k, const void* vt, const float* bias, void* out,
                 int32_t B, int32_t nh, int32_t S, int32_t Sp, int32_t dtype, void* stream);
int bs_attention_table(const void* q, const void* k, const void* vt, const float* table, void* out,
                       int32_t B, int32_t nh, int32_t hp, int32_t wp, int32_t Sp, int32_t grouped, int32_t dtype, void* stream);
int bs_attention_table_corr(const void* q, const void* k, const void* vt, const void* q_lo, const void* k_lo, const void* vt_lo,
                            const float* table, void* out, int32_t B, int32_t nh, int32_t hp, int32_t wp, int32_t Sp, int32_t grouped,
                            int32_t dtype, void* stream);

int bs_layernorm(const float* x, const float* gamma, const float* beta, void* out16, float* out32, int32_t rows,
                 int32_t cols, float eps, int32_t dtype, void* stream);

int bs_copy_f32(const float* src, float* dst, int64_t n, void* stream);

int bs_cast_split(const float* x, void* out, int64_t rows, int32_t cols, int32_t out_dtype, void* stream);
int bs_relu_split(const void* x, void* out, int64_t rows, int32_t cols, int32_t dtype, void* stream);

int bs_cast(const float* x, void* out, int64_t n, int32_t out_dtype, void* stream);

int bs_preprocess_patches(const uint8_t* frames, void* out, int32_t B, int32_t H, int32_t W, int32_t nh,
                          int32_t nw, int32_t flip, int32_t out_dtype, void* stream);
int bs_preprocess_image(const uint8_t* frames, float* out, int32_t B, int32_t H, int32_t W, int32_t nh,
                        int32_t nw, int32_t flip, void* stream);

int bs_fill_rows(float* x, const float* v, int32_t B, int32_t rows_per_image, int32_t cols, void* stream);

int bs_resize_bilinear_nhwc(const void* x, void* out, int32_t B, int32_t Hin, int32_t Win, int32_t C,
                            int32_t Hout, int32_t Wout, int32_t align_corners, int32_t dtype, void* stream);

int bs_resize_bias_relu_nhwc(const void* x, const float* bias, void* out, int32_t B, int32_t Hin, int32_t Win, int32_t C, int32_t Hout,
                             int32_t Wout, int32_t flags, int32_t dtype, void* stream);

int bs_upconv_tapsum(const float* y, const float* bias, void* out, int32_t B, int32_t Hin, int32_t Win, int32_t Cout,
                     int32_t Hout, int32_t Wout, int32_t align_corners, int32_t relu, int32_t dtype, void* stream);

int bs_upconv_fused(const void* x, const void* w, const float* bias, void* out, int32_t B, int32_t Hin, int32_t Win, int32_t Cin,
                    int32_t Cout, int32_t Hout, int32_t Wout, int32_t flags, int32_t relu, int32_t mode, int32_t sa0, int32_t sb0,
                    int32_t sa1, int32_t sb1, int32_t dtype, void* stream);

int bs_attractor_step(const float* A, const float* bins_prev, float* bins_out, const int32_t* route, int32_t B,
                      int32_t Hp, int32_t Wp, int32_t H, int32_t W, int32_t groups, int32_t n_bins, int32_t n_attr,
                      void* stream);
int bs_mlp2(const void* x, int32_t ldx, const void* W1, const float* b1, const void* W2, const float* b2, float* out, int32_t M,
            int32_t K1, int32_t N1, int32_t N2, int32_t act2, int32_t dtype, void* stream);
int bs_mlp2_add(const void* emb, const void* prev, const void* W1, const float* b1, const void* W2, const float* b2, float* out,
                int32_t B, int32_t Hp, int32_t Wp, int32_t H, int32_t W, int32_t K1, int32_t N1, int32_t N2, int32_t act2, int32_t dtype,
                void* stream);
int bs_projector_level(const void* z, const float* b_c1, const void* emb_prev, const void* Wc2, const float* b_c2, const void* We,
                       const float* b_e, void* x_out, void* emb_out, float* eh_out, int32_t B, int32_t Hl, int32_t Wl, int32_t H, int32_t W,
                       int32_t PM, int32_t E, int32_t NE, int32_t dtype, void* stream);
int bs_add_resized(const void* x, const void* prev, void* out, int32_t B, int32_t Hp, int32_t Wp, int32_t H,
                   int32_t W, int32_t C, int32_t dtype, void* stream);
int bs_logbinom_depth(const void* last, const float* Eh, const float* bins, const float* w0_last, const float* w2,
                      const float* b2, const int32_t* route, float* depth, int32_t B, int32_t H, int32_t W,
                      int32_t He, int32_t We, float min_temp, float max_temp, int32_t dtype, void* stream);
int bs_logbinom_depth_ex(const void* last, const float* Eh, const float* bins, const float* w0_last, const float* w2,
                         const float* b2, const float* rel_w, int32_t hid, const int32_t* route, float* depth, int32_t B,
                         int32_t H, int32_t W, int32_t He, int32_t We, float min_temp, float max_temp, int32_t dtype,
                         void* stream);
int bs_small_attention(const float* qkv, void* out, int32_t B, int32_t S, int32_t nheads, int32_t dtype, void* stream);
int bs_route_argmax(const float* logits, int32_t ld, int32_t* route, int32_t B, void* stream);

int bs_postprocess_depth(const float* depth_net, float* depth_m, uint16_t* depth_u16, int32_t B, int32_t H,
                         int32_t W, int32_t nh, int32_t nw, int32_t flip, void* stream);

int bs_cyclepose_im2col(const uint8_t* frames, const int32_t* pairs, void* out, int32_t P, int32_t H, int32_t W,
                        int32_t dtype, void* stream);
int bs_cyclepose_im2col_window(const uint8_t* frames, const int32_t* pairs, void* out, int32_t P, int32_t H, int32_t W,
                               int32_t top, int32_t left, int32_t CH, int32_t CW, int32_t dtype, void* stream);
int bs_instnorm_relu_nhwc(const float* x, void* out, float* out_f32, float* scratch, int32_t P, int32_t HW, int32_t C,
                          float eps, int32_t dtype, void* stream);
int bs_avgpool_nhwc(const float* x, float* out, int32_t P, int32_t HW, int32_t C, void* stream);
int bs_cyclepose_head(const float* pooled, const float* x2, const float* w_skip_pool, const float* w_skip_x2,
                      const float* b_skip, const float* w1, const float* b1, const float* w2, const float* b2,
                      float* pose7, float* T, float* scratch , int32_t P,
                      int32_t HW, int32_t C, void* stream);
// ... 172 lines not shown
```

Measured before the change: 496.4.

## Fuse bilinear 2x upsample of previous fusion level into residual-unit conv epilogue

```diff
diff --git a/bodyslam_amd/_lib.py b/bodyslam_amd/_lib.py
--- a/bodyslam_amd/_lib.py
+++ b/bodyslam_amd/_lib.py
@@ -42,6 +42,7 @@
         ("f8_skip_from", C.c_int32), ("bias2_row0", C.c_int32), ("bias2_group_rows", C.c_int32), ("out_planes_rows", C.c_int32),
         ("bias2", C.c_void_p),
         ("qkv_lo_off", C.c_int32), ("out2_relu", C.c_int32),
+        ("res2_up", C.c_void_p), ("res2_up_hin", C.c_int32), ("res2_up_win", C.c_int32), ("res2_up_hout", C.c_int32), ("res2_up_wout", C.c_int32),
     ]
 
 
@@ -226,7 +227,7 @@
                    shuffle=None, qkv=None, a_offset: int = 0, tile: int = 0, seg1: int = 0, out_split_off: int = 0,
                    res_split_off: int = 0, f8_seg: int = 0, f8_scales=(127, 127, 127, 127), out_f8=None, res_f8: bool = False,
                    f8_wonly_from: int = 0, out_lo8_rows: int = 0, f8_skip_from: int = 0, bias2=None, out_planes_rows: int = 0,
-                   out_relu: Optional[torch.Tensor] = None) -> GemmDesc:
+                   out_relu: Optional[torch.Tensor] = None, res2_up=None) -> GemmDesc:
     d = GemmDesc()
     d.A = A.data_ptr() + a_offset * A.element_size()
     d.W = W.data_ptr()
@@ -252,6 +253,11 @@
     if res2 is not None:
         assert res is not None and res2.dtype == A.dtype
         d.res2 = res2.data_ptr()
+    if res2_up is not None:
+        low, hin, win, hout, wout = res2_up
+        assert res2 is None and low.dtype == A.dtype and (res is not None or ldr)
+        d.res2_up, d.res2_up_hin, d.res2_up_win, d.res2_up_hout, d.res2_up_wout = low.data_ptr(), hin, win, hout, wout
+        d.ldr = ldr if ldr else N
     d.out = out.data_ptr()
     d.out_dtype = dt(out)
     d.ldo = N if ldo is None else ldo
@@ -291,7 +297,25 @@
     return d
 
 
+def _res2_up_two_launches(kw):
+    tile = kw.get("tile", 0)
+    if kw.get("res2_up") is None or not (tile // 100) & 4096:
+        return None
+    low, hin, win, hout, wout = kw["res2_up"]
+    N, f8 = kw["N"], bool(kw.get("res_f8"))
+    nb = kw["M"] // (hout * wout)
+    fused = torch.empty(nb, hout, wout, N * (2 if f8 else 1), dtype=low.dtype, device=low.device)
+    kw = {k: v for k, v in kw.items() if k != "res2_up"}
+    kw["tile"] = tile % 100 + 100 * ((tile // 100) & ~4096)
+    kw["res2" if kw.get("res") is not None else "res"] = fused
+    return (low, fused, nb, hin, win, N, hout, wout, 1 | (4 if f8 else 0), dt(low)), kw
+
+
 def gemm(A: torch.Tensor, W: torch.Tensor, out: torch.Tensor, **kw) -> None:
+    two = _res2_up_two_launches(kw)
+    if two is not None:
+        rz, kw = two
+        check(load_library().bs_resize_bilinear_nhwc(*[p(a) if isinstance(a, torch.Tensor) else a for a in rz], stream_ptr()), "bs_resize_bilinear_nhwc")
     d = make_gemm_desc(A, W, out, **kw)
     check(load_library().bs_gemm(C.byref(d), stream_ptr()), "bs_gemm")
 
@@ -314,6 +338,8 @@
     r_lo = min(r_lo, r_planes)
     out = d.N * (r_lo * per_row[0] + (r_planes - r_lo) * per_row[1] + (full - r_planes) * per_row[2])
     res = float(d.M) * d.N * (4 if (d.res and d.res_dtype == F32) else 0)
+    if d.res2_up:
+        res += float(d.M // (d.res2_up_hout * d.res2_up_wout)) * d.res2_up_hin * d.res2_up_win * d.N * (3 if d.res_f8 else 2)
     return a + w + out + res
 
 
@@ -326,12 +352,17 @@
         self.keep = []
         self.keep_descs = []
         self.marks = {}
+        self.lazy_marks = {}
         self.gemm_info = {}
         self.stack_info = {}
         self.events = None
         self._graph = None
 
     def gemm(self, name, A, W, out, **kw):
+        two = _res2_up_two_launches(kw)
+        if two is not None:
+            rz, kw = two
+            self.add(name + ".up", "bs_resize_bilinear_nhwc", *rz)
         passes = kw.pop("precision_passes", 1)
         d = make_gemm_desc(A, W, out, **kw)
         kw["precision_passes"] = passes
@@ -362,6 +393,9 @@
 
     def mark(self, name, tensor, meta=None):
         self.marks.setdefault(len(self.calls), []).append((name, tensor, meta))
+
+    def mark_lazy(self, name, make, meta=None):
+        self.lazy_marks.setdefault(len(self.calls), []).append((name, make, meta))
 
     def run_timed(self, events: list):
         stream = torch.cuda.current_stream(self.device)
@@ -415,6 +449,9 @@
                     continue
                 if means is None:
                     taps[name] = (t.clone(), meta)
+            if means is None:
+                for (name, make, meta) in self.lazy_marks.get(i, []):
+                    taps[name] = (make(st), meta)
             if i < len(self.calls):
                 fn, args = self.calls[i]
                 check(fn(*args, st), self.names[i])
diff --git a/bodyslam_amd/csrc/common.h b/bodyslam_amd/csrc/common.h
--- a/bodyslam_amd/csrc/common.h
+++ b/bodyslam_amd/csrc/common.h
@@ -176,6 +176,83 @@
 }
 constexpr int F8_ACT_HI_EXP = BS_F8_ACT_HI_EXP, F8_ACT_LO_EXP = BS_F8_ACT_LO_EXP;
 
+typedef int i32x2_ __attribute__((ext_vector_type(2)));
+__device__ __forceinline__ void resize_src(int o, int nin, float s, int align, int& i0, int& i1, float& l) {
+    const float f = align ? s * (float)o : fmaxf(__fmaf_rn(s, (float)o + 0.5f, -0.5f), 0.0f);
+    i0 = (int)f;
+    i0 = i0 > nin - 1 ? nin - 1 : i0;
+    i1 = i0 + (i0 < nin - 1 ? 1 : 0);
+    l = f - (float)i0;
+}
+static inline float resize_scale(int nin, int nout, int align) {
+    if (align) return nout > 1 ? (float)(nin - 1) / (float)(nout - 1) : 0.f;
+    return (float)nin / (float)nout;
+}
+template <typename T, bool F8>
+__device__ __forceinline__ void resize_decode8(typename T16<T>::v8 h, i32x2_ l, float (&q)[8]) {
+#pragma unroll
+    for (int e = 0; e < 8; ++e) q[e] = (float)h[e];
+    if (F8) {
+        const float sc = __builtin_ldexpf(1.0f, -F8_ACT_LO_EXP);
+        float l0[4], l1[4];
+        f8_unpack4(l[0], l0);
+        f8_unpack4(l[1], l1);
+#pragma unroll
+        for (int e = 0; e < 4; ++e) {
+            q[e] = fmaf(l0[e], sc, q[e]);
+            q[4 + e] = fmaf(l1[e], sc, q[4 + e]);
+        }
+    }
+}
+__device__ __forceinline__ void resize_lerp_x8(const float (&q0)[8], const float (&q1)[8], float lx, float (&r)[8]) {
+    const float hx = 1.0f - lx;
+    const f32x2_ hx2 = {hx, hx}, lx2 = {lx, lx};
+#pragma unroll
+    for (int e = 0; e < 8; e += 2) {
+        const f32x2_ t = __builtin_elementwise_fma(lx2, f32x2_{q1[e], q1[e + 1]}, hx2 * f32x2_{q0[e], q0[e + 1]});
+        r[e] = t[0];
+        r[e + 1] = t[1];
+    }
+}
+__device__ __forceinline__ void resize_lerp_y8(const float (&top)[8], const float (&bot)[8], float ly, float (&v)[8]) {
+    const float hy = 1.0f - ly;
+    const f32x2_ hy2 = {hy, hy}, ly2 = {ly, ly};
+#pragma unroll
+    for (int e = 0; e < 8; e += 2) {
+        const f32x2_ t = __builtin_elementwise_fma(ly2, f32x2_{bot[e], bot[e + 1]}, hy2 * f32x2_{top[e], top[e + 1]});
+        v[e] = t[0];
+        v[e + 1] = t[1];
+    }
+}
+__device__ __forceinline__ void resize_lerp8(const float (&q00)[8], const float (&q01)[8], const float (&q10)[8], const float (&q11)[8], float lx,
+                                             float ly, float (&v)[8]) {
+    float top[8], bot[8];
+    resize_lerp_x8(q00, q01, lx, top);
+    resize_lerp_x8(q10, q11, lx, bot);
+    resize_lerp_y8(top, bot, ly, v);
+}
+template <typename T, bool LO>
+__device__ __forceinline__ void resize_split8(const float (&v)[8], typename T16<T>::v8& hi, i32x2_& lo) {
+#pragma unroll
+    for (int e = 0; e < 8; ++e) hi[e] = T16<T>::from_f32(v[e]);
+    if (LO) {
+        const float sl = __builtin_ldexpf(1.0f, F8_ACT_LO_EXP);
+        lo = i32x2_{f8_pack4((v[0] - (float)hi[0]) * sl, (v[1] - (float)hi[1]) * sl, (v[2] - (float)hi[2]) * sl, (v[3] - (float)hi[3]) * sl),
+                    f8_pack4((v[4] - (float)hi[4]) * sl, (v[5] - (float)hi[5]) * sl, (v[6] - (float)hi[6]) * sl, (v[7] - (float)hi[7]) * sl)};
+    }
+}
+template <typename T, bool F8, bool LO = F8>
+__device__ __forceinline__ void resize_piece8(const typename T16<T>::v8 (&ch)[4], const i32x2_ (&cl)[4], float lx, float ly, float (&v)[8],
+                                              typename T16<T>::v8& hi, i32x2_& lo) {
+    float q00[8], q01[8], q10[8], q11[8];
+    resize_decode8<T, F8>(ch[0], cl[0], q00);
+    resize_decode8<T, F8>(ch[1], cl[1], q01);
+    resize_decode8<T, F8>(ch[2], cl[2], q10);
+    resize_decode8<T, F8>(ch[3], cl[3], q11);
+    resize_lerp8(q00, q01, q10, q11, lx, ly, v);
+    resize_split8<T, LO>(v, hi, lo);
+}
+
 __device__ __forceinline__ void glds16(const void* gptr, void* lds_wave_base) {
     __builtin_amdgcn_global_load_lds((const __attribute__((address_space(1))) void*)gptr,
                                      (__attribute__((address_space(3))) void*)lds_wave_base, 16, 0, 0);
diff --git a/bodyslam_amd/csrc/elementwise.hip b/bodyslam_amd/csrc/elementwise.hip
--- a/bodyslam_amd/csrc/elementwise.hip
+++ b/bodyslam_amd/csrc/elementwise.hip
@@ -250,72 +250,45 @@
     const int c16 = idx % c16n, ox = idx / c16n;
     const int b = blockIdx.y / Hout, oy = blockIdx.y - b * Hout;
     const int64_t pix = ((int64_t)b * Hout + oy) * Wout + ox;
-    float fy, fx;
-    if (align) {
-        fy = sy * (float)oy;
-        fx = sx * (float)ox;
-    } else {
-        fy = fmaxf(__fmaf_rn(sy, (float)oy + 0.5f, -0.5f), 0.0f);
-        fx = fmaxf(__fmaf_rn(sx, (float)ox + 0.5f, -0.5f), 0.0f);
-    }
-    int y0 = (int)fy, x0 = (int)fx;
-    y0 = y0 > Hin - 1 ? Hin - 1 : y0;
-    x0 = x0 > Win - 1 ? Win - 1 : x0;
-    const int y1 = y0 + (y0 < Hin - 1 ? 1 : 0), x1 = x0 + (x0 < Win - 1 ? 1 : 0);
-    const float ly = fy - (float)y0, lx = fx - (float)x0, hy = 1.0f - ly, hx = 1.0f - lx;
+    int y0, y1, x0, x1;
+    float ly, lx;
+    resize_src(oy, Hin, sy, align, y0, y1, ly);
+    resize_src(ox, Win, sx, align, x0, x1, lx);
     typedef typename T16<T>::v8 v8;
     typedef int i32x4 __attribute__((ext_vector_type(4)));
     const T* xb = x + (int64_t)b * Hin * Win * C * 2;
-    const float sc = __builtin_ldexpf(1.0f, -F8_ACT_LO_EXP);
-    float q00[16], q01[16], q10[16], q11[16];
-    auto ld = [&](int yy, int xx, float (&q)[16]) {
-        const T* pp = xb + ((int64_t)yy * Win + xx) * C * 2;
-        const v8 h0 = *reinterpret_cast<const v8*>(pp + c16 * 16), h1 = *reinterpret_cast<const v8*>(pp + c16 * 16 + 8);
+    const int64_t cpix[4] = {(int64_t)y0 * Win + x0, (int64_t)y0 * Win + x1, (int64_t)y1 * Win + x0, (int64_t)y1 * Win + x1};
+    v8 ch[2][4];
+    i32x2_ cl[2][4];
+#pragma unroll
+    for (int k = 0; k < 4; ++k) {
+        const T* pp = xb + cpix[k] * C * 2;
+        ch[0][k] = *reinterpret_cast<const v8*>(pp + c16 * 16);
+        ch[1][k] = *reinterpret_cast<const v8*>(pp + c16 * 16 + 8);
         const i32x4 l = *reinterpret_cast<const i32x4*>(reinterpret_cast<const char*>(pp + C + (C >> 1)) + c16 * 16);
-#pragma unroll
-        for (int e = 0; e < 8; ++e) {
-            q[e] = (float)h0[e];
-            q[8 + e] = (float)h1[e];
-        }
-#pragma unroll
-        for (int g = 0; g < 4; ++g) {
-            float lo[4];
-            f8_unpack4(l[g], lo);
-#pragma unroll
-            for (int e = 0; e < 4; ++e) q[4 * g + e] = fmaf(lo[e], sc, q[4 * g + e]);
-        }
-    };
-    ld(y0, x0, q00);
-    ld(y0, x1, q01);
-    ld(y1, x0, q10);
-    ld(y1, x1, q11);
-    v8 o0, o1;
-    float vv[16], rl[16];
-    const f32x2_ hx2 = {hx, hx}, lx2 = {lx, lx}, hy2 = {hy, hy}, ly2 = {ly, ly};
-#pragma unroll
-    for (int e = 0; e < 16; e += 2) {
-        const f32x2_ v2 = bilerp2(f32x2_{q00[e], q00[e + 1]}, f32x2_{q01[e], q01[e + 1]}, f32x2_{q10[e], q10[e + 1]}, f32x2_{q11[e], q11[e + 1]}, hx2, lx2, hy2, ly2);
-#pragma unroll
-        for (int u = 0; u < 2; ++u) {
-            const float v = v2[u];
-            vv[e + u] = v;
-            const T h = T16<T>::from_f32(v);
-            if (e + u < 8) o0[e + u] = h; else o1[e + u - 8] = h;
-            if (LO) rl[e + u] = v - (float)h;
-        }
+        cl[0][k] = i32x2_{l[0], l[1]};
+        cl[1][k] = i32x2_{l[2], l[3]};
+    }
+    v8 o[2];
+    i32x2_ plo[2];
+    float vv[16];
+#pragma unroll
+    for (int g = 0; g < 2; ++g) {
+        float v[8];
+        resize_piece8<T, true, LO>(ch[g], cl[g], lx, ly, v, o[g], plo[g]);
+#pragma unroll
+        for (int e = 0; e < 8; ++e) vv[8 * g + e] = v[e];
     }
     T* op = out + pix * C * 2;
-    *reinterpret_cast<v8*>(op + c16 * 16) = o0;
-    *reinterpret_cast<v8*>(op + c16 * 16 + 8) = o1;
+    *reinterpret_cast<v8*>(op + c16 * 16) = o[0];
+    *reinterpret_cast<v8*>(op + c16 * 16 + 8) = o[1];
     if (!HI8) return;
-    const float sh = __builtin_ldexpf(1.0f, F8_ACT_HI_EXP), sl = __builtin_ldexpf(1.0f, F8_ACT_LO_EXP);
+    const float sh = __builtin_ldexpf(1.0f, F8_ACT_HI_EXP);
     char* planes = reinterpret_cast<char*>(op + C);
     i32x4 ph, pl;
 #pragma unroll
-    for (int g = 0; g < 4; ++g) {
-        ph[g] = f8_pack4(vv[4 * g] * sh, vv[4 * g + 1] * sh, vv[4 * g + 2] * sh, vv[4 * g + 3] * sh);
-        if (LO) pl[g] = f8_pack4(rl[4 * g] * sl, rl[4 * g + 1] * sl, rl[4 * g + 2] * sl, rl[4 * g + 3] * sl);
-    }
+    for (int g = 0; g < 4; ++g) ph[g] = f8_pack4(vv[4 * g] * sh, vv[4 * g + 1] * sh, vv[4 * g + 2] * sh, vv[4 * g + 3] * sh);
+    if (LO) pl = i32x4{plo[0][0], plo[0][1], plo[1][0], plo[1][1]};
     *reinterpret_cast<i32x4*>(planes + c16 * 16) = ph;
     if (LO) *reinterpret_cast<i32x4*>(planes + C + c16 * 16) = pl;
 }
@@ -533,43 +506,25 @@
     const int c8 = idx % c8n, ox = idx / c8n;
     const int b = blockIdx.y / Hout, oy = blockIdx.y - b * Hout;
     const int64_t pix = ((int64_t)b * Hout + oy) * Wout + ox;
-    float fy, fx;
-    if (align) {
-        fy = sy * (float)oy;
-        fx = sx * (float)ox;
-    } else {
-        fy = fmaxf(__fmaf_rn(sy, (float)oy + 0.5f, -0.5f), 0.0f);
-        fx = fmaxf(__fmaf_rn(sx, (float)ox + 0.5f, -0.5f), 0.0f);
-    }
-    int y0 = (int)fy, x0 = (int)fx;
-    y0 = y0 > Hin - 1 ? Hin - 1 : y0;
-    x0 = x0 > Win - 1 ? Win - 1 : x0;
-    const int y1 = y0 + (y0 < Hin - 1 ? 1 : 0), x1 = x0 + (x0 < Win - 1 ? 1 : 0);
-    const float ly = fy - (float)y0, lx = fx - (float)x0, hy = 1.0f - ly, hx = 1.0f - lx;
+    int y0, y1, x0, x1;
+    float ly, lx;
+    resize_src(oy, Hin, sy, align, y0, y1, ly);
+    resize_src(ox, Win, sx, align, x0, x1, lx);
     typedef typename T16<T>::v8 v8;
     constexpr int PS = SPLIT ? 2 : 1;
     const T* xb = x + (int64_t)b * Hin * Win * C * PS + c8 * 8;
     float q00[8], q01[8], q10[8], q11[8], av[8];
     auto ld = [&](const T* ptr, float (&dst)[8]) {
         const v8 h = *reinterpret_cast<const v8*>(ptr);
-#pragma unroll
-        for (int e = 0; e < 8; ++e) dst[e] = (float)h[e];
+        if (SPLIT == 2) {
+            resize_decode8<T, true>(h, *reinterpret_cast<const i32x2_*>(reinterpret_cast<const char*>(ptr - c8 * 8 + C + (C >> 1)) + c8 * 8), dst);
+            return;
+        }
+        resize_decode8<T, false>(h, i32x2_{0, 0}, dst);
         if (SPLIT == 1) {
             const v8 l = *reinterpret_cast<const v8*>(ptr + C);
 #pragma unroll
             for (int e = 0; e < 8; ++e) dst[e] += (float)l[e];
-        } else if (SPLIT == 2) {
-            const char* lo8 = reinterpret_cast<const char*>(ptr - c8 * 8 + C + (C >> 1)) + c8 * 8;
-            const int p0 = *reinterpret_cast<const int*>(lo8), p1 = *reinterpret_cast<const int*>(lo8 + 4);
-            float l0[4], l1[4];
-            f8_unpack4(p0, l0);
-            f8_unpack4(p1, l1);
-            const float sc = __builtin_ldexpf(1.0f, -F8_ACT_LO_EXP);
-#pragma unroll
-            for (int e = 0; e < 4; ++e) {
-                dst[e] = fmaf(l0[e], sc, dst[e]);
-                dst[4 + e] = fmaf(l1[e], sc, dst[4 + e]);
-            }
         }
     };
     ld(xb + ((int64_t)y0 * Win + x0) * C * PS, q00);
@@ -578,34 +533,27 @@
     ld(xb + ((int64_t)y1 * Win + x1) * C * PS, q11);
     if (ADD) ld(addend + pix * C * PS + c8 * 8, av);
     v8 o, ol;
+    i32x2_ plo;
     float vv[8];
-    const f32x2_ hx2 = {hx, hx}, lx2 = {lx, lx}, hy2 = {hy, hy}, ly2 = {ly, ly};
-#pragma unroll
-    for (int e = 0; e < 8; e += 2) {
-        f32x2_ v = bilerp2(f32x2_{q00[e], q00[e + 1]}, f32x2_{q01[e], q01[e + 1]}, f32x2_{q10[e], q10[e + 1]}, f32x2_{q11[e], q11[e + 1]}, hx2, lx2, hy2, ly2);
-        if (ADD) v += f32x2_{av[e], av[e + 1]};
-        if (BIAS_RELU) {
-            v += *reinterpret_cast<const f32x2_*>(bias + c8 * 8 + e);
-            v = f32x2_{fmaxf(v[0], 0.0f), fmaxf(v[1], 0.0f)};
-        }
-#pragma unroll
-        for (int u = 0; u < 2; ++u) {
-            vv[e + u] = v[u];
-            o[e + u] = T16<T>::from_f32(v[u]);
-            if (SPLIT == 1) ol[e + u] = T16<T>::from_f32(v[u] - (float)o[e + u]);
-        }
-    }
+    resize_lerp8(q00, q01, q10, q11, lx, ly, vv);
+#pragma unroll
+    for (int e = 0; e < 8; ++e) {
+        if (ADD) vv[e] += av[e];
+        if (BIAS_RELU) vv[e] = fmaxf(vv[e] + bias[c8 * 8 + e], 0.0f);
+    }
+    resize_split8<T, SPLIT == 2>(vv, o, plo);
     *reinterpret_cast<v8*>(out + pix * C * PS + c8 * 8) = o;
-    if (SPLIT == 1) *reinterpret_cast<v8*>(out + pix * C * PS + C + c8 * 8) = ol;
+    if (SPLIT == 1) {
+#pragma unroll
+        for (int e = 0; e < 8; ++e) ol[e] = T16<T>::from_f32(vv[e] - (float)o[e]);
+        *reinterpret_cast<v8*>(out + pix * C * PS + C + c8 * 8) = ol;
+    }
     if (SPLIT == 2) {
-        const float sh = __builtin_ldexpf(1.0f, F8_ACT_HI_EXP), sl = __builtin_ldexpf(1.0f, F8_ACT_LO_EXP);
+        const float sh = __builtin_ldexpf(1.0f, F8_ACT_HI_EXP);
         char* planes = reinterpret_cast<char*>(out + pix * C * 2 + C);
-        typedef int i32x2 __attribute__((ext_vector_type(2)));
-        *reinterpret_cast<i32x2*>(planes + c8 * 8) = i32x2{f8_pack4(vv[0] * sh, vv[1] * sh, vv[2] * sh, vv[3] * sh),
-                                                           f8_pack4(vv[4] * sh, vv[5] * sh, vv[6] * sh, vv[7] * sh)};
-        *reinterpret_cast<i32x2*>(planes + C + c8 * 8) =
-            i32x2{f8_pack4((vv[0] - (float)o[0]) * sl, (vv[1] - (float)o[1]) * sl, (vv[2] - (float)o[2]) * sl, (vv[3] - (float)o[3]) * sl),
-                  f8_pack4((vv[4] - (float)o[4]) * sl, (vv[5] - (float)o[5]) * sl, (vv[6] - (float)o[6]) * sl, (vv[7] - (float)o[7]) * sl)};
+        *reinterpret_cast<i32x2_*>(planes + c8 * 8) = i32x2_{f8_pack4(vv[0] * sh, vv[1] * sh, vv[2] * sh, vv[3] * sh),
+                                                            f8_pack4(vv[4] * sh, vv[5] * sh, vv[6] * sh, vv[7] * sh)};
+        *reinterpret_cast<i32x2_*>(planes + C + c8 * 8) = plo;
     }
 }
 
@@ -758,14 +706,7 @@
 template <typename T>
 static int launch_resize(const void* x, const void* addend, void* out, int B, int Hin, int Win, int C, int Hout, int Wout, int align,
                          hipStream_t st, int split = 0) {
-    float sy, sx;
-    if (align) {
-        sy = Hout > 1 ? (float)(Hin - 1) / (float)(Hout - 1) : 0.f;
-        sx = Wout > 1 ? (float)(Win - 1) / (float)(Wout - 1) : 0.f;
-    } else {
-        sy = (float)Hin / (float)Hout;
-        sx = (float)Win / (float)Wout;
-    }
+    const float sy = resize_scale(Hin, Hout, align), sx = resize_scale(Win, Wout, align);
     const dim3 blocks(cdiv(Wout * (C / 8), 256), B * Hout);
     if (split >= 2 && split <= 4) {
         const dim3 blocks16(cdiv(Wout * (C / 16), 256), B * Hout);
diff --git a/bodyslam_amd/csrc/engine.hip b/bodyslam_amd/csrc/engine.hip
--- a/bodyslam_amd/csrc/engine.hip
+++ b/bodyslam_amd/csrc/engine.hip
@@ -14,7 +14,7 @@
 
 namespace {
 
-constexpr char kMagic[8] = {'B', 'S', 'E', 'N', 'G', '0', '2', '\0'};
+constexpr char kMagic[8] = {'B', 'S', 'E', 'N', 'G', '0', '3', '\0'};
 enum { KIND_WORKSPACE = 0, KIND_ZERO = 1, KIND_DATA = 2 };
 enum { ARG_I64 = 0, ARG_F64 = 1, ARG_PTR = 2, ARG_NULL = 3, ARG_DESC = 4 };
 enum { OP_CALL = 0, OP_SIGNAL = 1, OP_WAIT = 2 };
diff --git a/bodyslam_amd/csrc/igemm.hip b/bodyslam_amd/csrc/igemm.hip
--- a/bodyslam_amd/csrc/igemm.hip
+++ b/bodyslam_amd/csrc/igemm.hip
@@ -156,7 +156,8 @@
     p.f8_sa0 = d->f8_scales & 0xff; p.f8_sb0 = (d->f8_scales >> 8) & 0xff; p.f8_sa1 = (d->f8_scales >> 16) & 0xff; p.f8_sb1 = d->f8_scales >> 24;
     p.out_f8 = d->out_f8;
     p.res_f8 = d->res_f8;
-    BS_REQUIRE(!d->res_f8 || (d->res && d->res_dtype == d->dtype && d->res_split_off == 0 && d->ldr >= 2 * d->N && d->N % 8 == 0), "bs_gemm: res_f8 needs a 16-bit residual in (hi16 | hi8 | lo8) rows, ldr >= 2N");
+    BS_REQUIRE(!d->res_f8 || ((d->res ? d->res_dtype == d->dtype : d->res2_up != nullptr) && d->res_split_off == 0 && d->ldr >= 2 * d->N && d->N % 8 == 0),
+               "bs_gemm: res_f8 needs a 16-bit residual in (hi16 | hi8 | lo8) rows, ldr >= 2N");
     BS_REQUIRE(d->f8_seg >= 0 && d->f8_seg % 256 == 0, "bs_gemm: f8_seg=%d must be a multiple of 256 (two halves of whole 128-byte stages)", d->f8_seg);
     BS_REQUIRE(d->f8_seg == 0 || (d->seg1 == 0 && !d->relu_a), "bs_gemm: the FP8 segment excludes seg1 and relu_a");
     p.f8_stages = d->f8_seg / 128;
@@ -197,6 +198,20 @@
     p.bias = d->bias; p.bias_group_rows = d->bias_group_rows; p.act = d->act; p.scale = d->scale;
     p.res = d->res; p.res2 = d->res2; p.res_dtype = d->res_dtype; p.ldr = d->ldr;
     BS_REQUIRE(!d->res2 || d->res, "bs_gemm: res2 needs res (they share ldr)");
+    p.res2_up = d->res2_up;
+    if (d->res2_up) {
+        BS_REQUIRE(!d->res2 && d->out_mode == BS_OUT_PLAIN && !d->out_group_rows && d->res_split_off == 0 && d->N % 8 == 0 && d->ldr % 8 == 0 &&
+                       d->ldr >= (d->res_f8 ? 2 : 1) * d->N && (!d->res || d->res_dtype == d->dtype),
+                   "bs_gemm: res2_up excludes res2 and needs a plain output, N %% 8 == 0, ldr %% 8 == 0 and 16-bit or (hi16 | hi8 | lo8) residual rows");
+        BS_REQUIRE(d->res2_up_hin > 0 && d->res2_up_win > 0 && d->res2_up_hout > 0 && d->res2_up_wout > 0 &&
+                       d->M % (d->res2_up_hout * d->res2_up_wout) == 0,
+                   "bs_gemm: res2_up needs the map's sizes, M a multiple of res2_up_hout * res2_up_wout");
+        p.up_hin = d->res2_up_hin; p.up_win = d->res2_up_win; p.up_hout = d->res2_up_hout; p.up_wout = d->res2_up_wout;
+        p.up_sy = resize_scale(d->res2_up_hin, d->res2_up_hout, 1);
+        p.up_sx = resize_scale(d->res2_up_win, d->res2_up_wout, 1);
+        up_magic((unsigned)d->res2_up_wout, p.up_wmagic, p.up_wshift);
+        up_magic((unsigned)d->res2_up_hout, p.up_hmagic, p.up_hshift);
+    }
     p.out = d->out; p.out2 = d->out2; p.out3 = d->out3; p.out_dtype = d->out_dtype; p.ldo = d->ldo; p.out_mode = d->out_mode;
     p.out_group_rows = d->out_group_rows; p.out_group_stride = d->out_group_stride; p.out_row_offset = d->out_row_offset;
     p.shuffle_s = d->shuffle_s; p.shuffle_cout = d->shuffle_cout;
@@ -208,7 +223,7 @@
     p.out2_relu = d->out2_relu;
     BS_REQUIRE(!d->out2_relu || (d->out2 && d->out_mode == BS_OUT_PLAIN && d->out_f8 && !d->scale && !d->out_group_rows && !d->bias_group_rows &&
                                  !d->bias2 && (d->act == BS_ACT_NONE || d->act == BS_ACT_RELU) && d->out_split_off == d->N && d->N % 256 == 0 &&
-                                 d->ldo % 8 == 0 && d->out_dtype == d->dtype && (!d->res || d->res_f8)),
+                                 d->ldo % 8 == 0 && d->out_dtype == d->dtype && ((!d->res && !d->res2_up) || d->res_f8)),
                "bs_gemm: out2_relu needs the plain (hi16 | hi8 | lo8) output form (out_f8, N %% 256 == 0, no scale / row groups / bias2)");
     BS_REQUIRE(d->qkv_lo_off == 0 || (d->out_mode == BS_OUT_QKV && d->qkv_lo_off > 0 && d->qkv_lo_off % 8 == 0),
                "bs_gemm: qkv_lo_off needs BS_OUT_QKV and a multiple of 8 elements");
diff --git a/bodyslam_amd/csrc/igemm_kernel.h b/bodyslam_amd/csrc/igemm_kernel.h
--- a/bodyslam_amd/csrc/igemm_kernel.h
+++ b/bodyslam_amd/csrc/igemm_kernel.h
@@ -23,6 +23,10 @@
     const float* scale;
     const void* res;
     const void* res2;
+    const void* res2_up;
+    int up_hin, up_win, up_hout, up_wout;
+    float up_sy, up_sx;
+    unsigned up_wmagic, up_wshift, up_hmagic, up_hshift;
     int res_dtype, ldr;
     void* out;
     void* out2;
@@ -166,6 +170,37 @@
     y[0] += a[0] * sc; y[1] += a[1] * sc; y[2] += b[0] * sc; y[3] += b[1] * sc;
 }
 
+static inline void up_magic(unsigned d, unsigned& magic, unsigned& shift) {
+    shift = 0;
+    while ((1ull << shift) < d) ++shift;
+    magic = (unsigned)((((1ull << shift) - d) << 32) / d + 1);
+}
+__device__ __forceinline__ void up_row(const IgemmParams& p, int m, int64_t (&c)[4], float& lx, float& ly) {
+    const unsigned r = (__umulhi((unsigned)m, p.up_wmagic) + (unsigned)m) >> p.up_wshift, ox = (unsigned)m - r * (unsigned)p.up_wout;
+    const unsigned b = (__umulhi(r, p.up_hmagic) + r) >> p.up_hshift, oy = r - b * (unsigned)p.up_hout;
+    int y0, y1, x0, x1;
+    resize_src((int)oy, p.up_hin, p.up_sy, 1, y0, y1, ly);
+    resize_src((int)ox, p.up_win, p.up_sx, 1, x0, x1, lx);
+    const int64_t r0 = ((int64_t)b * p.up_hin + y0) * p.up_win, r1 = ((int64_t)b * p.up_hin + y1) * p.up_win;
+    c[0] = (r0 + x0) * p.ldr;
+    c[1] = (r0 + x1) * p.ldr;
+    c[2] = (r1 + x0) * p.ldr;
+    c[3] = (r1 + x1) * p.ldr;
+}
+template <typename T, bool F8>
+__device__ __forceinline__ void add_piece8(float (&y8)[8], typename T16<T>::v8 hv, i32x2_ lv) {
+    const float lsc = __builtin_ldexpf(1.0f, -BS_F8_ACT_LO_EXP);
+#pragma unroll
+    for (int h = 0; h < 2; ++h) {
+#pragma unroll
+        for (int e = 0; e < 4; ++e) y8[4 * h + e] += T16<T>::to_f32(hv[4 * h + e]);
+        if (F8) {
+            const f32x2_ a = __builtin_amdgcn_cvt_pk_f32_fp8(lv[h], false), b = __builtin_amdgcn_cvt_pk_f32_fp8(lv[h], true);
+            y8[4 * h] += a[0] * lsc; y8[4 * h + 1] += a[1] * lsc; y8[4 * h + 2] += b[0] * lsc; y8[4 * h + 3] += b[1] * lsc;
+        }
+    }
+}
+
 constexpr int NW_CHECK(int a, int b) { return a * b; }
 
 template <int N>
@@ -664,7 +699,7 @@
         }
     }
     if (!v_tile) {
-        auto epi = [&](auto act_tag) {
+        auto epi = [&](auto act_tag) __attribute__((always_inline)) {
             constexpr int ACT = decltype(act_tag)::value;
             BS_FRESH_LANE
             f32x4 bj[FN], sj[FN];
@@ -790,6 +825,37 @@
                             }
                         }
                     }
+                    if (p.res2_up && n0j[jp * 2] < p.N) {
+                        int64_t c[4];
+                        float lx, ly;
+                        up_row(p, m, c, lx, ly);
+                        const bool f8r = F8 && p.res_f8;
+                        float rowv[2][8], v[8];
+#pragma unroll
+                        for (int r = 0; r < 2; ++r) {
+                            float q[2][8];
+#pragma unroll
+                            for (int k = 0; k < 2; ++k) {
+                                const T* rp = reinterpret_cast<const T*>(p.res2_up) + c[2 * r + k];
+                                const v8 h = *reinterpret_cast<const v8*>(rp + n0j[jp * 2]);
+                                if (f8r) resize_decode8<T, true>(h, *reinterpret_cast<const i32x2_*>(reinterpret_cast<const char*>(rp + p.N + (p.N >> 1)) + n0j[jp * 2]), q[k]);
+                                else resize_decode8<T, false>(h, i32x2_{0, 0}, q[k]);
+                            }
+                            resize_lerp_x8(q[0], q[1], lx, rowv[r]);
+                            __builtin_amdgcn_sched_barrier(0);
+                        }
+                        resize_lerp_y8(rowv[0], rowv[1], ly, v);
+                        v8 hv;
+                        i32x2_ lv = {};
+                        if (f8r) {
+                            resize_split8<T, true>(v, hv, lv);
+                            add_piece8<T, true>(y8, hv, lv);
+                        } else {
+                            resize_split8<T, false>(v, hv, lv);
+                            add_piece8<T, false>(y8, hv, lv);
+                        }
+                        __builtin_amdgcn_sched_barrier(0);
+                    }
                 }
 #pragma unroll
                 for (int jp = 0; jp < FN / 2; ++jp) {
@@ -866,11 +932,11 @@
             if (p.out_mode == BS_OUT_PLAIN && !p.out_group_rows && !p.bias_group_rows && p.N % BN == 0 && p.ldo % 8 == 0 && !b2_rows &&
                 !(p.ablate & (16 | 2048)) && p.out_f8 && !p.scale && (p.act == BS_ACT_NONE || p.act == BS_ACT_RELU) && p.split_off == p.N &&
                 p.N % 8 == 0 && p.out_dtype != BS_F32 &&
-                (!p.res || (p.res_f8 && p.res_dtype != BS_F32 && p.res_split_off == 0 && p.ldr % 8 == 0)) && (!p.res2 || p.res)) {
+                (!p.res || (p.res_f8 && p.res_dtype != BS_F32 && p.res_split_off == 0 && p.ldr % 8 == 0)) && (!p.res2 || p.res) &&
+                (!p.res2_up || (p.res_f8 && p.ldr % 8 == 0))) {
                 BS_FRESH_LANE
                 typedef typename T16<T>::v8 v8;
-                typedef int i32x2 __attribute__((ext_vector_type(2)));
-                typedef float f32x2 __attribute__((ext_vector_type(2)));
+                typedef i32x2_ i32x2;
                 constexpr int NP = FM * (FN / 2), RDEPTH = 4;
                 f32x4 bj[FN];
 #pragma unroll
@@ -884,11 +950,29 @@
                 const int ea = p.out_f8 & 0xff, el = (p.out_f8 >> 8) & 0xff;
                 const bool lo_plane = !(p.out_lo8_rows > 0 && m0 >= p.out_lo8_rows);
                 const bool hi_plane = !(p.out_planes_rows > 0 && m0 >= p.out_planes_rows);
-                const float lsc = __builtin_ldexpf(1.0f, -BS_F8_ACT_LO_EXP);
-                auto body = [&](auto nres_tag) {
+                auto body = [&](auto nres_tag, auto up_tag) __attribute__((always_inline)) {
                     constexpr int NRES = decltype(nres_tag)::value;
-                    v8 rh[NRES ? RDEPTH : 1][NRES ? NRES : 1];
-                    i32x2 rl[NRES ? RDEPTH : 1][NRES ? NRES : 1];
+                    constexpr bool UP = decltype(up_tag)::value;
+                    constexpr int UDEPTH = 1, RD = RDEPTH;
+                    v8 rh[NRES ? RD : 1][NRES ? NRES : 1];
+                    i32x2 rl[NRES ? RD : 1][NRES ? NRES : 1];
+                    v8 uh[UP ? UDEPTH : 1][4];
+                    i32x2_ ul[UP ? UDEPTH : 1][4];
+                    float ulx[UP ? UDEPTH : 1], uly[UP ? UDEPTH : 1];
+                    auto issue_up = [&](int it, int slot) {
+                        const int i = it / (FN / 2), jp = it - i * (FN / 2);
+                        int m = mrow + i * 16;
+                        m = m < p.M ? m : p.M - 1;
+                        const int n = n_wave + jp * 32 + fq * 8;
+                        int64_t c[4];
+                        up_row(p, m, c, ulx[slot], uly[slot]);
+#pragma unroll
+                        for (int k = 0; k < 4; ++k) {
+                            const T* rp = reinterpret_cast<const T*>(p.res2_up) + c[k];
+                            uh[slot][k] = *reinterpret_cast<const v8*>(rp + n);
+                            ul[slot][k] = *reinterpret_cast<const i32x2_*>(reinterpret_cast<const char*>(rp + p.N + (p.N >> 1)) + n);
+                        }
+                    };
                     auto issue = [&](int it, int slot) {
                         const int i = it / (FN / 2), jp = it - i * (FN / 2);
                         int m = mrow + i * 16;
@@ -903,7 +987,11 @@
                     };
                     if constexpr (NRES > 0) {
 #pragma unroll
-                        for (int it = 0; it < RDEPTH; ++it) issue(it, it);
+                        for (int it = 0; it < RD; ++it) issue(it, it);
+                    }
+                    if constexpr (UP) {
+#pragma unroll
+                        for (int it = 0; it < UDEPTH; ++it) issue_up(it, it);
                     }
 #pragma unroll
                     for (int it = 0; it < NP; ++it) {
@@ -920,19 +1008,18 @@
                             }
                         if constexpr (NRES > 0) {
 #pragma unroll
-                            for (int q = 0; q < NRES; ++q) {
-                                const v8 hv = rh[it % RDEPTH][q];
-                                const i32x2 lv = rl[it % RDEPTH][q];
-#pragma unroll
-                                for (int h = 0; h < 2; ++h) {
-#pragma unroll
-                                    for (int e = 0; e < 4; ++e) y8[4 * h + e] += T16<T>::to_f32(hv[4 * h + e]);
-                                    const f32x2 a = __builtin_amdgcn_cvt_pk_f32_fp8(lv[h], false), b = __builtin_amdgcn_cvt_pk_f32_fp8(lv[h], true);
-                                    y8[4 * h] += a[0] * lsc; y8[4 * h + 1] += a[1] * lsc; y8[4 * h + 2] += b[0] * lsc; y8[4 * h + 3] += b[1] * lsc;
-                                }
-                            }
-                            if (it + RDEPTH < NP) issue(it + RDEPTH, it % RDEPTH);
-                        }
+                            for (int q = 0; q < NRES; ++q) add_piece8<T, true>(y8, rh[it % RD][q], rl[it % RD][q]);
+                            if (it + RD < NP) issue(it + RD, it % RD);
+                        }
+                        if constexpr (UP) {
+                            float v[8];
+                            v8 hv;
+                            i32x2_ lv;
+                            resize_piece8<T, true>(uh[it % UDEPTH], ul[it % UDEPTH], ulx[it % UDEPTH], uly[it % UDEPTH], v, hv, lv);
+                            add_piece8<T, true>(y8, hv, lv);
+                            if (it + UDEPTH < NP) issue_up(it + UDEPTH, it % UDEPTH);
+                        }
+                        if constexpr (UP) __builtin_amdgcn_sched_barrier(0);
                         if (m < p.M) store8_f8<T>(p.out, (int64_t)m * p.ldo, n_wave + jp * 32 + fq * 8, p.split_off, y8, ea, el, lo_plane && hi_plane, hi_plane);
                         if (p.out2_relu) {
 #pragma unroll
@@ -941,9 +1028,11 @@
                         }
                     }
                 };
-                if (p.res2) body(std::integral_constant<int, 2>{});
-                else if (p.res) body(std::integral_constant<int, 1>{});
-                else body(std::integral_constant<int, 0>{});
+                if (p.res2_up && p.res) body(std::integral_constant<int, 1>{}, std::true_type{});
+                else if (p.res2_up) body(std::integral_constant<int, 0>{}, std::true_type{});
+                else if (p.res2) body(std::integral_constant<int, 2>{}, std::false_type{});
+                else if (p.res) body(std::integral_constant<int, 1>{}, std::false_type{});
+                else body(std::integral_constant<int, 0>{}, std::false_type{});
                 return;
             }
             if (plain_full && p.act == BS_ACT_GELU && !p.res && p.out_f8 && !p.scale && p.split_off == p.N && p.N % 8 == 0) {
diff --git a/bodyslam_amd/engine_export.py b/bodyslam_amd/engine_export.py
--- a/bodyslam_amd/engine_export.py
+++ b/bodyslam_amd/engine_export.py
@@ -9,7 +9,7 @@
 
 from . import _lib as L
 
-MAGIC = b"BSENG02\0"
+MAGIC = b"BSENG03\0"
 KIND_WORKSPACE, KIND_ZERO, KIND_DATA = 0, 1, 2
 ARG_I64, ARG_F64, ARG_PTR, ARG_NULL, ARG_DESC = 0, 1, 2, 3, 4
 OP_CALL = 0
diff --git a/bodyslam_amd/zoedepth.py b/bodyslam_amd/zoedepth.py
--- a/bodyslam_amd/zoedepth.py
+++ b/bodyslam_amd/zoedepth.py
@@ -90,7 +90,7 @@
 ACCURATE_NECK_MODE = "full"
 
 _CALIBRATION_CACHE: Dict[Tuple, dict] = {}
-_ARITHMETIC_SWITCHES = ("BS_UPCONV_FUSED", "BS_NECK_PLAIN", "BS_MLP2", "BS_NECK_BIAS_CORR", "BS_PROJECTOR_LEVEL", "BS_AUTO_WSTAT")
+_ARITHMETIC_SWITCHES = ("BS_UPCONV_FUSED", "BS_FUSED_RES_UP", "BS_NECK_PLAIN", "BS_MLP2", "BS_NECK_BIAS_CORR", "BS_PROJECTOR_LEVEL", "BS_AUTO_WSTAT")
 
 ZOED_NK = ZoeConfig()
 ZOED_N = ZoeConfig(head_names=("nyu",))
@@ -981,7 +981,7 @@
         P.add("route", "bs_route_argmax", self.logits, 4, self.route, NB)
         P.mark("logits", self.logits, ("raw",))
 
-    def res_unit(self, name, xin, hh, ww, other=None):
+    def res_unit(self, name, xin, hh, ww, other=None, other_up=None):
         w, P, NB, Fc, nf8, e16, free, nconv = self.w, self.plan, self.NB, self.c.fusion, self.nf8, self.e16, self.pool.free, self.nconv
         t = e16(NB, hh, ww, Fc * self.m2)
         y = e16(NB, hh, ww, Fc * self.m2)
@@ -993,7 +993,11 @@
             free(xr)
         else:
             nconv(name + ".c1", xin, name + ".c1.w", t, hh, ww, Fc, Fc, relu_a=True, bias=w[name + ".c1.b"], act=L.ACT_RELU)
-        nconv(name + ".c2", t, name + ".c2.w", y, hh, ww, Fc, Fc, bias=w[name + ".c2.b"], res=xin, res2=other)
+        if other_up is not None:
+            low, lh, lw = other_up
+            nconv(name + ".c2", t, name + ".c2.w", y, hh, ww, Fc, Fc, bias=w[name + ".c2.b"], res=xin, res2_up=(low, lh, lw, hh, ww))
+        else:
+            nconv(name + ".c2", t, name + ".c2.w", y, hh, ww, Fc, Fc, bias=w[name + ".c2.b"], res=xin, res2=other)
         free(t)
         return y
 
@@ -1003,18 +1007,25 @@
         rh_in = "rh.projection.w" if eng.add_projection else "rh.conv1.w"
         pj_low, fused_list = [], []
         fused = None
+        res_up = os.environ.get("BS_FUSED_RES_UP", "1") != "0"
+        low_prev = None
         for li in range(4):
             feat = feats[3 - li]
             fh, fw = fshape[3 - li]
-            if fused is None:
+            if li == 0:
                 cur = feat
+            elif low_prev is not None:
+                assert (2 * low_prev[1], 2 * low_prev[2]) == (fh, fw)
+                cur = self.res_unit(f"fu{li}.r1", feat, fh, fw, other_up=low_prev)
+                free(feat)
+                free(low_prev[0])
             else:
                 cur = self.res_unit(f"fu{li}.r1", feat, fh, fw, other=fused)
                 free(feat)
                 free(fused)
             cur_in = cur
             cur = self.res_unit(f"fu{li}.r2", cur, fh, fw)
-            if fused is not None:
+            if li > 0:
                 free(cur_in)
             lowp = e16(NB, fh, fw, Fc * m2)
             nplain(f"fu{li}.proj", cur, f"fu{li}.proj.w", lowp, NB * fh * fw, Fc, Fc, bias=w[f"fu{li}.proj.b"])
@@ -1022,6 +1033,18 @@
             z = e16(NB * fh * fw, PM * m2)
             nplain(f"pj{li}.c1", lowp, f"pj{li}.c1.w", z, NB * fh * fw, PM, Fc, out8=False)
             pj_low.append((z, fh, fw))
+            if li < 3 and res_up and ((not self.acc) or (self.nf8 and f"fu{li + 1}.r1.c2.w" in eng.f8s)):
+                low_prev, fused = (lowp, fh, fw), None
+
+                def make(st, lowp=lowp, fh=fh, fw=fw):
+                    t = torch.empty(NB, 2 * fh, 2 * fw, Fc * m2, device=lowp.device, dtype=lowp.dtype)
+                    L.check(L.load_library().bs_resize_bilinear_nhwc(lowp.data_ptr(), t.data_ptr(), NB, fh, fw, Fc, 2 * fh, 2 * fw, self.RZ, L.dt(t), st),
+                            "bs_resize_bilinear_nhwc")
+                    return t
+                P.mark_lazy(f"fused{li}", make, ("nhwc", NB, 2 * fh, 2 * fw, Fc, self.mfmt()))
+                fused_list.append((None, 2 * fh, 2 * fw))
+                continue
+            low_prev = None
             fused = e16(NB, 2 * fh, 2 * fw, Fc * m2)
             nolo = bool(li == 3 and self.lo8_rows(rh_in))
             nopl = bool(nolo and self.hi8_rows(rh_in))
diff --git a/include/bodyslam_hip.h b/include/bodyslam_hip.h
--- a/include/bodyslam_hip.h
+++ b/include/bodyslam_hip.h
@@ -71,6 +71,8 @@
     const float* bias2;
     int32_t qkv_lo_off;
     int32_t out2_relu;
+    const void* res2_up;
+    int32_t res2_up_hin, res2_up_win, res2_up_hout, res2_up_wout;
 } bs_gemm_desc;
 int bs_gemm(const bs_gemm_desc* d, void* stream);
 int bs_gemm_tile(const bs_gemm_desc* d);
```

Measured after the change: 488.3. 0.984x the previous value.
